# nomic-ai/contrastors

Measured on AMD Instinct MI355X. Metric: query-doc pairs/sec (whole node), nomic-bert-2048 seq128 global-batch 16384, higher is better.
Workload: dtype bf16

## Files before the change

contrastors_amd/_C.py:

```python
from __future__ import annotations

import ctypes as C
import os
from pathlib import Path

_PKG = Path(__file__).resolve().parent
LIB_PATH = Path(os.environ.get("CONTRASTORS_HIP_LIB", _PKG / "lib" / "libcontrastors_hip.so"))

CX_OK = 0
_ERR = {-1: "CX_ERR_SHAPE", -2: "CX_ERR_ALIGN", -3: "CX_ERR_ARG", -4: "CX_ERR_LAUNCH"}

vp = C.c_void_p
i32 = C.c_int
i64 = C.c_long
f32 = C.c_float
u64 = C.c_ulonglong
u32 = C.c_uint


class CxLayerWeights(C.Structure):
    _fields_ = (
        [(n, vp) for n in ("Wqkv", "Wout", "Wfc1", "Wfc2", "WqkvT", "WoutT", "Wfc1T", "Wfc2T")]
        + [(n, vp) for n in ("bqkv", "bout", "bfc1", "bfc2")]
        + [(n, vp) for n in ("ln1_g", "ln1_b", "ln2_g", "ln2_b")]
# ... 52 lines not shown
    "cx_error_string": (C.c_char_p, [i32]),
    "cx_gemm_bf16_nt": (i32, [vp, vp, vp, vp, i32, i32, i32, i32, i32, i32, i32, i32, f32, vp]),
    "cx_gemm_bf16_nt_accum": (i32, [vp, vp, vp, vp, i64, i32, i32, i32, i32, i32, vp]),
    "cx_gemm_bf16_tn_accum": (i32, [vp, vp, vp, vp, i64, i32, i32, i32, i32, i32, vp]),
    "cx_prof_gemm_config": (i32, [i32, i32]),
    "cx_prof_gemm_collect": (i32, [C.POINTER(C.c_double), C.POINTER(C.c_double), C.POINTER(i64), C.POINTER(i64)]),
    "cx_calib_mfma_bf16": (i32, [vp, i32, i32, vp, vp, vp]),
    "cx_calib_copy": (i32, [vp, vp, i64, vp]),
    "cx_transpose_bf16": (i32, [vp, vp, i32, i32, i32, i32, i32, vp]),
    "cx_cast_f32_to_bf16": (i32, [vp, vp, i64, vp]),
    "cx_cast_transpose_f32_to_bf16": (i32, [vp, vp, i32, i32, vp]),
    "cx_cast_transpose_f32_to_bf16_batched": (i32, [vp, i32, i32, vp]),
    "cx_cast_bf16_to_f32": (i32, [vp, vp, i64, vp]),
    "cx_layernorm_fwd": (i32, [vp, vp, vp, vp, vp, vp, vp, vp, i32, i32, f32, vp]),
    "cx_layernorm_bwd": (i32, [vp, vp, vp, vp, vp, vp, vp, vp, vp, vp, vp, i64, i32, i32, vp]),
    "cx_layernorm_bwd_pooled": (i32, [vp, vp, vp, vp, i32, i32, i32, vp, vp, vp, vp, vp, vp, vp, vp, vp, i64, i32, i32, vp]),
    "cx_layernorm_bwd_colsum": (i32, [vp, vp, vp, vp, vp, vp, vp, vp, vp, vp, vp, vp, i64, i32, i32, vp]),
    "cx_dropout_add_layernorm_fwd": (i32, [vp, vp, vp, vp, vp, vp, vp, vp, i32, i32, f32, f32, C.c_ulonglong, C.c_ulonglong,
                                           C.c_uint, vp]),
    "cx_dropout_add_layernorm_bwd": (i32, [vp, vp, vp, vp, vp, vp, vp, vp, vp, vp, vp, i64, i32, i32, f32, C.c_ulonglong,
                                           C.c_ulonglong, C.c_uint, vp]),
    "cx_dropout_add_layernorm_bwd_colsum": (i32, [vp, vp, vp, vp, vp, vp, vp, vp, vp, vp, vp, vp, i64, i32, i32, f32, C.c_ulonglong,
                                                  C.c_ulonglong, C.c_uint, vp]),
    "cx_dropout_scale": (i32, [vp, i64, f32, C.c_ulonglong, C.c_ulonglong, C.c_uint, vp]),
    "cx_layernorm_fwd_mixed": (i32, [vp, vp, vp, vp, vp, vp, vp, vp, i32, i32, f32, i32, vp]),
    "cx_layernorm_bwd_mixed": (i32, [vp, vp, vp, vp, vp, vp, vp, vp, vp, vp, i32, i32, i32, vp]),
    "cx_embed_ln_fwd": (i32, [vp, vp, vp, vp, vp, vp, vp, vp, vp, vp, i32, i32, i32, f32, vp]),
    "cx_embed_ln_bwd": (i32, [vp] * 15 + [i32, i32, i32, i32, vp]),
    "cx_embed_ln_bwd_sorted": (i32, [vp] * 15 + [i32, i32, i32, i32, i32, vp, vp, vp, vp]),
    "cx_swiglu_fwd": (i32, [vp, vp, i32, i32, i32, vp]),
    "cx_swiglu_bwd": (i32, [vp, vp, vp, i32, i32, i32, vp]),
    "cx_gemm_bf16_swiglu": (i32, [vp, vp, vp, vp, i32, i32, i32, i32, i32, i32, i32, vp]),
    "cx_gemm_bf16_nt_residual": (i32, [vp, vp, vp, vp, vp, i32, i32, i32, i32, i32, i32, i32, vp]),
    "cx_gemm_bf16_swiglu_bwd": (i32, [vp, vp, vp, vp, i32, i32, i32, i32, i32, i32, vp]),
    "cx_gemm_bf16_nt_splitk": (i32, [vp, vp, vp, vp, vp, vp, i64, i32, i32, i32, i32, i32, i32, i32, vp]),
    "cx_gemm_bf16_swiglu_gate": (i32, [vp, vp, vp, vp, i32, i32, i32, i32, i32, i32, i32, vp]),
    "cx_gemm_bf16_swiglu_bwd_gate": (i32, [vp, vp, vp, vp, vp, i32, i32, i32, i32, i32, i32, i32, vp]),
    "cx_swiglu_bwd_gate": (i32, [vp, vp, vp, vp, i32, i32, vp]),
    "cx_gemm_bf16_bias_gelu": (i32, [vp, vp, vp, vp, vp, i32, i32, i32, i32, i32, i32, i32, vp]),
    "cx_gemm_bf16_bias_act": (i32, [vp, vp, vp, vp, vp, i32, i32, i32, i32, i32, i32, i32, i32, vp]),
    "cx_bias_gelu_fwd": (i32, [vp, vp, vp, i32, i32, vp]),
    "cx_bias_gelu_bwd": (i32, [vp, vp, vp, vp, i32, i32, vp]),
    "cx_bias_grad": (i32, [vp, vp, i32, i32, i32, vp]),
    "cx_bias_gelu_bwd_colsum": (i32, [vp, vp, vp, vp, vp, i32, i32, vp]),
    "cx_bias_act_fwd": (i32, [vp, vp, vp, i32, i32, i32, vp]),
    "cx_bias_act_bwd_colsum": (i32, [vp, vp, vp, vp, vp, i32, i32, i32, vp]),
    "cx_gemm_bf16_act_bwd": (i32, [vp, vp, vp, vp, vp, vp, i64, i32, i32, i32, i32, i32, i32, i32, i32, vp]),
    "cx_attn_varlen_fwd": (i32, [vp, vp, vp, vp, vp, vp, i32, i32, i32, i32, f32, vp]),
    "cx_attn_varlen_bwd": (i32, [vp] * 9 + [i32, i32, i32, i32, f32, vp]),
    "cx_attn_varlen_bwd_prerotated": (i32, [vp] * 9 + [i32, i32, i32, i32, f32, vp]),
    "cx_attn_varlen_dropout_fwd": (i32, [vp] * 6 + [i32, i32, i32, i32, f32, f32, u64, u64, u32, vp]),
    "cx_attn_varlen_dropout_bwd": (i32, [vp] * 9 + [i32, i32, i32, i32, f32, f32, u64, u64, u32, vp]),
    "cx_ipc_alloc": (i32, [C.POINTER(vp), i64, i32]),
    "cx_ipc_free": (i32, [vp]),
    "cx_ipc_export": (i32, [vp, vp]),
    "cx_ipc_open": (i32, [vp, C.POINTER(vp)]),
    "cx_ipc_close": (i32, [vp]),
    "cx_xgmi_push": (i32, [vp, vp, i64, i64, i32, vp]),
    "cx_xgmi_scatter": (i32, [vp, vp, i32, i64, i32, vp]),
    "cx_xgmi_signal_wait": (i32, [vp, vp, i32, i32, u32, i64, vp, vp]),
    "cx_sum_slots_f32": (i32, [vp, vp, i64, i32, vp]),
    "cx_attn_varlen_kvpacked_fwd": (i32, [vp] * 6 + [i32, i32, i32, i32, i32, f32, vp]),
    "cx_attn_varlen_kvpacked_bwd": (i32, [vp] * 10 + [i32, i32, i32, i32, i32, f32, vp]),
    "cx_rotary_qkv_inplace": (i32, [vp, vp, vp, vp, i32, i32, i32, i32, i32, vp]),
    "cx_rotary_apply": (i32, [vp, i64, vp, vp, vp, i32, i32, i32, i32, i32, vp]),
    "cx_pool_normalize_fwd": (i32, [vp, vp, vp, vp, i32, i32, i32, i32, vp]),
# ... 29 lines not shown
    "cx_infonce_ws_floats": (i64, [i32, i32]),
    "cx_infonce_fwd": (i32, [vp, vp, vp, f32, vp, vp, vp, i32, i32, i32, i32, i32, vp]),
    "cx_infonce_argmax_ws_floats": (i64, [i32, i32]),
    "cx_infonce_fwd_argmax": (i32, [vp, vp, vp, f32, vp, vp, vp, vp, i32, i32, i32, i32, i32, vp]),
    "cx_infonce_bwd": (i32, [vp, vp, vp, vp, f32, f32, vp, vp, vp, vp, vp, vp, vp, i32, i32, i32, i32, i32, vp]),
    "cx_search_ws_bytes": (i64, [i32, i64, i32, i32]),
    "cx_search_topk": (i32, [vp, vp, i32, i64, i32, i64, i64, i32, vp, vp, vp, i32, vp, vp, vp, vp]),
    "cx_pack_sign_bits": (i32, [vp, i32, i64, i32, i64, vp, i64, vp]),
    "cx_search_hamming_ws_bytes": (i64, [i32, i64, i32, i32]),
    "cx_search_hamming_topk": (i32, [vp, vp, i32, i64, i32, i64, i64, i32, vp, vp, vp, i32, vp, vp, vp, vp]),
    "cx_rescore_topk": (i32, [vp, vp, vp, vp, i32, i64, i32, i64, i64, i32, i32, vp, vp, vp, vp]),
    "cx_embed_ln_fwd_typed": (i32, [vp, vp, vp, vp, vp, i32, vp, vp, vp, vp, vp, vp, i32, i32, i32, f32, vp]),
    "cx_embed_ln_bwd_typed": (i32, [vp] * 7 + [i32] + [vp] * 10 + [i64, i32, i32, i32, i32, vp]),
    "cx_embed_ln_bwd_sorted_typed": (i32, [vp] * 7 + [i32] + [vp] * 10 + [i64, i32, i32, i32, i32, i32, vp, vp, vp, vp]),
    "cx_seqcls_ws_floats": (i64, [i32, i32, i32]),
    "cx_seqcls_head_fwd": (i32, [vp, i64, vp, vp, vp, vp, vp, i32, f32, u64, u64, vp, vp, vp, i32, i32, i32, vp]),
    "cx_seqcls_head_bwd": (i32, [vp, i64, vp, vp, vp, vp, vp, i32, f32, f32, u64, u64, vp, i64, vp, vp, vp, vp, vp, i32, i32,
                                 i32, vp]),
    "cx_simkl_ws_floats": (i64, [i32, i32]),
    "cx_simkl_fwd": (i32, [vp, vp, vp, vp, f32, vp, vp, vp, vp, i32, i32, i32, i32, i32, i32, i32, i32, vp]),
    "cx_simkl_bwd": (i32, [vp, vp, vp, vp, vp, vp, f32, f32, vp, vp, vp, vp, vp, vp, i32, i32, i32, i32, i32, i32, i32, i32, vp]),
    "cx_infonce_fp8_ws_floats": (i64, [i32, i32]),
    "cx_infonce_fp8_fwd": (i32, [vp, vp, vp, f32, vp, vp, vp, vp, vp, vp, vp, i32, i32, i32, i32, i32, vp]),
    "cx_infonce_fp8_bwd": (i32, [vp, vp, vp, vp, f32, f32, vp, vp, vp, vp, vp, vp, vp, vp, vp, i64, vp, vp, vp, i32, i32, i32,
                                 i32, i32, vp]),
    "cx_sgemm_nt": (i32, [vp, vp, vp, i32, i32, i32, i32, i32, i32, vp]),
    "cx_transpose_f32": (i32, [vp, vp, i32, i32, i32, i32, vp]),
    "cx_encoder_forward": (i32, [C.POINTER(CxEncoderDesc), C.POINTER(CxChunkBuffers), vp, vp, vp, i32, i32, i32,
                                 i32, i32, vp, vp]),
    "cx_encoder_forward_typed": (i32, [C.POINTER(CxEncoderDesc), C.POINTER(CxChunkBuffers), vp, vp, vp, vp, i32, i32, i32,
                                       i32, i32, vp, vp]),
    "cx_encoder_backward_typed": (i32, [C.POINTER(CxEncoderDesc), C.POINTER(CxChunkBuffers), vp, vp, vp, vp, i32, i32, i32,
                                        i32, vp, vp, vp, vp, vp]),
    "cx_encoder_forward_hidden": (i32, [C.POINTER(CxEncoderDesc), C.POINTER(CxChunkBuffers), vp, vp, vp, i32, i32, i32,
                                        i32, i32, vp, vp]),
    "cx_encoder_backward_hidden": (i32, [C.POINTER(CxEncoderDesc), C.POINTER(CxChunkBuffers), vp, vp, vp, i32, i32, i32,
                                         i32, vp, vp, vp, vp]),
    "cx_encoder_backward": (i32, [C.POINTER(CxEncoderDesc), C.POINTER(CxChunkBuffers), vp, vp, vp, i32, i32, i32,
                                  i32, vp, vp, vp, vp, vp]),
}

_DEV_SIGS = {
    "cx_gemm_set_variant": (None, [i32]),
    "cx_gemm_get_variant": (i32, []),
    "cx_gemm_set_debug": (None, [i32]),
    "cx_gemm_set_trace": (None, [vp]),
    "cx_gemm_v6_ablate": (None, [i32]),
    "cx_gemm_v6_trace": (None, [vp]),
    "cx_gemm_v7_mode": (None, [i32]),
    "cx_gemm_v7_trace": (None, [vp]),
    "cx_gemm_v7_occupancy": (i32, []),
    "cx_gemm_v7_ablate": (None, [i32]),
    "cx_gemm_v7_flags": (None, [i32]),
    "cx_gemm_v7_period": (None, [i32]),
    "cx_gemm_set_glds": (None, [i32]),
    "cx_gemm_get_glds": (i32, []),
    "cx_attn_set_bwd_s128": (None, [i32]),
    "cx_attn_set_prio": (None, [i32]),
    "cx_attn_set_fwd_s128": (None, [i32]),
    "cx_attn_set_fwd_long": (None, [i32]),
    "cx_attn_set_bwd_long": (None, [i32]),
    "cx_probe_mfma_layout": (i32, [vp, vp]),
    "cx_probe_ds_read_tr16": (i32, [vp, vp, vp]),
    "cx_probe_mfma_rate": (i32, [vp, i32, i32, i32, vp, vp, vp]),
    "cx_attn_dropout_keep_mask": (i32, [vp, i32, i32, i32, f32, u64, u64, u32, vp]),
    "cx_probe_rmw": (i32, [vp, i64, i32, i32, i32, vp]),
# ... 61 lines not shown
```

contrastors_amd/csrc/cx_common.h:

```cpp
#pragma once
#include <hip/hip_runtime.h>
#include <stdint.h>
#include "../../include/contrastors_hip.h"

typedef uint16_t bf16_t;

typedef __attribute__((ext_vector_type(8))) __bf16 bf16x8_t;
typedef __attribute__((ext_vector_type(4))) __bf16 bf16x4_t;
typedef __attribute__((ext_vector_type(16))) float f32x16_t;
typedef __attribute__((ext_vector_type(4))) float f32x4_t;
typedef __attribute__((ext_vector_type(2))) float f32x2_t;
typedef __attribute__((ext_vector_type(4))) uint32_t u32x4_t;
typedef __attribute__((ext_vector_type(2))) uint32_t u32x2_t;

#define CX_DEVICE __device__ __forceinline__

CX_DEVICE float bf16_to_f32(bf16_t v) { return __uint_as_float(((uint32_t)v) << 16); }
CX_DEVICE float bf16lo_to_f32(uint32_t packed) { return __uint_as_float(packed << 16); }
CX_DEVICE float bf16hi_to_f32(uint32_t packed) { return __uint_as_float(packed & 0xffff0000u); }

typedef float cx_f32x2 __attribute__((ext_vector_type(2)));
typedef __bf16 cx_bf16x2 __attribute__((ext_vector_type(2)));
CX_DEVICE uint32_t pack_bf16x2(float lo, float hi) {
    const cx_f32x2 v = {lo, hi};
// ... 14 lines not shown
    v.z = pack_bf16x2(f[4], f[5]); v.w = pack_bf16x2(f[6], f[7]);
    return v;
}
CX_DEVICE void load8_f32(const float* p, float (&f)[8]) {
    const float4 a = *reinterpret_cast<const float4*>(p), b = *reinterpret_cast<const float4*>(p + 4);
    f[0] = a.x; f[1] = a.y; f[2] = a.z; f[3] = a.w; f[4] = b.x; f[5] = b.y; f[6] = b.z; f[7] = b.w;
}

CX_DEVICE int ycol(int c, int I, int layout) { return layout ? ((c >> 5) << 6) + (c & 31) : c; }
CX_DEVICE int gcol(int c, int I, int layout) { return layout ? ((c >> 5) << 6) + 32 + (c & 31) : I + c; }

CX_DEVICE float sigmoid_fast(float x) { return __builtin_amdgcn_rcpf(1.f + __builtin_amdgcn_exp2f(-1.4426950408889634f * x)); }

CX_DEVICE void rotary_pair(float x1, float x2, float c, float s, float& o1, float& o2) {
#pragma clang fp contract(off)
    o1 = __builtin_fmaf(x1, c, -(x2 * s));
    o2 = __builtin_fmaf(x2, c, x1 * s);
}

CX_DEVICE float rcp_clamped(float g) { return __builtin_amdgcn_fmed3f(__builtin_amdgcn_rcpf(g), -3.4028235e38f, 3.4028235e38f); }
CX_DEVICE void swiglu_bwd_from_act(float d, float act, float g, float& dy, float& dg) {
    const float s = sigmoid_fast(g);
    dy = g * s * d;
    dg = (d * act) * (rcp_clamped(g) + 1.f - s);
}
typedef float cx_f2 __attribute__((ext_vector_type(2)));
CX_DEVICE void swiglu_bwd_from_act2(cx_f2 d, cx_f2 act, cx_f2 g, cx_f2& dy, cx_f2& dg) {
    const cx_f2 m = g * -1.4426950408889634f;
    const cx_f2 t = cx_f2{__builtin_amdgcn_exp2f(m.x), __builtin_amdgcn_exp2f(m.y)} + 1.f;
    const cx_f2 s = {__builtin_amdgcn_rcpf(t.x), __builtin_amdgcn_rcpf(t.y)};
    dy = g * s * d;
    const cx_f2 w = cx_f2{rcp_clamped(g.x), rcp_clamped(g.y)} + 1.f - s;
    dg = (d * act) * w;
}

CX_DEVICE float gelu_cdf(float v, float& gauss) {
    const float av = fabsf(v);
    const float t = __builtin_amdgcn_rcpf(1.f + 0.3275911f * 0.70710678118654752f * av);
    const float poly =
        t * (0.254829592f + t * (-0.284496736f + t * (1.421413741f + t * (-1.453152027f + t * 1.061405429f))));
    gauss = __builtin_amdgcn_exp2f(-0.72134752044448170f * v * v);
    const float erf_abs = 1.f - poly * gauss;
    return 0.5f * (1.f + copysignf(erf_abs, v));
}

enum { CX_ACT_GELU = 0, CX_ACT_QUICK_GELU = 1 };
CX_DEVICE float act_val(float v, int act) {
    if (act == CX_ACT_QUICK_GELU) return v * __builtin_amdgcn_rcpf(1.f + __builtin_amdgcn_exp2f(-1.702f * 1.4426950408889634f * v));
    float gauss;
    return v * gelu_cdf(v, gauss);
}
CX_DEVICE float act_grad(float v, int act) {
    if (act == CX_ACT_QUICK_GELU) {
        const float s = __builtin_amdgcn_rcpf(1.f + __builtin_amdgcn_exp2f(-1.702f * 1.4426950408889634f * v));
        return s * (1.f + 1.702f * v * (1.f - s));
    }
    float gauss;
    const float cdf = gelu_cdf(v, gauss);
    return cdf + v * 0.3989422804014327f * gauss;
}

CX_DEVICE float wave_sum(float v) {
#pragma unroll
    for (int o = 32; o > 0; o >>= 1) v += __shfl_xor(v, o, 64);
    return v;
}
// ... 67 lines not shown
```

contrastors_amd/csrc/engine.hip:

```cpp
#include <hip/hip_runtime.h>
#include "../../include/contrastors_hip.h"
#include "ln_workspace.h"

namespace {

#define CX_TRY(expr)              \
    do {                          \
        int rc__ = (expr);        \
        if (rc__ != CX_OK) return rc__; \
    } while (0)

inline long round_up(long v, long m) { return (v + m - 1) / m * m; }

inline int mark_grads_done(const CxChunkBuffers* buf, int idx, void* stream) {
    if (!buf->layer_events || !buf->layer_events[idx]) return CX_OK;
    return hipEventRecord((hipEvent_t)buf->layer_events[idx], (hipStream_t)stream) == hipSuccess ? CX_OK : CX_ERR_LAUNCH;
}

struct Slots {
    const CxChunkBuffers* b;
    const CxEncoderDesc* e;
    long T_cap;
    int d, I, wfc1;
    int mode;
// ... 40 lines not shown
                 save ? (buf->checkpoint ? 2 : 1) : 0, L - keep};
}

int check_desc(const CxEncoderDesc* e, const CxChunkBuffers* b, int T) {
    if (!e || !b || !e->layers) return CX_ERR_ARG;
    if (e->n_layer <= 0 || e->d <= 0 || e->n_head <= 0) return CX_ERR_ARG;
    if (e->d != e->n_head * 64) return CX_ERR_SHAPE;
    if ((e->d % 64) != 0 || (e->d_inner % 64) != 0) return CX_ERR_SHAPE;
    if (b->T_cap < round_up(T, 64)) return CX_ERR_SHAPE;
    return CX_OK;
}

int wgrad_split(int out_f, int in_f, long Tp) {
    const long tiles = (long)((out_f + 127) / 128) * ((in_f + 127) / 128);
    const long nk = Tp / 64;
    long s = (512 + tiles - 1) / tiles;
    if (s > nk / 2) s = nk / 2;
    if (s < 1) s = 1;
    return (int)s;
}

int wgrad(const uint16_t* dY, int out_f, const uint16_t* X, int in_f, float* gW, const CxChunkBuffers* b, int T,
          void* stream) {
    if (!gW) return CX_OK;
    const int rc = cx_gemm_bf16_tn_accum(dY, X, gW, b->ws_f32, b->ws_floats, T, out_f, in_f, out_f, in_f, stream);
    if (rc != CX_ERR_SHAPE) return rc;
    if (!b->tr_a || !b->tr_b) return CX_ERR_ARG;
    const int Tp = (int)round_up(T, 64);
    CX_TRY(cx_transpose_bf16(dY, b->tr_a, T, out_f, out_f, Tp, Tp, stream));
    CX_TRY(cx_transpose_bf16(X, b->tr_b, T, in_f, in_f, Tp, Tp, stream));
    return cx_gemm_bf16_nt_accum(b->tr_a, b->tr_b, gW, b->ws_f32, b->ws_floats, out_f, in_f, Tp, Tp, Tp, stream);
}

int proj_residual(const uint16_t* x, const uint16_t* W, const float* bias, const uint16_t* residual, uint16_t* out, int T,
                  int N, int K, bool* folded, void* stream, const CxChunkBuffers* buf = nullptr) {
    *folded = false;
    if (buf && buf->ws_f32 && (long)((T + 255) / 256) * ((N + 255) / 256) <= 64 && K >= 1536) {
        const int rc = cx_gemm_bf16_nt_splitk(x, W, out, bias, residual, buf->ws_f32, buf->ws_floats, T, N, K, K, K, N, N, stream);
        if (rc != CX_ERR_SHAPE) {
            *folded = residual != nullptr && rc == CX_OK;
            return rc;
        }
    }
    if (residual) {
        const int rc = cx_gemm_bf16_nt_residual(x, W, out, bias, residual, T, N, K, K, K, N, N, stream);
        if (rc != CX_ERR_SHAPE) {
            *folded = rc == CX_OK;
            return rc;
        }
    }
    return cx_gemm_bf16_nt(x, W, out, bias, T, N, K, K, K, N, 0, 1, 1.f, stream);
}

bool gelu_fused_shape(int T, int N, int K) {
    return T > 0 && (K % 64) == 0 && (N % 8) == 0;
}

struct BlockRunner {
    const CxEncoderDesc* enc;
    const CxChunkBuffers* buf;
    const Slots& s;
    const int32_t* cu_seqlens;
    int Bc, T, max_seqlen;
    void* stream;
    const CxVitExt* ext = nullptr;

    int mlp_up(const CxLayerWeights& w, const uint16_t* x, int l, bool keep) const {
        const int d = enc->d, I = enc->d_inner;
        if (ext_subln(ext)) {
            uint16_t* yg = ext->yg_wide ? ext->yg_wide : buf->g_wide;
            CX_TRY(cx_gemm_bf16_nt(x, w.Wfc1, yg, w.bfc1, T, 2 * I, d, d, d, 2 * I, 0, 1, 1.f, stream));
            const CxVitSubLN& n = ext->sub_ln[l];
            return cx_swiglu_subln_fwd(yg, n.norm_g, n.norm_b, keep ? s.yg(l) : nullptr, s.act(l), s.ez(ext, l), s.ezmean(ext, l),
                                       s.ezrstd(ext, l), T, I, ext->subln_eps, stream);
        }
        if (enc->gated) {
            return cx_gemm_bf16_swiglu_gate(x, w.Wfc1, keep ? s.yg(l) : nullptr, s.act(l), T, I, d, d, d, I, I, stream);
        }
        const int rc = cx_gemm_bf16_bias_act(x, w.Wfc1, w.bfc1, keep ? s.yg(l) : nullptr, s.act(l), T, s.wfc1, d, d, d, s.wfc1,
                                             I, enc->mlp_act, stream);
        if (rc != CX_ERR_SHAPE) return rc;
        CX_TRY(cx_gemm_bf16_nt(x, w.Wfc1, s.yg(l), nullptr, T, s.wfc1, d, d, d, s.wfc1, 0, 1, 1.f, stream));
        return cx_bias_act_fwd(s.yg(l), w.bfc1, s.act(l), T, I, enc->mlp_act, stream);
    }
    int mlp(const CxLayerWeights& w, const uint16_t* x, int l, uint16_t* out, const uint16_t* residual, bool keep,
            bool* folded) const {
        CX_TRY(mlp_up(w, x, l, keep));
        return proj_residual(ext_subln(ext) ? s.ez(ext, l) : s.act(l), w.Wfc2, w.bfc2, residual, out, T, enc->d, enc->d_inner, folded, stream, buf);
    }
    int attn(const CxLayerWeights& w, const uint16_t* x, int l, uint16_t* out, const uint16_t* residual, bool* folded) const {
        const int d = enc->d;
        CX_TRY(cx_gemm_bf16_nt(x, w.Wqkv, s.qkv(l), w.bqkv, T, 3 * d, d, d, d, 3 * d, 0, 1, 1.f, stream));
        if (ext_rope(ext))
            CX_TRY(cx_rope2d_qkv_inplace(s.qkv(l), cu_seqlens, ext->rope_cos, ext->rope_sin, ext->n_rope, Bc, enc->n_head, T,
                                         ext->n_prefix, 1, stream));
        if (buf->drop_active && enc->attn_pdrop > 0.f) {
            CX_TRY(cx_attn_varlen_dropout_fwd(s.qkv(l), cu_seqlens, enc->rot_cos, enc->rot_sin, s.ctx(l), s.lse(l), Bc,
                                              enc->n_head, T, max_seqlen, enc->softmax_scale, enc->attn_pdrop, buf->drop_seed,
                                              buf->drop_offset, (unsigned)(2 * enc->n_layer + 1 + l), stream));
        } else if (enc->rot_cos && max_seqlen > 128) {
            CX_TRY(cx_rotary_qkv_inplace(s.qkv(l), cu_seqlens, enc->rot_cos, enc->rot_sin, Bc, enc->n_head, T, max_seqlen, 1,
                                         stream));
            CX_TRY(cx_attn_varlen_fwd(s.qkv(l), cu_seqlens, nullptr, nullptr, s.ctx(l), s.lse(l), Bc, enc->n_head, T, max_seqlen,
                                      enc->softmax_scale, stream));
        } else {
            CX_TRY(cx_attn_varlen_fwd(s.qkv(l), cu_seqlens, enc->rot_cos, enc->rot_sin, s.ctx(l), s.lse(l), Bc, enc->n_head, T,
                                      max_seqlen, enc->softmax_scale, stream));
        }
        return proj_residual(s.ctx(l), w.Wout, w.bout, residual, out, T, d, d, folded, stream);
    }
    int post_block(int l, const uint16_t* h_in, bool keep) const {
        const CxLayerWeights& w = enc->layers[l];
        const int d = enc->d;
        bool f1 = false, f2 = false;
        if (drop()) {
            const float p = enc->resid_pdrop;
            CX_TRY(attn(w, h_in, l, s.z1(l), nullptr, &f1));
            CX_TRY(cx_dropout_add_layernorm_fwd(s.z1(l), h_in, w.ln1_g, w.ln1_b, s.h1(l), keep ? s.z1(l) : nullptr, s.mean1(l),
                                                s.rstd1(l), T, d, enc->ln_eps, p, buf->drop_seed, buf->drop_offset, 2 * l, stream));
            CX_TRY(mlp(w, s.h1(l), l, s.z2(l), nullptr, keep, &f2));
            return cx_dropout_add_layernorm_fwd(s.z2(l), s.h1(l), w.ln2_g, w.ln2_b, s.h2(l), keep ? s.z2(l) : nullptr, s.mean2(l),
                                                s.rstd2(l), T, d, enc->ln_eps, p, buf->drop_seed, buf->drop_offset, 2 * l + 1,
                                                stream);
        }
        CX_TRY(attn(w, h_in, l, s.z1(l), h_in, &f1));
        CX_TRY(cx_layernorm_fwd(s.z1(l), f1 ? nullptr : h_in, w.ln1_g, w.ln1_b, s.h1(l), (keep && !f1) ? s.z1(l) : nullptr,
                                s.mean1(l), s.rstd1(l), T, d, enc->ln_eps, stream));
        CX_TRY(mlp(w, s.h1(l), l, s.z2(l), s.h1(l), keep, &f2));
        return cx_layernorm_fwd(s.z2(l), f2 ? nullptr : s.h1(l), w.ln2_g, w.ln2_b, s.h2(l), (keep && !f2) ? s.z2(l) : nullptr,
                                s.mean2(l), s.rstd2(l), T, d, enc->ln_eps, stream);
    }
    bool drop() const { return buf->drop_active && enc->resid_pdrop > 0.f; }
    int pre_block(int l, const uint16_t* x, const uint16_t* r, bool r_folded, bool keep, bool up_only, const uint16_t** x_out,
                  const uint16_t** r_out, bool* folded_out) const {
        const CxLayerWeights& w = enc->layers[l];
        const int d = enc->d, L = enc->n_layer;
        CX_TRY(cx_layernorm_fwd(x, r, w.ln1_g, w.ln1_b, s.h1(l), (r_folded && x == s.z1(l)) ? nullptr : s.z1(l), s.mean1(l),
                                s.rstd1(l), T, d, enc->ln_eps, stream));
        bool f1 = false, f2 = false;
        CX_TRY(attn(w, s.h1(l), l, s.z2(l), s.z1(l), &f1));
        CX_TRY(cx_layernorm_fwd(s.z2(l), f1 ? nullptr : s.z1(l), w.ln2_g, w.ln2_b, s.h2(l), f1 ? nullptr : s.z2(l), s.mean2(l),
                                s.rstd2(l), T, d, enc->ln_eps, stream));
        if (up_only) return mlp_up(w, s.h2(l), l, keep);
        uint16_t* nxt = (l + 1 < L) ? s.z1(l + 1) : buf->zf;
        CX_TRY(mlp(w, s.h2(l), l, nxt, s.z2(l), keep, &f2));
        *x_out = nxt;
        *r_out = f2 ? nullptr : s.z2(l);
        *folded_out = f2;
        return CX_OK;
    }
};

int blocks_forward(const CxEncoderDesc* enc, const CxChunkBuffers* buf, const Slots& s, const uint16_t* h0,
                   const int32_t* cu_seqlens, int Bc, int T, int max_seqlen, int save, const uint16_t** h_final,
                   void* stream, const CxVitExt* ext = nullptr) {
    const int d = enc->d, L = enc->n_layer;
    const BlockRunner run{enc, buf, s, cu_seqlens, Bc, T, max_seqlen, stream, ext};
    if (!enc->prenorm) {
        const uint16_t* h_in = h0;
        for (int l = 0; l < L; ++l) {
            CX_TRY(run.post_block(l, h_in, save != 0 && s.kept(l)));
            h_in = s.h2(l);
        }
        *h_final = h_in;
        return CX_OK;
    }
    if (!buf->zf || !buf->hf || !buf->meanf || !buf->rstdf || (!ext_no_lnf(ext) && (!enc->lnf_g || !enc->lnf_b))) return CX_ERR_ARG;
    if (buf->drop_active && enc->resid_pdrop > 0.f) return CX_ERR_ARG;
    const uint16_t* x = h0;
    const uint16_t* r = nullptr;
    bool r_folded = false;
    for (int l = 0; l < L; ++l) {
        CX_TRY(run.pre_block(l, x, r, r_folded, save != 0 && s.kept(l), false, &x, &r, &r_folded));
        if (save == 2 && !r_folded) return CX_ERR_SHAPE;
    }
    if (ext_no_lnf(ext)) {
        if (!r_folded || x != buf->zf) return CX_ERR_SHAPE;
        *h_final = buf->zf;
        return CX_OK;
    }
    CX_TRY(cx_layernorm_fwd(x, r, enc->lnf_g, enc->lnf_b, buf->hf, r_folded ? nullptr : buf->zf, buf->meanf, buf->rstdf, T,
                            d, enc->ln_eps, stream));
    *h_final = buf->hf;
    return CX_OK;
}

int check_bwd_buffers(const CxChunkBuffers* buf) {
    return (!buf->g_a || !buf->g_b || !buf->g_c || !buf->g_wide || !buf->g_act || !buf->delta ||
            !buf->ws_f32) ? CX_ERR_ARG : CX_OK;
}
// ... 3 lines not shown
    const int Tp = (int)round_up(T, 64);
    if (Tp == T) return CX_OK;
    const int d = enc->d, I = enc->d_inner, L = enc->n_layer;
    auto clear = [&](uint16_t* base, int width) {
        return hipMemsetAsync(base + (size_t)T * width, 0, (size_t)(Tp - T) * width * sizeof(uint16_t),
                              (hipStream_t)stream) == hipSuccess ? CX_OK : CX_ERR_LAUNCH;
    };
    CX_TRY(clear(buf->g_a, d));
    CX_TRY(clear(buf->g_b, d));
    CX_TRY(clear(buf->g_c, d));
    if (buf->g_d) CX_TRY(clear(buf->g_d, d));
    CX_TRY(clear(buf->g_wide, 3 * d));
    CX_TRY(clear(buf->g_wide, s.wfc1));
    CX_TRY(clear(buf->h0, d));
    for (int l = 0; l < L; ++l) {
        CX_TRY(clear(s.act(l), I));
        CX_TRY(clear(s.h1(l), d));
        CX_TRY(clear(s.ctx(l), d));
        CX_TRY(clear(s.h2(l), d));
        if (ext_subln(ext)) CX_TRY(clear(s.ez(ext, l), I));
    }
    return CX_OK;
}

struct PooledGrad {
    const float* demb;
    const float* emb;
    const float* norm;
    int pool_mode, normalize;
};

int blocks_backward(const CxEncoderDesc* enc, const CxChunkBuffers* buf, const Slots& s, const int32_t* cu_seqlens, int Bc,
                    int T, int max_seqlen, const PooledGrad* pg, const uint16_t** da_out, const uint16_t** db_out, void* stream,
                    const CxVitExt* ext = nullptr) {
    const int d = enc->d, I = enc->d_inner, H = enc->n_head, L = enc->n_layer;
    auto mlp_bwd = [&](const CxLayerWeights& w, int l, const uint16_t* dm, const uint16_t* mlp_in, const uint16_t* add,
                       bool* folded, bool bias_done) -> int {
        if (w.gbfc2 && !bias_done) CX_TRY(cx_bias_grad(dm, w.gbfc2, T, d, d, stream));
        if (ext_subln(ext)) {
            CX_TRY(wgrad(dm, d, s.ez(ext, l), I, w.gWfc2, buf, T, stream));
            CX_TRY(cx_gemm_bf16_nt(dm, w.Wfc2T, buf->g_act, nullptr, T, I, d, d, d, I, 0, 1, 1.f, stream));
            const CxVitSubLN& n = ext->sub_ln[l];
            CX_TRY(cx_swiglu_subln_bwd(buf->g_act, s.act(l), s.yg(l), s.ezmean(ext, l), s.ezrstd(ext, l), n.norm_g, buf->g_wide,
                                       n.gnorm_g, n.gnorm_b, w.gbfc1, buf->ws_f32, buf->ws_floats, T, I, stream));
            CX_TRY(wgrad(buf->g_wide, s.wfc1, mlp_in, d, w.gWfc1, buf, T, stream));
            return proj_residual(buf->g_wide, w.Wfc1T, nullptr, add, buf->g_b, T, d, s.wfc1, folded, stream, buf);
        }
        CX_TRY(wgrad(dm, d, s.act(l), I, w.gWfc2, buf, T, stream));
        int fused = CX_ERR_SHAPE;
        if (enc->gated)
            fused = cx_gemm_bf16_swiglu_bwd_gate(dm, w.Wfc2T, s.act(l), s.yg(l), buf->g_wide, T, I, d, d, d, I, s.wfc1, stream);
#ifndef CX_AB_R5_ROUTES
        if (!enc->gated && gelu_fused_shape(T, s.wfc1, d))
            fused = cx_gemm_bf16_act_bwd(dm, w.Wfc2T, s.yg(l), buf->g_wide, w.gbfc1, buf->ws_f32, buf->ws_floats, T, I, d, d, d, I, I,
                                         enc->mlp_act, stream);
#endif
        if (fused != CX_ERR_SHAPE) {
            CX_TRY(fused);
        } else {
            CX_TRY(cx_gemm_bf16_nt(dm, w.Wfc2T, buf->g_act, nullptr, T, I, d, d, d, I, 0, 1, 1.f, stream));
        }
        if (enc->gated) {
            if (fused == CX_ERR_SHAPE)
                CX_TRY(cx_swiglu_bwd_gate(buf->g_act, s.act(l), s.yg(l), buf->g_wide, T, I, stream));
        } else if (fused == CX_ERR_SHAPE) {
            CX_TRY(cx_bias_act_bwd_colsum(buf->g_act, s.yg(l), gelu_fused_shape(T, s.wfc1, d) ? nullptr : w.bfc1, buf->g_wide,
                                          w.gbfc1, T, I, enc->mlp_act, stream));
// ... 2 lines not shown
        return proj_residual(buf->g_wide, w.Wfc1T, nullptr, add, buf->g_b, T, d, s.wfc1, folded, stream, buf);
    };
    auto attn_bwd = [&](const CxLayerWeights& w, int l, const uint16_t* dx, const uint16_t* attn_in, const uint16_t* add,
                        bool* folded, bool bias_done) -> int {
        if (w.gbout && !bias_done) CX_TRY(cx_bias_grad(dx, w.gbout, T, d, d, stream));
        CX_TRY(wgrad(dx, d, s.ctx(l), d, w.gWout, buf, T, stream));
        CX_TRY(cx_gemm_bf16_nt(dx, w.WoutT, buf->g_b, nullptr, T, d, d, d, d, d, 0, 1, 1.f, stream));
        if (buf->drop_active && enc->attn_pdrop > 0.f) {
            CX_TRY(cx_attn_varlen_dropout_bwd(buf->g_b, s.qkv(l), s.ctx(l), s.lse(l), cu_seqlens, enc->rot_cos, enc->rot_sin,
                                              buf->delta, buf->g_wide, Bc, H, T, max_seqlen, enc->softmax_scale, enc->attn_pdrop,
                                              buf->drop_seed, buf->drop_offset, (unsigned)(2 * enc->n_layer + 1 + l), stream));
        } else if (enc->rot_cos && max_seqlen > 128) {
            CX_TRY(cx_attn_varlen_bwd_prerotated(buf->g_b, s.qkv(l), s.ctx(l), s.lse(l), cu_seqlens, enc->rot_cos, enc->rot_sin,
                                                 buf->delta, buf->g_wide, Bc, H, T, max_seqlen, enc->softmax_scale, stream));
        } else {
            CX_TRY(cx_attn_varlen_bwd(buf->g_b, s.qkv(l), s.ctx(l), s.lse(l), cu_seqlens, enc->rot_cos, enc->rot_sin,
                                      buf->delta, buf->g_wide, Bc, H, T, max_seqlen, enc->softmax_scale, stream));
        }
        if (ext_rope(ext))
            CX_TRY(cx_rope2d_qkv_inplace(buf->g_wide, cu_seqlens, ext->rope_cos, ext->rope_sin, ext->n_rope, Bc, H, T, ext->n_prefix,
                                         -1, stream));
        if (w.gbqkv) CX_TRY(cx_bias_grad(buf->g_wide, w.gbqkv, T, 3 * d, 3 * d, stream));
        CX_TRY(wgrad(buf->g_wide, 3 * d, attn_in, d, w.gWqkv, buf, T, stream));
        return proj_residual(buf->g_wide, w.WqkvT, nullptr, add, buf->g_b, T, d, 3 * d, folded, stream, buf);
    };
    const bool ws_holds_colsum = cx_ln_bwd_ws_holds(buf->ws_f32, buf->ws_floats, 3, d);
    auto ln_bwd = [&](const uint16_t* a, const uint16_t* b2, const uint16_t* z, const float* g, const float* mean,
                      const float* rstd, const uint16_t* dz_extra, uint16_t* dz, float* gg, float* gb, float* gbias,
                      bool* done) -> int {
        *done = gbias && ws_holds_colsum;
        return cx_layernorm_bwd_colsum(a, b2, z, g, mean, rstd, dz_extra, dz, gg, gb, *done ? gbias : nullptr, buf->ws_f32,
                                       buf->ws_floats, T, d, stream);
    };
    const BlockRunner run{enc, buf, s, cu_seqlens, Bc, T, max_seqlen, stream, ext};
    if (!enc->prenorm) {
        const uint16_t* da = buf->g_a;
        const uint16_t* db = nullptr;
        for (int l = L - 1; l >= 0; --l) {
            const CxLayerWeights& w = enc->layers[l];
            const uint16_t* h_in = (l == 0) ? buf->h0 : s.h2(l - 1);
            if (!s.kept(l)) CX_TRY(run.post_block(l, h_in, true));
            if (run.drop()) {
                if (!buf->g_d) return CX_ERR_ARG;
                const float p = enc->resid_pdrop;
                bool f1 = false, f2 = false;
#ifdef CX_AB_R5_ROUTES
                const bool cs = false;
#else
                const bool cs = ws_holds_colsum;
#endif
                CX_TRY(cx_dropout_add_layernorm_bwd_colsum(da, db, s.z2(l), w.ln2_g, s.mean2(l), s.rstd2(l), buf->g_c, buf->g_d, w.gln2_g,
                                                           w.gln2_b, cs ? w.gbfc2 : nullptr, buf->ws_f32, buf->ws_floats, T, d, p,
                                                           buf->drop_seed, buf->drop_offset, 2 * l + 1, stream));
                CX_TRY(mlp_bwd(w, l, buf->g_d, s.h1(l), buf->g_c, &f1, cs));
                CX_TRY(cx_dropout_add_layernorm_bwd_colsum(f1 ? buf->g_b : buf->g_c, f1 ? nullptr : buf->g_b, s.z1(l), w.ln1_g, s.mean1(l),
                                                           s.rstd1(l), buf->g_a, buf->g_d, w.gln1_g, w.gln1_b, cs ? w.gbout : nullptr,
                                                           buf->ws_f32, buf->ws_floats, T, d, p, buf->drop_seed, buf->drop_offset, 2 * l,
                                                           stream));
                CX_TRY(attn_bwd(w, l, buf->g_d, h_in, buf->g_a, &f2, cs));
                da = f2 ? buf->g_b : buf->g_a;
                db = f2 ? nullptr : buf->g_b;
                CX_TRY(mark_grads_done(buf, l, stream));
                continue;
            }
            bool b2_done = false, b1_done = false;
            if (pg && l == L - 1) {
                const bool cs = w.gbfc2 && ws_holds_colsum;
// ... 124 lines not shown
                                     enc->normalize, stream));
    }
    const uint16_t* da = nullptr;
    const uint16_t* db = nullptr;
    CX_TRY(blocks_backward(enc, buf, s, cu_seqlens, Bc, T, S, fold_pool ? &pg : nullptr, &da, &db, stream, ext));
    if (db) return CX_ERR_ARG;
    if (enc->lnpre_g) {
        if (!buf->zpre) return CX_ERR_ARG;
        CX_TRY(cx_layernorm_bwd(da, nullptr, buf->zpre, enc->lnpre_g, buf->emb_mean, buf->emb_rstd, nullptr, buf->g_a,
                                enc->glnpre_g, enc->glnpre_b, buf->ws_f32, buf->ws_floats, T, d, stream));
        da = buf->g_a;
    }
    const int Tp = Bc * P, Tpp = (int)round_up(Tp, 64);
    if (Tpp > Tp) {
        if (hipMemsetAsync(buf->patch_proj + (size_t)Tp * d, 0, (size_t)(Tpp - Tp) * d * 2, (hipStream_t)stream) != hipSuccess ||
            hipMemsetAsync(buf->patch_in + (size_t)Tp * enc->patch_dim, 0, (size_t)(Tpp - Tp) * enc->patch_dim * 2,
                           (hipStream_t)stream) != hipSuccess)
            return CX_ERR_LAUNCH;
    }
    if (buf->patch_keep) {
        if (!buf->patch_inv || buf->n_keep != P || buf->n_patch_all < P) return CX_ERR_ARG;
        CX_TRY(cx_vit_assemble_bwd_gather(da, buf->patch_proj, enc->gcls_token, enc->gvit_pos, Bc, P, d, buf->patch_inv,
                                          buf->n_patch_all, stream));
    } else {
        CX_TRY(cx_vit_assemble_bwd(da, buf->patch_proj, enc->gcls_token, enc->gvit_pos, Bc, P, d, stream));
    }
    if (enc->gbpatch) CX_TRY(cx_bias_grad(buf->patch_proj, enc->gbpatch, Tp, d, d, stream));
    CX_TRY(wgrad(buf->patch_proj, d, buf->patch_in, enc->patch_dim, enc->gWpatch, buf, Tp, stream));
    return mark_grads_done(buf, enc->n_layer, stream);
}

int text_forward_impl(const CxEncoderDesc* enc, const CxChunkBuffers* buf, const int64_t* input_ids,
                      const int64_t* token_type_ids, const int32_t* indices, const int32_t* cu_seqlens, int Bc, int S, int T,
                      int max_seqlen, int save_for_backward, float* emb_out, void* stream) {
    if (Bc <= 0 || T <= 0) return CX_OK;
    CX_TRY(check_desc(enc, buf, T));
    (void)hipGetLastError();
    const int d = enc->d, I = enc->d_inner;
    const Slots s = make_slots(enc, buf, save_for_backward);
    if (token_type_ids)
        CX_TRY(cx_embed_ln_fwd_typed(input_ids, token_type_ids, indices, enc->word_emb, enc->type_emb, 2, enc->pos_emb,
                                     enc->emb_ln_g, enc->emb_ln_b, buf->h0, buf->emb_mean, buf->emb_rstd, T, S, d, enc->ln_eps,
                                     stream));
    else
        CX_TRY(cx_embed_ln_fwd(input_ids, indices, enc->word_emb, enc->type_emb, enc->pos_emb, enc->emb_ln_g,
                               enc->emb_ln_b, buf->h0, buf->emb_mean, buf->emb_rstd, T, S, d, enc->ln_eps, stream));
    if (buf->drop_active && enc->embd_pdrop > 0.f)
        CX_TRY(cx_dropout_scale(buf->h0, (long)T * d, enc->embd_pdrop, buf->drop_seed, buf->drop_offset, 2 * enc->n_layer, stream));
    const uint16_t* h_final = nullptr;
    CX_TRY(blocks_forward(enc, buf, s, buf->h0, cu_seqlens, Bc, T, max_seqlen, s.mode, &h_final, stream));
    return cx_pool_normalize_fwd(h_final, cu_seqlens, emb_out, buf->pool_norm, Bc, d, enc->pool_mode, enc->normalize,
                                 stream);
}

int text_backward_impl(const CxEncoderDesc* enc, const CxChunkBuffers* buf, const int64_t* input_ids,
                       const int64_t* token_type_ids, const int32_t* indices, const int32_t* cu_seqlens, int Bc, int S, int T,
                       int max_seqlen, const float* demb, const float* emb_out, const int32_t* sort_ids,
                       const int32_t* sort_perm, void* stream) {
    if (Bc <= 0 || T <= 0) return CX_OK;
    CX_TRY(check_desc(enc, buf, T));
    if (!demb || !emb_out) return CX_ERR_ARG;
    CX_TRY(check_bwd_buffers(buf));
    (void)hipGetLastError();
    const int d = enc->d, I = enc->d_inner;
    const Slots s = make_slots(enc, buf, 1);
    CX_TRY(clear_pad_rows(enc, buf, s, T, stream));
    const PooledGrad pg{demb, emb_out, buf->pool_norm, enc->pool_mode, enc->normalize};
    const bool fold_pool = !(buf->drop_active && enc->resid_pdrop > 0.f) && (enc->pool_mode == 0 || enc->pool_mode == 1);
    if (!fold_pool)
        CX_TRY(cx_pool_normalize_bwd(demb, emb_out, buf->pool_norm, cu_seqlens, buf->g_a, Bc, d, enc->pool_mode,
                                     enc->normalize, stream));
    const uint16_t* da = fold_pool ? nullptr : buf->g_a;
    const uint16_t* db = nullptr;
    CX_TRY(blocks_backward(enc, buf, s, cu_seqlens, Bc, T, max_seqlen, fold_pool ? &pg : nullptr, &da, &db, stream));
    if (buf->drop_active && enc->embd_pdrop > 0.f) {
        CX_TRY(cx_dropout_scale(const_cast<uint16_t*>(da), (long)T * d, enc->embd_pdrop, buf->drop_seed, buf->drop_offset,
                                2 * enc->n_layer, stream));
        if (db)
            CX_TRY(cx_dropout_scale(const_cast<uint16_t*>(db), (long)T * d, enc->embd_pdrop, buf->drop_seed, buf->drop_offset,
                                    2 * enc->n_layer, stream));
    }
    if (token_type_ids && sort_ids && sort_perm) {
        CX_TRY(cx_embed_ln_bwd_sorted_typed(da, db, input_ids, token_type_ids, indices, enc->word_emb, enc->type_emb, 2,
                                            enc->pos_emb, enc->emb_ln_g, buf->emb_mean, buf->emb_rstd, enc->gword_emb,
                                            enc->gtype_emb, enc->gpos_emb, enc->gemb_ln_g, enc->gemb_ln_b, buf->ws_f32,
                                            buf->ws_floats, T, S, d, enc->padding_idx, enc->vocab, sort_ids, sort_perm,
                                            reinterpret_cast<float*>(buf->g_wide), stream));
    } else if (token_type_ids) {
        CX_TRY(cx_embed_ln_bwd_typed(da, db, input_ids, token_type_ids, indices, enc->word_emb, enc->type_emb, 2, enc->pos_emb,
                                     enc->emb_ln_g, buf->emb_mean, buf->emb_rstd, enc->gword_emb, enc->gtype_emb, enc->gpos_emb,
                                     enc->gemb_ln_g, enc->gemb_ln_b, buf->ws_f32, buf->ws_floats, T, S, d, enc->padding_idx,
                                     stream));
    } else if (sort_ids && sort_perm) {
        CX_TRY(cx_embed_ln_bwd_sorted(da, db, input_ids, indices, enc->word_emb, enc->type_emb, enc->pos_emb, enc->emb_ln_g,
                                      buf->emb_mean, buf->emb_rstd, enc->gword_emb, enc->gtype_emb, enc->gpos_emb,
                                      enc->gemb_ln_g, enc->gemb_ln_b, T, S, d, enc->padding_idx, enc->vocab, sort_ids,
                                      sort_perm, reinterpret_cast<float*>(buf->g_wide), stream));
    } else {
        CX_TRY(cx_embed_ln_bwd(da, db, input_ids, indices, enc->word_emb, enc->type_emb, enc->pos_emb, enc->emb_ln_g,
                               buf->emb_mean, buf->emb_rstd, enc->gword_emb, enc->gtype_emb, enc->gpos_emb,
                               enc->gemb_ln_g, enc->gemb_ln_b, T, S, d, enc->padding_idx, stream));
    }
    return mark_grads_done(buf, enc->n_layer, stream);
}
}

extern "C" {

int cx_encoder_forward(const CxEncoderDesc* enc, const CxChunkBuffers* buf, const int64_t* input_ids,
                       const int32_t* indices, const int32_t* cu_seqlens, int Bc, int S, int T, int max_seqlen,
                       int save_for_backward, float* emb_out, void* stream) {
    return text_forward_impl(enc, buf, input_ids, nullptr, indices, cu_seqlens, Bc, S, T, max_seqlen, save_for_backward, emb_out,
                             stream);
}
int cx_encoder_forward_typed(const CxEncoderDesc* enc, const CxChunkBuffers* buf, const int64_t* input_ids,
                             const int64_t* token_type_ids, const int32_t* indices, const int32_t* cu_seqlens, int Bc, int S,
                             int T, int max_seqlen, int save_for_backward, float* emb_out, void* stream) {
    return text_forward_impl(enc, buf, input_ids, token_type_ids, indices, cu_seqlens, Bc, S, T, max_seqlen, save_for_backward,
                             emb_out, stream);
}

int cx_encoder_backward(const CxEncoderDesc* enc, const CxChunkBuffers* buf, const int64_t* input_ids,
                        const int32_t* indices, const int32_t* cu_seqlens, int Bc, int S, int T, int max_seqlen,
                        const float* demb, const float* emb_out, const int32_t* sort_ids, const int32_t* sort_perm,
                        void* stream) {
    return text_backward_impl(enc, buf, input_ids, nullptr, indices, cu_seqlens, Bc, S, T, max_seqlen, demb, emb_out, sort_ids,
                              sort_perm, stream);
}
int cx_encoder_backward_typed(const CxEncoderDesc* enc, const CxChunkBuffers* buf, const int64_t* input_ids,
                              const int64_t* token_type_ids, const int32_t* indices, const int32_t* cu_seqlens, int Bc, int S,
                              int T, int max_seqlen, const float* demb, const float* emb_out, const int32_t* sort_ids,
                              const int32_t* sort_perm, void* stream) {
    return text_backward_impl(enc, buf, input_ids, token_type_ids, indices, cu_seqlens, Bc, S, T, max_seqlen, demb, emb_out,
                              sort_ids, sort_perm, stream);
}

int cx_encoder_forward_hidden(const CxEncoderDesc* enc, const CxChunkBuffers* buf, const int64_t* input_ids,
                              const int32_t* indices, const int32_t* cu_seqlens, int Bc, int S, int T, int max_seqlen,
                              int save_for_backward, uint16_t* hidden_out, void* stream) {
    if (Bc <= 0 || T <= 0) return CX_OK;
    CX_TRY(check_desc(enc, buf, T));
    if (!hidden_out) return CX_ERR_ARG;
    (void)hipGetLastError();
    const int d = enc->d, I = enc->d_inner;
    const Slots s = make_slots(enc, buf, save_for_backward);
    CX_TRY(cx_embed_ln_fwd(input_ids, indices, enc->word_emb, enc->type_emb, enc->pos_emb, enc->emb_ln_g,
                           enc->emb_ln_b, buf->h0, buf->emb_mean, buf->emb_rstd, T, S, d, enc->ln_eps, stream));
    if (buf->drop_active && enc->embd_pdrop > 0.f)
        CX_TRY(cx_dropout_scale(buf->h0, (long)T * d, enc->embd_pdrop, buf->drop_seed, buf->drop_offset, 2 * enc->n_layer, stream));
    const uint16_t* h_final = nullptr;
    CX_TRY(blocks_forward(enc, buf, s, buf->h0, cu_seqlens, Bc, T, max_seqlen, s.mode, &h_final, stream));
    return hipMemcpyAsync(hidden_out, h_final, (size_t)T * d * sizeof(uint16_t), hipMemcpyDeviceToDevice,
                          (hipStream_t)stream) == hipSuccess ? CX_OK : CX_ERR_LAUNCH;
}

int cx_encoder_backward_hidden(const CxEncoderDesc* enc, const CxChunkBuffers* buf, const int64_t* input_ids,
                               const int32_t* indices, const int32_t* cu_seqlens, int Bc, int S, int T, int max_seqlen,
                               const uint16_t* dhidden, const int32_t* sort_ids, const int32_t* sort_perm, void* stream) {
    if (Bc <= 0 || T <= 0) return CX_OK;
    CX_TRY(check_desc(enc, buf, T));
    if (!dhidden) return CX_ERR_ARG;
    CX_TRY(check_bwd_buffers(buf));
    (void)hipGetLastError();
    const int d = enc->d, I = enc->d_inner;
    const Slots s = make_slots(enc, buf, 1);
    CX_TRY(clear_pad_rows(enc, buf, s, T, stream));
    if (hipMemcpyAsync(buf->g_a, dhidden, (size_t)T * d * sizeof(uint16_t), hipMemcpyDeviceToDevice,
// ... 94 lines not shown
```

contrastors_amd/csrc/gemm_api.hip:

```cpp
#include "cx_common.h"
#include "../../include/contrastors_hip.h"
#include "gemm_params.h"
#include <mutex>

namespace {

constexpr int BK = 64;

__global__ __launch_bounds__(256) void splitk_reduce_kernel(const float* __restrict__ part, float* __restrict__ out, long n4,
                                                            long slab, int splits) {
    const long stride = (long)gridDim.x * blockDim.x;
    for (long i = (long)blockIdx.x * blockDim.x + threadIdx.x; i < n4; i += stride) {
        float4 a = reinterpret_cast<const float4*>(out)[i];
        for (int s = 0; s < splits; ++s) {
            const float4 v = reinterpret_cast<const float4*>(part + s * slab)[i];
            a.x += v.x; a.y += v.y; a.z += v.z; a.w += v.w;
        }
        reinterpret_cast<float4*>(out)[i] = a;
    }
}

int reduce_slabs(const float* ws, float* out, long slab, int split, hipStream_t s) {
    const long n4 = slab / 4;
    long g = (n4 + 255) / 256;
// ... 133 lines not shown
    GemmParams p = base_params(X, W, YG, nullptr, M, 2 * I, K, ldx, ldw, ld_yg);
    p.Out2 = Act; p.ldo2 = ld_act;
    ProfScope prof(2.0 * (double)M * (double)(2 * I) * (double)K, (hipStream_t)stream);
    const hipError_t e = ((ld_yg % 8) == 0 && (ld_act % 8) == 0)
                             ? cx_launch_gemm_v6(p, GEMM_EPI_SWIGLU, (hipStream_t)stream)
                             : cx_launch_gemm_v5(p, 0, GEMM_OUT_BF16, GEMM_EPI_SWIGLU, (hipStream_t)stream);
    return e == hipSuccess ? CX_OK : CX_ERR_LAUNCH;
}

int cx_gemm_bf16_swiglu_gate(const uint16_t* X, const uint16_t* W, uint16_t* G, uint16_t* Act, int M, int I, int K, int ldx,
                             int ldw, int ld_g, int ld_act, void* stream) {
    if (M <= 0 || I <= 0) return CX_OK;
    if (K <= 0 || (K % BK) != 0 || (I % 32) != 0 || (ld_g % 8) != 0 || (ld_act % 8) != 0) return CX_ERR_SHAPE;
    if ((ldx % 8) != 0 || (ldw % 8) != 0) return CX_ERR_ALIGN;
    if (!Act) return CX_ERR_ARG;
    GemmParams p = base_params(X, W, G, nullptr, M, 2 * I, K, ldx, ldw, ld_g);
    p.Out2 = Act; p.ldo2 = ld_act;
    ProfScope prof(2.0 * (double)M * (double)(2 * I) * (double)K, (hipStream_t)stream);
    return cx_launch_gemm_v6(p, GEMM_EPI_SWIGLU_G, (hipStream_t)stream) == hipSuccess ? CX_OK : CX_ERR_LAUNCH;
}

int cx_gemm_bf16_nt_residual(const uint16_t* X, const uint16_t* W, uint16_t* Out, const float* bias, const uint16_t* Residual,
                             int M, int N, int K, int ldx, int ldw, int ldo, int ldr, void* stream) {
    if (M <= 0 || N <= 0) return CX_OK;
    if (!Residual || !Out) return CX_ERR_ARG;
    if (K <= 0 || (K % 64) != 0 || (N % 8) != 0 || (ldo % 8) != 0 || (ldr % 8) != 0) return CX_ERR_SHAPE;
    if ((ldx % 8) != 0 || (ldw % 8) != 0) return CX_ERR_ALIGN;
    GemmParams p = base_params(X, W, Out, bias, M, N, K, ldx, ldw, ldo);
    p.Out2 = const_cast<uint16_t*>(Residual); p.ldo2 = ldr;
    ProfScope prof(2.0 * (double)M * (double)N * (double)K, (hipStream_t)stream);
    return cx_launch_gemm_v6(p, GEMM_EPI_NONE, (hipStream_t)stream) == hipSuccess ? CX_OK : CX_ERR_LAUNCH;
}

int cx_gemm_bf16_bias_gelu(const uint16_t* X, const uint16_t* W, const float* bias, uint16_t* Pre, uint16_t* Act, int M, int N,
                           int K, int ldx, int ldw, int ld_pre, int ld_act, void* stream) {
    return cx_gemm_bf16_bias_act(X, W, bias, Pre, Act, M, N, K, ldx, ldw, ld_pre, ld_act, 0, stream);
}

int cx_gemm_bf16_bias_act(const uint16_t* X, const uint16_t* W, const float* bias, uint16_t* Pre, uint16_t* Act, int M, int N,
                          int K, int ldx, int ldw, int ld_pre, int ld_act, int act, void* stream) {
    if (M <= 0 || N <= 0) return CX_OK;
    if (!Act || (act != 0 && act != 1)) return CX_ERR_ARG;
    if (K <= 0 || (K % 64) != 0 || (N % 8) != 0 || (ld_act % 8) != 0 || (Pre && (ld_pre % 8) != 0)) return CX_ERR_SHAPE;
    if ((ldx % 8) != 0 || (ldw % 8) != 0) return CX_ERR_ALIGN;
    GemmParams p = base_params(X, W, Pre, bias, M, N, K, ldx, ldw, ld_pre);
    p.Out2 = Act; p.ldo2 = ld_act;
    p.act = act;
    ProfScope prof(2.0 * (double)M * (double)N * (double)K, (hipStream_t)stream);
    return cx_launch_gemm_v6(p, act == 1 ? GEMM_EPI_QGELU : GEMM_EPI_GELU, (hipStream_t)stream) == hipSuccess ? CX_OK : CX_ERR_LAUNCH;
}

int cx_gemm_bf16_swiglu_bwd(const uint16_t* dY, const uint16_t* W, const uint16_t* YG, uint16_t* dYG, int M, int I, int K,
                            int ldx, int ldw, int ld_yg, void* stream) {
    if (M <= 0 || I <= 0) return CX_OK;
    if (!dY || !W || !YG || !dYG) return CX_ERR_ARG;
    if (K <= 0 || (K % 64) != 0 || (I % 256) != 0 || (ld_yg % 8) != 0 || ld_yg < 2 * I) return CX_ERR_SHAPE;
    if ((ldx % 8) != 0 || (ldw % 8) != 0) return CX_ERR_ALIGN;
    GemmParams p = base_params(dY, W, dYG, nullptr, M, I, K, ldx, ldw, ld_yg);
    p.Out2 = const_cast<uint16_t*>(YG); p.ldo2 = ld_yg;
    ProfScope prof(2.0 * (double)M * (double)I * (double)K, (hipStream_t)stream);
    return cx_launch_gemm_v6(p, GEMM_EPI_SWIGLU_BWD, (hipStream_t)stream) == hipSuccess ? CX_OK : CX_ERR_LAUNCH;
}

int cx_gemm_bf16_swiglu_bwd_gate(const uint16_t* dY, const uint16_t* W, const uint16_t* Act, const uint16_t* G, uint16_t* dYG,
                                 int M, int I, int K, int ldx, int ldw, int ld_ag, int ld_dyg, void* stream) {
    if (M <= 0 || I <= 0) return CX_OK;
// ... 61 lines not shown
```

contrastors_amd/csrc/gemm_bf16.hip:

```cpp
#include "cx_common.h"
#include "../../include/contrastors_hip.h"
#include "gemm_params.h"

namespace {

constexpr int BM = 128, BN = 128, BK = 64;
constexpr int TILE_BYTES = 128 * BK * 2;

typedef __attribute__((address_space(3))) void* lds_void_ptr;
typedef const __attribute__((address_space(1))) void* glb_void_ptr;

enum OutMode { OUT_BF16 = GEMM_OUT_BF16, OUT_F32 = GEMM_OUT_F32, OUT_F32_ATOMIC = GEMM_OUT_F32_ATOMIC };

struct StageRegs { uint4 r0, r1, r2, r3; };

CX_DEVICE uint4 stage_load(const bf16_t* __restrict__ base, int ld, int row0, int nrows, int k0, int tid, int p) {
    const int r = p * 32 + (tid >> 3);
    int gr = row0 + r;
    gr = gr < nrows ? gr : nrows - 1;
    return *reinterpret_cast<const uint4*>(base + (size_t)gr * ld + k0 + (tid & 7) * 8);
}

template <bool GLDS>
CX_DEVICE void stage_tile(const bf16_t* __restrict__ base, int ld, int row0, int nrows, int k0, char* lds_tile,
// ... 765 lines not shown

int cx_gemm_bf16_nt_residual(const uint16_t* X, const uint16_t* W, uint16_t* Out, const float* bias,
                             const uint16_t* Residual, int M, int N, int K, int ldx, int ldw, int ldo, int ldr,
                             void* stream) {
    if (M <= 0 || N <= 0) return CX_OK;
    if (!Residual || !Out) return CX_ERR_ARG;
    if (K <= 0 || (K % 64) != 0 || (N % 8) != 0 || (ldo % 8) != 0 || (ldr % 8) != 0) return CX_ERR_SHAPE;
    if ((ldx % 8) != 0 || (ldw % 8) != 0) return CX_ERR_ALIGN;
    if (cx_gemm_get_variant() != 6) return CX_ERR_SHAPE;
    GemmParams p;
    p.X = X; p.W = W; p.Out = Out; p.bias = bias;
    p.M = M; p.N = N; p.K = K; p.ldx = ldx; p.ldw = ldw; p.ldo = ldo;
    p.tiles_m = p.tiles_n = 0; p.split_k = 1; p.alpha = 1.f; p.dbg = g_dbg;
    p.Out2 = const_cast<uint16_t*>(Residual); p.ldo2 = ldr; p.sup_m = p.sup_n = 0; p.trace = nullptr;
    int slot = -1;
    if (g_prof.enabled) {
        if ((g_prof.launches % g_prof.stride) == 0 && g_prof.used < GemmProf::CAP) {
            slot = g_prof.used++;
            if (slot >= g_prof.created) {
                if (hipEventCreate(&g_prof.ev0[slot]) != hipSuccess || hipEventCreate(&g_prof.ev1[slot]) != hipSuccess)
                    return CX_ERR_LAUNCH;
                g_prof.created = slot + 1;
            }
            g_prof.flop[slot] = 2.0 * (double)M * (double)N * (double)K;
            (void)hipEventRecord(g_prof.ev0[slot], (hipStream_t)stream);
        }
        ++g_prof.launches;
    }
    const hipError_t e = cx_launch_gemm_v6(p, GEMM_EPI_NONE, (hipStream_t)stream);
    if (slot >= 0) (void)hipEventRecord(g_prof.ev1[slot], (hipStream_t)stream);
    return e == hipSuccess ? CX_OK : CX_ERR_LAUNCH;
}

int cx_gemm_bf16_bias_gelu(const uint16_t* X, const uint16_t* W, const float* bias, uint16_t* Pre, uint16_t* Act, int M,
                           int N, int K, int ldx, int ldw, int ld_pre, int ld_act, void* stream) {
    return cx_gemm_bf16_bias_act(X, W, bias, Pre, Act, M, N, K, ldx, ldw, ld_pre, ld_act, 0, stream);
}

int cx_gemm_bf16_bias_act(const uint16_t* X, const uint16_t* W, const float* bias, uint16_t* Pre, uint16_t* Act, int M,
                          int N, int K, int ldx, int ldw, int ld_pre, int ld_act, int act, void* stream) {
    if (M <= 0 || N <= 0) return CX_OK;
    if (!Act || (act != 0 && act != 1)) return CX_ERR_ARG;
    if (K <= 0 || (K % 64) != 0 || (N % 8) != 0 || (ld_act % 8) != 0 || (Pre && (ld_pre % 8) != 0)) return CX_ERR_SHAPE;
    if ((ldx % 8) != 0 || (ldw % 8) != 0) return CX_ERR_ALIGN;
    if (cx_gemm_get_variant() != 6) return CX_ERR_SHAPE;
    GemmParams p;
    p.X = X; p.W = W; p.Out = Pre; p.bias = bias;
    p.M = M; p.N = N; p.K = K; p.ldx = ldx; p.ldw = ldw; p.ldo = ld_pre;
    p.tiles_m = p.tiles_n = 0; p.split_k = 1; p.alpha = 1.f; p.dbg = g_dbg;
    p.Out2 = Act; p.ldo2 = ld_act; p.sup_m = p.sup_n = 0; p.trace = nullptr;
    p.act = act;
    int slot = -1;
    if (g_prof.enabled) {
        if ((g_prof.launches % g_prof.stride) == 0 && g_prof.used < GemmProf::CAP) {
            slot = g_prof.used++;
            if (slot >= g_prof.created) {
                if (hipEventCreate(&g_prof.ev0[slot]) != hipSuccess || hipEventCreate(&g_prof.ev1[slot]) != hipSuccess)
                    return CX_ERR_LAUNCH;
                g_prof.created = slot + 1;
            }
            g_prof.flop[slot] = 2.0 * (double)M * (double)N * (double)K;
            (void)hipEventRecord(g_prof.ev0[slot], (hipStream_t)stream);
        }
        ++g_prof.launches;
    }
    const hipError_t e = cx_launch_gemm_v6(p, act == 1 ? GEMM_EPI_QGELU : GEMM_EPI_GELU, (hipStream_t)stream);
// ... 112 lines not shown
```

contrastors_amd/csrc/gemm_bf16_v6.hip:

```cpp
#include "cx_common.h"
#include "../../include/contrastors_hip.h"
#include "gemm_params.h"
#include <type_traits>

namespace {

#ifndef CX_V6_HI_EARLY
#define CX_V6_HI_EARLY 1
#endif
#ifndef CX_V6_OPAQUE
#define CX_V6_OPAQUE 1
#endif
#ifndef CX_V6_NT
#define CX_V6_NT 3
#endif
template <int J>
__device__ __forceinline__ void v6_dma_m0(uint32_t slot_base) {
    asm volatile("s_add_u32 m0, %0, %1" ::"s"(slot_base), "n"(J * 4096) : "memory", "scc");
}
__device__ __forceinline__ void v6_dma_ld(uint32_t off, const bf16_t* base) {
    asm volatile("global_load_lds_dwordx4 %0, %1" ::"v"(off), "s"(base) : "memory");
}
template <int J>
__device__ __forceinline__ void v6_dma_full(uint32_t slot_base, uint32_t off, const bf16_t* base) {
// ... 252 lines not shown
        const char* nxs = dsm + nxs_slot * XS6;
        const char* nws = dsm + (3 + nws_slot) * XS6;
        CX_SEG(mma1, F1, 32, 64, F0, nxs, nws, 0, RS_ == 2 ? 32 : 33, RS_, 2, RS_ == 2 ? 33 : 49, RS_ == 2 ? 8 : DS_, 4, 4);
        x_advance();
        if constexpr ((DBG & 128) != 0 && decltype(first)::value) {
            const long long now_ = (long long)__builtin_amdgcn_s_memtime();
            kt0_cyc += now_ - t_last;
        }
        ++cp_kt;
        pxs_slot = xs_slot;
        pws_slot = ws_slot;
        xs_slot = nxs_slot;
        ws_slot = nws_slot;
    };

#pragma unroll 1
    while (cp_tile >= 0) {
        cp_kt = 0;
        kt_body(std::true_type{});
#pragma unroll 1
        while (cp_kt < nk) kt_body(std::false_type{});

        {
            CX_PH(2);
            asm volatile("s_nop 7\n\ts_nop 7\n\ts_nop 7" ::: "memory");
            const int tn = cp_tile & 255, tm = cp_tile >> 8;
            const int m0 = tm * BM6 + wm * 128, n0 = tn * BN6 + wn * 128;
            char* my = ((wave < 2) ? dsm + pxs_slot * XS6 : dsm + (3 + pws_slot) * XS6) + (wave & 1) * 16384;
            constexpr int ROWB = 272;
            auto prow = [&](int q) { return (q >> 1) * 16 + l15; };
            auto pcol = [&](int q) { return (q & 1) * 16 + 4 * g4; };
            auto qoff = [](int q, int rowb) { return (q >> 1) * 16 * rowb + (q & 1) * 32; };
            if constexpr ((DBG & 16) != 0) {
            } else if constexpr (EPI == GEMM_EPI_NONE || EPI == GEMM_EPI_ACT_BWD || EPI == GEMM_EPI_QACT_BWD) {
                constexpr bool ACTB = EPI == GEMM_EPI_ACT_BWD || EPI == GEMM_EPI_QACT_BWD;
                float cs0 = 0.f, cs1 = 0.f, cs2 = 0.f, cs3 = 0.f, cs4 = 0.f, cs5 = 0.f, cs6 = 0.f, cs7 = 0.f;
                constexpr int act_kind = EPI == GEMM_EPI_QACT_BWD ? CX_ACT_QUICK_GELU : CX_ACT_GELU;
                auto mul_grad = [&](uint4& v, const uint4& r) {
#define CX_MG(w_, ca, cb)                                                                              \
    {                                                                                                 \
        const float o0 = bf16lo_to_f32(v.w_) * act_grad(bf16lo_to_f32(r.w_), act_kind);               \
        const float o1 = bf16hi_to_f32(v.w_) * act_grad(bf16hi_to_f32(r.w_), act_kind);               \
        v.w_ = pack_bf16x2(o0, o1);                                                                   \
        ca += bf16lo_to_f32(v.w_);                                                                    \
        cb += bf16hi_to_f32(v.w_);                                                                    \
    }
                    CX_MG(x, cs0, cs1) CX_MG(y, cs2, cs3) CX_MG(z, cs4, cs5) CX_MG(w, cs6, cs7)
#undef CX_MG
                };
                auto flush_colsum = [&]() {
                    if constexpr (ACTB) {
                        float c[8] = {cs0, cs1, cs2, cs3, cs4, cs5, cs6, cs7};
#pragma unroll
                        for (int e = 0; e < 8; ++e) {
                            c[e] += __shfl_xor(c[e], 16, 64);
                            c[e] += __shfl_xor(c[e], 32, 64);
                        }
                        const int n = n0 + (lane & 15) * 8;
                        if (p.colsum_part && lane < 16 && m0 < p.M && n + 8 <= p.N) {
                            float* dst = p.colsum_part + (size_t)(m0 >> 7) * p.N + n;
                            *reinterpret_cast<float4*>(dst) = make_float4(c[0], c[1], c[2], c[3]);
                            *reinterpret_cast<float4*>(dst + 4) = make_float4(c[4], c[5], c[6], c[7]);
                        }
                    }
                };
                const bool add_bias = p.bias != nullptr;
                const bf16_t* resid = reinterpret_cast<const bf16_t*>(p.Out2);
                auto fast_tile = [&](auto with_resid) {
                    constexpr bool RES = decltype(with_resid)::value;
                    const int rrow = lane >> 4, rch = lane & 15;
                    bf16_t* outp = reinterpret_cast<bf16_t*>(p.Out) + (size_t)(m0 + rrow) * p.ldo + n0 + rch * 8;
                    const bf16_t* resp = RES ? resid + (size_t)(m0 + rrow) * p.ldo2 + n0 + rch * 8 : nullptr;
                    const char* rd = my + rrow * ROWB + rch * 16;
                    char* wr = my + prow(0) * ROWB + pcol(0) * 2;
                    uint2 pk[16];
                    auto pack_pass = [&](int b) {
#pragma unroll
                        for (int a = 0; a < 4; ++a) {
                            float blk[16];
                            v6_read_block(4 * b + a, blk);
#pragma unroll
                            for (int q = 0; q < 4; ++q) {
                                pk[a * 4 + q].x = pack_bf16x2(blk[4 * q], blk[4 * q + 1]);
                                pk[a * 4 + q].y = pack_bf16x2(blk[4 * q + 2], blk[4 * q + 3]);
                            }
                        }
                    };
                    auto stage = [&]() {
#pragma unroll
                        for (int a = 0; a < 4; ++a)
#pragma unroll
                            for (int q = 0; q < 4; ++q) *reinterpret_cast<uint2*>(wr + a * 64 + qoff(q, ROWB)) = pk[a * 4 + q];
                    };
                    uint4 r0 = {}, r1 = {}, r2 = {}, r3 = {}, r4 = {}, r5 = {}, r6 = {}, r7 = {};
#define CX_RES_ROWS(b_)                                                                                   \
    r0 = gld(resp + (size_t)((b_) * 32 + 0) * p.ldo2);                          \
    r1 = gld(resp + (size_t)((b_) * 32 + 4) * p.ldo2);                          \
    r2 = gld(resp + (size_t)((b_) * 32 + 8) * p.ldo2);                          \
    r3 = gld(resp + (size_t)((b_) * 32 + 12) * p.ldo2);                         \
    r4 = gld(resp + (size_t)((b_) * 32 + 16) * p.ldo2);                         \
    r5 = gld(resp + (size_t)((b_) * 32 + 20) * p.ldo2);                         \
    r6 = gld(resp + (size_t)((b_) * 32 + 24) * p.ldo2);                         \
    r7 = gld(resp + (size_t)((b_) * 32 + 28) * p.ldo2);
                    auto add_res = [&](uint4& v, const uint4& r) {
                        v.x = pack_bf16x2(bf16lo_to_f32(v.x) + bf16lo_to_f32(r.x), bf16hi_to_f32(v.x) + bf16hi_to_f32(r.x));
                        v.y = pack_bf16x2(bf16lo_to_f32(v.y) + bf16lo_to_f32(r.y), bf16hi_to_f32(v.y) + bf16hi_to_f32(r.y));
                        v.z = pack_bf16x2(bf16lo_to_f32(v.z) + bf16lo_to_f32(r.z), bf16hi_to_f32(v.z) + bf16hi_to_f32(r.z));
// ... 4 lines not shown
                        uint4 v0 = *reinterpret_cast<const uint4*>(rd + 0 * ROWB), v1 = *reinterpret_cast<const uint4*>(rd + 4 * ROWB),
                              v2 = *reinterpret_cast<const uint4*>(rd + 8 * ROWB), v3 = *reinterpret_cast<const uint4*>(rd + 12 * ROWB),
                              v4 = *reinterpret_cast<const uint4*>(rd + 16 * ROWB), v5 = *reinterpret_cast<const uint4*>(rd + 20 * ROWB),
                              v6 = *reinterpret_cast<const uint4*>(rd + 24 * ROWB), v7 = *reinterpret_cast<const uint4*>(rd + 28 * ROWB);
                        __builtin_amdgcn_sched_barrier(0);
                        if constexpr (b < 3) pack_pass(b + 1);
                        __builtin_amdgcn_sched_barrier(0);
                        if constexpr (RES) {
                            add_res(v0, r0); add_res(v1, r1); add_res(v2, r2); add_res(v3, r3);
                            add_res(v4, r4); add_res(v5, r5); add_res(v6, r6); add_res(v7, r7);
                            if constexpr (b < 3) {
                                __builtin_amdgcn_sched_barrier(0);
                                CX_RES_ROWS(b + 1)
                                __builtin_amdgcn_sched_barrier(0);
                            }
                        }
                        if constexpr (b < 3) stage();
                        bf16_t* o = outp + (size_t)(b * 32) * p.ldo;
                        if constexpr ((DBG & 64) != 0) {
                            const uint4 vs[8] = {v0, v1, v2, v3, v4, v5, v6, v7};
#pragma unroll
                            for (int i = 0; i < 8; ++i) asm volatile("" ::"v"(vs[i].x), "v"(vs[i].y), "v"(vs[i].z), "v"(vs[i].w));
                            asm volatile("" ::"v"(o));
                            return;
                        }
                        gst(o, v0);
                        gst(o + (size_t)4 * p.ldo, v1);
                        gst(o + (size_t)8 * p.ldo, v2);
                        gst(o + (size_t)12 * p.ldo, v3);
                        gst(o + (size_t)16 * p.ldo, v4);
                        gst(o + (size_t)20 * p.ldo, v5);
                        gst(o + (size_t)24 * p.ldo, v6);
                        gst(o + (size_t)28 * p.ldo, v7);
                    };
                    if constexpr (RES) { CX_RES_ROWS(0) }
                    pack_pass(0);
                    stage();
                    one_pass(std::integral_constant<int, 0>{});
                    one_pass(std::integral_constant<int, 1>{});
                    one_pass(std::integral_constant<int, 2>{});
                    one_pass(std::integral_constant<int, 3>{});
#undef CX_RES_ROWS
                };
                auto fast_tile_actb = [&]() {
                    const int rrow = lane >> 4, rch = lane & 15;
                    bf16_t* outp = reinterpret_cast<bf16_t*>(p.Out) + (size_t)(m0 + rrow) * p.ldo + n0 + rch * 8;
                    const bf16_t* resp = resid + (size_t)(m0 + rrow) * p.ldo2 + n0 + rch * 8;
                    const char* rd = my + rrow * ROWB + rch * 16;
                    char* wr = my + prow(0) * ROWB + pcol(0) * 2;
                    auto stage_pass = [&](int b) {
#pragma unroll
                        for (int a = 0; a < 4; ++a) {
                            float blk[16];
                            v6_read_block(4 * b + a, blk);
#pragma unroll
                            for (int q = 0; q < 4; ++q) {
                                uint2 pk2;
                                pk2.x = pack_bf16x2(blk[4 * q], blk[4 * q + 1]);
                                pk2.y = pack_bf16x2(blk[4 * q + 2], blk[4 * q + 3]);
                                *reinterpret_cast<uint2*>(wr + a * 64 + qoff(q, ROWB)) = pk2;
                            }
                            __builtin_amdgcn_sched_barrier(0);
                        }
                    };
                    uint4 r0, r1, r2, r3;
#define CX_PRE_ROWS(hh_)                                                        \
    r0 = gld(resp + (size_t)((hh_) * 16 + 0) * p.ldo2);                         \
    r1 = gld(resp + (size_t)((hh_) * 16 + 4) * p.ldo2);                         \
    r2 = gld(resp + (size_t)((hh_) * 16 + 8) * p.ldo2);                         \
    r3 = gld(resp + (size_t)((hh_) * 16 + 12) * p.ldo2);
// ... 58 lines not shown
                                    if (add_bias) {
                                        const int n = n0 + nl;
                                        if (n < p.N) {
                                            const float4 bv = *reinterpret_cast<const float4*>(p.bias + n);
                                            v[0] += bv.x; v[1] += bv.y; v[2] += bv.z; v[3] += bv.w;
                                        }
                                    }
                                }
                                uint2 pk;
                                pk.x = pack_bf16x2(v[0], v[1]);
                                pk.y = pack_bf16x2(v[2], v[3]);
                                *reinterpret_cast<uint2*>(my + prow(q) * ROWB + nl * 2) = pk;
                            }
                        }
#pragma unroll
                        for (int ps = 0; ps < 8; ++ps) {
                            const int row = ps * 4 + (lane >> 4), ch = lane & 15;
                            const int m = m0 + b * 32 + row, n = n0 + ch * 8;
                            uint4 vv = *reinterpret_cast<const uint4*>(my + row * ROWB + ch * 16);
                            if (resid && ACTB) {
                                const uint4 rr = ps == 0 ? r0 : ps == 1 ? r1 : ps == 2 ? r2 : ps == 3 ? r3 : ps == 4 ? r4 : ps == 5 ? r5
                                                 : ps == 6 ? r6 : r7;
                                if (m < p.M && n + 8 <= p.N) mul_grad(vv, rr);
                            } else if (resid) {
                                const uint4 rr = ps == 0 ? r0 : ps == 1 ? r1 : ps == 2 ? r2 : ps == 3 ? r3 : ps == 4 ? r4 : ps == 5 ? r5
                                                 : ps == 6 ? r6 : r7;
                                vv.x = pack_bf16x2(bf16lo_to_f32(vv.x) + bf16lo_to_f32(rr.x), bf16hi_to_f32(vv.x) + bf16hi_to_f32(rr.x));
                                vv.y = pack_bf16x2(bf16lo_to_f32(vv.y) + bf16lo_to_f32(rr.y), bf16hi_to_f32(vv.y) + bf16hi_to_f32(rr.y));
                                vv.z = pack_bf16x2(bf16lo_to_f32(vv.z) + bf16lo_to_f32(rr.z), bf16hi_to_f32(vv.z) + bf16hi_to_f32(rr.z));
                                vv.w = pack_bf16x2(bf16lo_to_f32(vv.w) + bf16lo_to_f32(rr.w), bf16hi_to_f32(vv.w) + bf16hi_to_f32(rr.w));
                            }
                            if (m < p.M && n + 8 <= p.N)
                                gst(reinterpret_cast<bf16_t*>(p.Out) + (size_t)m * p.ldo + n, vv);
                        }
                    }
                };
                if constexpr (ACTB) {
                    if (fast) {
                        fast_tile_actb();
                    } else {
                        store_tile(std::true_type{});
                    }
                    flush_colsum();
                } else if (fast) {
                    if (resid) {
                        fast_tile(std::true_type{});
                    } else {
                        fast_tile(std::false_type{});
                    }
                } else if (p.alpha == 1.f && !add_bias) {
                    store_tile(std::true_type{});
                } else {
                    store_tile(std::false_type{});
                }
            } else if constexpr (IS_SWIGLU_BWD) {
                const bf16_t* yg_in = reinterpret_cast<const bf16_t*>(p.Out2);
                const bf16_t* g_in = reinterpret_cast<const bf16_t*>(p.In3);
                bf16_t* dyg = reinterpret_cast<bf16_t*>(p.Out);
                const int c0 = 2 * n0;
                auto bwd_elem = [&](float yv, float gv, float dv, float& dyo, float& dgo) {
                    if constexpr (AG) {
                        swiglu_bwd_from_act(dv, yv, gv, dyo, dgo);
                    } else {
                        const float sg = __builtin_amdgcn_rcpf(1.f + __builtin_amdgcn_exp2f(-1.4426950408889634f * gv));
                        const float gs = gv * sg;
                        dyo = gs * dv;
                        dgo = (sg + gs * (1.f - sg)) * dv * yv;
                    }
                };
                auto bwd_quad = [&](const float (&yv)[4], const float (&gv)[4], const float* dv, float (&dyo)[4], float (&dgo)[4]) {
                    if constexpr (AG) {
#pragma unroll
                        for (int h = 0; h < 2; ++h) {
                            cx_f2 y2, g2;
                            swiglu_bwd_from_act2(cx_f2{dv[2 * h], dv[2 * h + 1]}, cx_f2{yv[2 * h], yv[2 * h + 1]},
                                                 cx_f2{gv[2 * h], gv[2 * h + 1]}, y2, g2);
// ... 797 lines not shown
#ifndef CX_PRODUCT
    if (epi == GEMM_EPI_NONE && g_v6_dbg) {
        p.trace = g_v6_trace;
        switch (g_v6_dbg) {
            case 1: return launch6<GEMM_EPI_NONE, 1>(p, stream);
            case 2: return launch6<GEMM_EPI_NONE, 2>(p, stream);
            case 4: return launch6<GEMM_EPI_NONE, 4>(p, stream);
            case 16: return launch6<GEMM_EPI_NONE, 16>(p, stream);
            case 32: return launch6<GEMM_EPI_NONE, 32>(p, stream);
            case 33: return launch6<GEMM_EPI_NONE, 33>(p, stream);
            case 35: return launch6<GEMM_EPI_NONE, 35>(p, stream);
            case 39: return launch6<GEMM_EPI_NONE, 39>(p, stream);
            case 55: return launch6<GEMM_EPI_NONE, 55>(p, stream);
            case 59: return launch6<GEMM_EPI_NONE, 59>(p, stream);
            case 64: return launch6<GEMM_EPI_NONE, 64>(p, stream);
            case 128: return launch6<GEMM_EPI_NONE, 128>(p, stream);
            default: break;
        }
    }
#endif
#ifndef CX_PRODUCT
    if (g_v6_dbg == 128 && (epi == GEMM_EPI_SWIGLU_G || epi == GEMM_EPI_SWIGLU || epi == GEMM_EPI_SWIGLU_BWD_AG)) {
        p.trace = g_v6_trace;
        return epi == GEMM_EPI_SWIGLU_G ? launch6<GEMM_EPI_SWIGLU_G, 128>(p, stream)
               : epi == GEMM_EPI_SWIGLU ? launch6<GEMM_EPI_SWIGLU, 128>(p, stream) : launch6<GEMM_EPI_SWIGLU_BWD_AG, 128>(p, stream);
    }
#endif
    return epi == GEMM_EPI_SWIGLU ? launch6<GEMM_EPI_SWIGLU>(p, stream)
           : epi == GEMM_EPI_SWIGLU_G ? launch6<GEMM_EPI_SWIGLU_G>(p, stream)
           : epi == GEMM_EPI_SWIGLU_BWD_AG ? launch6<GEMM_EPI_SWIGLU_BWD_AG>(p, stream)
           : epi == GEMM_EPI_GELU ? launch6<GEMM_EPI_GELU>(p, stream)
           : epi == GEMM_EPI_QGELU ? launch6<GEMM_EPI_QGELU>(p, stream)
           : epi == GEMM_EPI_SWIGLU_BWD ? launch6<GEMM_EPI_SWIGLU_BWD>(p, stream)
           : epi == GEMM_EPI_ACT_BWD ? (p.act == CX_ACT_QUICK_GELU ? launch6<GEMM_EPI_QACT_BWD>(p, stream) : launch6<GEMM_EPI_ACT_BWD>(p, stream))
                                  : launch6<GEMM_EPI_NONE>(p, stream);
}
```

contrastors_amd/csrc/gemm_bf16_v7.hip:

```cpp
#include "cx_common.h"
#include "../../include/contrastors_hip.h"
#include "gemm_params.h"
#include <type_traits>

namespace {

#ifndef CX_V7_NT
#define CX_V7_NT 3
#endif

template <int IMM>
__device__ __forceinline__ void v7_dma_m0(uint32_t base) {
    asm volatile("s_add_u32 m0, %0, %1" ::"s"(base), "n"(IMM) : "memory", "scc");
}
__device__ __forceinline__ void v7_dma_ld(uint32_t off, const bf16_t* base) {
    asm volatile("global_load_lds_dwordx4 %0, %1" ::"v"(off), "s"(base) : "memory");
}
template <int IMM>
__device__ __forceinline__ void v7_dma_full(uint32_t slot_base, uint32_t off, const bf16_t* base) {
    asm volatile("s_add_u32 m0, %0, %1\n\ts_nop 0\n\tglobal_load_lds_dwordx4 %2, %3" ::"s"(slot_base), "n"(IMM), "v"(off), "s"(base)
                 : "memory", "scc");
}
typedef unsigned int v4u7 __attribute__((ext_vector_type(4)));
__device__ __forceinline__ __amdgpu_buffer_rsrc_t rsrc7(const void* base, uint32_t bytes) {
// ... 13 lines not shown
__device__ __forceinline__ void bst7(__amdgpu_buffer_rsrc_t r, uint32_t voff, uint32_t soff, uint4 v) {
    const v4u7 t = {v.x, v.y, v.z, v.w};
    __builtin_amdgcn_raw_buffer_store_b128(t, r, voff, soff, (CX_V7_NT & 1) ? 2 : 0);
}
template <uint32_t IMM>
__device__ __forceinline__ uint32_t vxor7(uint32_t a) {
    uint32_t r;
    asm volatile("v_xor_b32 %0, %2, %1" : "=v"(r) : "v"(a), "i"(IMM));
    return r;
}

typedef __attribute__((address_space(3))) void* lds_void_ptr7;

constexpr int BM7 = 256, BN7 = 128, BK7 = 64;
constexpr int XW7 = 8192;
constexpr int W0_OFF7 = 32768, SP_OFF7 = 49152, W1_OFF7 = 65536;
constexpr int LDS7 = 81920;

#define V7_MFMA(i, w, x) asm volatile("v_mfma_f32_32x32x16_bf16 %0, %1, %2, %0" : "+a"(acc[(i)]) : "v"(w), "v"(x))
#define V7_MFMA_Z(i, w, x) asm volatile("v_mfma_f32_32x32x16_bf16 %0, %1, %2, 0" : "=a"(acc[(i)]) : "v"(w), "v"(x))

struct XFrags7 {
    bf16x8_t f[2][4];
};
struct WFrags7 {
    bf16x8_t f[4];
};

template <int EPI, int DBG = 0>
__global__ __launch_bounds__(256, 2) __attribute__((amdgpu_waves_per_eu(2, 2))) void gemm_bf16_v7_kernel(GemmParams p) {
    extern __shared__ __attribute__((aligned(16))) char dsm[];
    constexpr bool IS_BWD = EPI == GEMM_EPI_SWIGLU_BWD_AG;
    constexpr bool IS_SWIGLU = EPI == GEMM_EPI_SWIGLU_G;
    static_assert(EPI == GEMM_EPI_NONE || IS_BWD || IS_SWIGLU, "v7 serves the plain / residual, SwiGLU (gate save) and SwiGLU-backward (act, gate) forms");
    const int tid = threadIdx.x;
    const int lane = tid & 63;
    const int wave = __builtin_amdgcn_readfirstlane(tid >> 6);
#ifndef CX_PRODUCT
    long long t_begin = 0;
    if (p.trace) t_begin = (long long)__builtin_amdgcn_s_memtime();
#endif
    const int hi_m = lane >> 5, l31_m = lane & 31;
    const int nk = p.K / BK7;
    const int per_xcd = gridDim.x >> 3;
    const int xcd = blockIdx.x & 7, idx = blockIdx.x >> 3;
    const int gn = p.sup_n > 0 ? p.sup_n : 1, gm = 8 / gn;
    const int xi = xcd / gn, xj = xcd - xi * gn;
    const int m_lo = p.tiles_m * xi / gm, m_hi = p.tiles_m * (xi + 1) / gm;
    const int n_lo = p.tiles_n * xj / gn, n_wd = p.tiles_n * (xj + 1) / gn - n_lo;
    const int nloc = (m_hi - m_lo) * n_wd;
    auto tile_of = [&](int round) {
        const int l = round * per_xcd + idx;
        if (l >= nloc) return -1;
        const int q = l / n_wd;
        return ((m_lo + q) << 8) | (n_lo + (l - q * n_wd));
    };

    uint32_t xoff[8], woff[8];
    const bf16_t* xbase = p.X;
    const bf16_t* wbase = p.W;
    int lx_round = 0, lx_kt = 0;
    int lw_round = 0, lw_kt = 0, lw_slot = 0;
    const int first_tile = tile_of(0);
    bool x_clamped = true, w_clamped = true;
    auto x_setup = [&](int tile) {
        const int tm = tile >> 8;
        xbase = p.X + (size_t)tm * BM7 * p.ldx;
// ... 173 lines not shown
        V7_SLOT(V7_MFMA, 1, W1, 3, 0, 0, read_w(W0, nws, 0, 1));
        V7_SLOT(V7_MFMA, 2, W1, 3, 0, 0, read_w(W0, nws, 0, 2));
        V7_SLOT(V7_MFMA, 3, W1, 3, 0, 0, read_w(W0, nws, 0, 3));
        V7_SLOT(V7_MFMA, 4, W1, 3, 0, 0, V7_NORD);
        V7_SLOT(V7_MFMA, 5, W1, 3, 0, 0, V7_NORD);
        V7_SLOT(V7_MFMA, 6, W1, 3, 0, 0, V7_NORD);
        V7_SLOT(V7_MFMA, 7, W1, 3, 0, 0, V7_NORD);
        ws_slot ^= 1;
    };

#pragma unroll 1
    while (cp_tile >= 0) {
        if (p.dbg & 1) __builtin_amdgcn_s_setprio(1);
        kt_body(std::true_type{});
#pragma unroll 1
        for (int kt = 1; kt < nk; ++kt) kt_body(std::false_type{});

        if (p.dbg & 1) __builtin_amdgcn_s_setprio(0);
        asm volatile("s_nop 7\n\ts_nop 7\n\ts_nop 7" : "+a"(acc[0]), "+a"(acc[1]), "+a"(acc[2]), "+a"(acc[3]), "+a"(acc[4]), "+a"(acc[5]), "+a"(acc[6]), "+a"(acc[7]));
        int le = lane;
        asm volatile("" : "+v"(le));
        const int hi = le >> 5, l31 = le & 31;
        const int tn = cp_tile & 255, tm = cp_tile >> 8;
        const int m0 = tm * BM7 + wave * 64, n0 = tn * BN7;
        const int rows_left = p.M - m0;
        const uint32_t rows_here = rows_left >= 64 ? 64u : (rows_left > 0 ? (uint32_t)rows_left : 0u);
        const uint32_t my = (uint32_t)((ws_slot ? W0_OFF7 : SP_OFF7) + wave * 8192);
        const uint32_t cb = my + (uint32_t)l31 * 256 + ((l31 & 15) << 4) + hi * 8;
        const int lrow = le >> 4, lch = le & 15;
        const uint32_t rb = my + (uint32_t)lrow * 256 + ((lch ^ lrow) << 4);
#define V7_CELL(c) (dsm + vxor7<((c) << 4)>(cb))
#define V7_ROW(i) (dsm + vxor7<(((i) & 3) << 6)>(rb) + 1024 * (i))
        if constexpr ((DBG & 16) != 0) {
        } else if constexpr (EPI == GEMM_EPI_NONE) {
            const bf16_t* resid = reinterpret_cast<const bf16_t*>(p.Out2);
            const __amdgpu_buffer_rsrc_t rs_out = rsrc7(reinterpret_cast<bf16_t*>(p.Out) + (size_t)m0 * p.ldo + n0, rows_here * (uint32_t)p.ldo * 2u);
            const uint32_t vo = ((uint32_t)lrow * (uint32_t)p.ldo + lch * 8) * 2u;
            const uint32_t so = (uint32_t)p.ldo * 8u;
            auto add_res = [&](uint4& v, const uint4& r) {
                v.x = pack_bf16x2(bf16lo_to_f32(v.x) + bf16lo_to_f32(r.x), bf16hi_to_f32(v.x) + bf16hi_to_f32(r.x));
                v.y = pack_bf16x2(bf16lo_to_f32(v.y) + bf16lo_to_f32(r.y), bf16hi_to_f32(v.y) + bf16hi_to_f32(r.y));
                v.z = pack_bf16x2(bf16lo_to_f32(v.z) + bf16lo_to_f32(r.z), bf16hi_to_f32(v.z) + bf16hi_to_f32(r.z));
                v.w = pack_bf16x2(bf16lo_to_f32(v.w) + bf16lo_to_f32(r.w), bf16hi_to_f32(v.w) + bf16hi_to_f32(r.w));
            };
            auto tile_epi = [&](auto with_resid, auto with_bias) {
                constexpr bool RES = decltype(with_resid)::value;
                constexpr bool BIAS = decltype(with_bias)::value;
                const __amdgpu_buffer_rsrc_t rs_bias = rsrc7(BIAS ? p.bias + n0 : nullptr, BIAS ? (uint32_t)BN7 * 4u : 0u);
                const __amdgpu_buffer_rsrc_t rs_res = rsrc7(RES ? resid + (size_t)m0 * p.ldo2 + n0 : nullptr, RES ? rows_here * (uint32_t)p.ldo2 * 2u : 0u);
                const uint32_t vr = ((uint32_t)lrow * (uint32_t)p.ldo2 + lch * 8) * 2u;
                const uint32_t sr = (uint32_t)p.ldo2 * 8u;
                uint4 r0 = {}, r1 = {}, r2 = {}, r3 = {}, r4 = {}, r5 = {}, r6 = {}, r7 = {};
#define V7_RES_ROWS(b_)                                                                                                     \
    r0 = bld7(rs_res, vr, sr * (8 * (b_) + 0)); r1 = bld7(rs_res, vr, sr * (8 * (b_) + 1)); r2 = bld7(rs_res, vr, sr * (8 * (b_) + 2)); \
    r3 = bld7(rs_res, vr, sr * (8 * (b_) + 3)); r4 = bld7(rs_res, vr, sr * (8 * (b_) + 4)); r5 = bld7(rs_res, vr, sr * (8 * (b_) + 5)); \
    r6 = bld7(rs_res, vr, sr * (8 * (b_) + 6)); r7 = bld7(rs_res, vr, sr * (8 * (b_) + 7));
                auto stage_pass = [&](auto bc) {
                    constexpr int b = decltype(bc)::value;
#pragma unroll
                    for (int a = 0; a < 4; ++a) {
                        uint2 pk[4];
                        float4 bq[4] = {};
                        if constexpr (BIAS) {
#pragma unroll
                            for (int q = 0; q < 4; ++q) bq[q] = bldf7(rs_bias, (uint32_t)hi * 16u, (uint32_t)(a * 128 + q * 32));
                        }
#pragma unroll
                        for (int q = 0; q < 4; ++q) {
                            pk[q].x = pack_bf16x2(acc[4 * b + a][4 * q] + bq[q].x, acc[4 * b + a][4 * q + 1] + bq[q].y);
                            pk[q].y = pack_bf16x2(acc[4 * b + a][4 * q + 2] + bq[q].z, acc[4 * b + a][4 * q + 3] + bq[q].w);
                        }
                        if (a == 0) { *reinterpret_cast<uint2*>(V7_CELL(0)) = pk[0]; *reinterpret_cast<uint2*>(V7_CELL(1)) = pk[1]; *reinterpret_cast<uint2*>(V7_CELL(2)) = pk[2]; *reinterpret_cast<uint2*>(V7_CELL(3)) = pk[3]; }
                        if (a == 1) { *reinterpret_cast<uint2*>(V7_CELL(4)) = pk[0]; *reinterpret_cast<uint2*>(V7_CELL(5)) = pk[1]; *reinterpret_cast<uint2*>(V7_CELL(6)) = pk[2]; *reinterpret_cast<uint2*>(V7_CELL(7)) = pk[3]; }
                        if (a == 2) { *reinterpret_cast<uint2*>(V7_CELL(8)) = pk[0]; *reinterpret_cast<uint2*>(V7_CELL(9)) = pk[1]; *reinterpret_cast<uint2*>(V7_CELL(10)) = pk[2]; *reinterpret_cast<uint2*>(V7_CELL(11)) = pk[3]; }
                        if (a == 3) { *reinterpret_cast<uint2*>(V7_CELL(12)) = pk[0]; *reinterpret_cast<uint2*>(V7_CELL(13)) = pk[1]; *reinterpret_cast<uint2*>(V7_CELL(14)) = pk[2]; *reinterpret_cast<uint2*>(V7_CELL(15)) = pk[3]; }
                        __builtin_amdgcn_sched_barrier(0);
                    }
                };
                auto one_pass = [&](auto bc) {
                    constexpr int b = decltype(bc)::value;
                    uint4 v0 = *reinterpret_cast<const uint4*>(V7_ROW(0)), v1 = *reinterpret_cast<const uint4*>(V7_ROW(1)),
                          v2 = *reinterpret_cast<const uint4*>(V7_ROW(2)), v3 = *reinterpret_cast<const uint4*>(V7_ROW(3)),
                          v4 = *reinterpret_cast<const uint4*>(V7_ROW(4)), v5 = *reinterpret_cast<const uint4*>(V7_ROW(5)),
                          v6 = *reinterpret_cast<const uint4*>(V7_ROW(6)), v7 = *reinterpret_cast<const uint4*>(V7_ROW(7));
                    __builtin_amdgcn_sched_barrier(0);
                    if constexpr (RES) {
                        add_res(v0, r0); add_res(v1, r1); add_res(v2, r2); add_res(v3, r3);
                        add_res(v4, r4); add_res(v5, r5); add_res(v6, r6); add_res(v7, r7);
                        __builtin_amdgcn_sched_barrier(0);
                        if constexpr (b == 0) {
                            V7_RES_ROWS(1)
                            __builtin_amdgcn_sched_barrier(0);
                        }
                    }
                    if constexpr (b == 0) stage_pass(std::integral_constant<int, 1>{});
                    bst7(rs_out, vo, so * (8 * b + 0), v0); bst7(rs_out, vo, so * (8 * b + 1), v1);
                    bst7(rs_out, vo, so * (8 * b + 2), v2); bst7(rs_out, vo, so * (8 * b + 3), v3);
                    bst7(rs_out, vo, so * (8 * b + 4), v4); bst7(rs_out, vo, so * (8 * b + 5), v5);
                    bst7(rs_out, vo, so * (8 * b + 6), v6); bst7(rs_out, vo, so * (8 * b + 7), v7);
                    __builtin_amdgcn_sched_barrier(0);
                };
                if constexpr (RES) { V7_RES_ROWS(0) }
                __builtin_amdgcn_sched_barrier(0);
                stage_pass(std::integral_constant<int, 0>{});
                one_pass(std::integral_constant<int, 0>{});
                one_pass(std::integral_constant<int, 1>{});
#undef V7_RES_ROWS
            };
            if (p.bias) {
                if (resid) tile_epi(std::true_type{}, std::true_type{});
                else tile_epi(std::false_type{}, std::true_type{});
            } else {
                if (resid) tile_epi(std::true_type{}, std::false_type{});
                else tile_epi(std::false_type{}, std::false_type{});
            }
        } else if constexpr (IS_SWIGLU) {
            const uint32_t ab = my + (uint32_t)l31 * 128 + ((l31 & 7) << 4) + hi * 8;
            const int arow = le >> 3, ach = le & 7;
            const uint32_t arb = my + (uint32_t)arow * 128 + ((ach ^ arow) << 4);
            const int ncol = (n0 >> 1);
            const __amdgpu_buffer_rsrc_t rs_act = rsrc7(reinterpret_cast<bf16_t*>(p.Out2) + (size_t)m0 * p.ldo2 + ncol, rows_here * (uint32_t)p.ldo2 * 2u);
            const uint32_t va = ((uint32_t)arow * (uint32_t)p.ldo2 + ach * 8) * 2u;
            const uint32_t sa8 = (uint32_t)p.ldo2 * 16u;
            auto swiglu_epi = [&](auto save_c) {
                constexpr bool SAVE = decltype(save_c)::value;
                const __amdgpu_buffer_rsrc_t rs_g = rsrc7(SAVE ? reinterpret_cast<bf16_t*>(p.Out) + (size_t)m0 * p.ldo + ncol : nullptr, SAVE ? rows_here * (uint32_t)p.ldo * 2u : 0u);
                const uint32_t vg = ((uint32_t)arow * (uint32_t)p.ldo + ach * 8) * 2u;
                const uint32_t sg8 = (uint32_t)p.ldo * 16u;
                auto stage_q = [&](auto bc, auto prc, auto qc) {
                    constexpr int b = decltype(bc)::value, pr = decltype(prc)::value, q = decltype(qc)::value;
                    uint2 py, pg;
                    py.x = pack_bf16x2(acc[4 * b + 2 * pr][4 * q], acc[4 * b + 2 * pr][4 * q + 1]);
                    py.y = pack_bf16x2(acc[4 * b + 2 * pr][4 * q + 2], acc[4 * b + 2 * pr][4 * q + 3]);
                    pg.x = pack_bf16x2(acc[4 * b + 2 * pr + 1][4 * q], acc[4 * b + 2 * pr + 1][4 * q + 1]);
                    pg.y = pack_bf16x2(acc[4 * b + 2 * pr + 1][4 * q + 2], acc[4 * b + 2 * pr + 1][4 * q + 3]);
                    const float yy[4] = {bf16lo_to_f32(py.x), bf16hi_to_f32(py.x), bf16lo_to_f32(py.y), bf16hi_to_f32(py.y)};
                    const float gg[4] = {bf16lo_to_f32(pg.x), bf16hi_to_f32(pg.x), bf16lo_to_f32(pg.y), bf16hi_to_f32(pg.y)};
                    float o[4];
#pragma unroll
                    for (int e = 0; e < 4; ++e) o[e] = gg[e] * yy[e] * __builtin_amdgcn_rcpf(1.f + __expf(-gg[e]));
                    uint2 pa;
                    pa.x = pack_bf16x2(o[0], o[1]);
// ... 161 lines not shown
    }
#endif
}

template <int EPI, int DBG = 0>
hipError_t launch7(const GemmParams& p, hipStream_t stream) {
    static CxLdsOptIn lds;
    if (!lds.ensure(reinterpret_cast<const void*>(&gemm_bf16_v7_kernel<EPI, DBG>), LDS7)) return hipErrorInvalidValue;
    const int ntiles = p.tiles_m * p.tiles_n;
    const int grid = ntiles < 512 ? (ntiles + 7) / 8 * 8 : 512;
    hipLaunchKernelGGL((gemm_bf16_v7_kernel<EPI, DBG>), dim3(grid), dim3(256), LDS7, stream, p);
    return hipGetLastError();
}

int v7_groups(int tiles_m, int tiles_n, int K) {
    const double xb = (double)tiles_m * BM7 * K * 2, wb = (double)tiles_n * BN7 * K * 2;
    int best = 1;
    double best_cost = 0;
    for (int gn = 1; gn <= 8; gn *= 2) {
        const int gm = 8 / gn;
        if ((tiles_n % gn) != 0 || (tiles_m % gm) != 0) continue;
        const double slice = wb / gn;
        const double rounds = (double)tiles_m / gm * (tiles_n / gn) / 64.0;
        const double wcost = slice <= 2.5 * 1048576 ? gm * wb : (rounds < 1 ? 1 : rounds) * slice * 8;
        const double cost = gn * xb + wcost;
        if (gn == 1 || cost < best_cost) { best = gn; best_cost = cost; }
    }
    return best;
}

}

bool cx_gemm_v7_covers(const GemmParams& p, int epi) {
    if (epi != GEMM_EPI_NONE && epi != GEMM_EPI_SWIGLU_G && epi != GEMM_EPI_SWIGLU_BWD_AG) return false;
    if ((p.N % BN7) != 0 || (p.K % BK7) != 0 || p.K < 2 * BK7) return false;
    if (epi == GEMM_EPI_NONE && p.alpha != 1.f) return false;
    if ((p.N / BN7) > 256) return false;
    return true;
}

#ifndef CX_PRODUCT
static int g_v7_period = -1;
void cx_gemm_v7_set_period(int cycles) { g_v7_period = cycles; }
#else
constexpr int g_v7_period = -1;
#endif
static int v7_stagger_unit(const GemmParams& p, int epi) {
    if (g_v7_period == 0) return 0;
    if ((long)p.tiles_m * p.tiles_n < 1024) return 0;
    const int epi_cycles = epi == GEMM_EPI_SWIGLU_BWD_AG ? 24000 : epi == GEMM_EPI_SWIGLU_G ? 12000 : 9000;
    const int period = g_v7_period > 0 ? g_v7_period : (p.K / BK7) * 2400 + epi_cycles;
    return period / 64;
}

#ifndef CX_PRODUCT
static long long* g_v7_trace = nullptr;
static int g_v7_dbg = 0;
static int g_v7_flags = 1;
void cx_gemm_v7_set_flags(int f) { g_v7_flags = f; }
void cx_gemm_v7_set_trace(long long* buf) { g_v7_trace = buf; }
void cx_gemm_v7_set_ablate(int mask) { g_v7_dbg = mask; }
int cx_gemm_v7_occupancy_query(void) {
    int n = -1;
    static CxLdsOptIn lds;
    if (!lds.ensure(reinterpret_cast<const void*>(&gemm_bf16_v7_kernel<GEMM_EPI_SWIGLU_BWD_AG>), LDS7)) return -2;
    if (hipOccupancyMaxActiveBlocksPerMultiprocessor(&n, gemm_bf16_v7_kernel<GEMM_EPI_SWIGLU_BWD_AG>, 256, LDS7) != hipSuccess) return -3;
    return n;
}
#endif

hipError_t cx_launch_gemm_v7(GemmParams p, int epi, int force_gn, hipStream_t stream) {
#ifndef CX_PRODUCT
    p.trace = g_v7_trace;
    p.dbg = g_v7_flags;
#else
    p.trace = nullptr;
    p.dbg = 1;
#endif
#ifndef CX_PRODUCT
    if (g_v7_dbg) {
        p.tiles_m = (p.M + BM7 - 1) / BM7;
        p.tiles_n = p.N / BN7;
        p.sup_n = force_gn > 0 ? force_gn : v7_groups(p.tiles_m, p.tiles_n, p.K);
        p.sup_m = v7_stagger_unit(p, epi);
        const bool bwd = epi == GEMM_EPI_SWIGLU_BWD_AG;
        switch (g_v7_dbg) {
#define V7_ABL(m) case m: return bwd ? launch7<GEMM_EPI_SWIGLU_BWD_AG, m>(p, stream) : launch7<GEMM_EPI_NONE, m>(p, stream);
            V7_ABL(1) V7_ABL(2) V7_ABL(16) V7_ABL(17) V7_ABL(19) V7_ABL(64) V7_ABL(65) V7_ABL(81) V7_ABL(83) V7_ABL(87) V7_ABL(119) V7_ABL(127) V7_ABL(111)
#undef V7_ABL
            default: break;
        }
    }
#endif
    p.tiles_m = (p.M + BM7 - 1) / BM7;
    p.tiles_n = p.N / BN7;
    p.sup_n = force_gn > 0 ? force_gn : v7_groups(p.tiles_m, p.tiles_n, p.K);
    p.sup_m = v7_stagger_unit(p, epi);
    return epi == GEMM_EPI_SWIGLU_G        ? launch7<GEMM_EPI_SWIGLU_G>(p, stream)
           : epi == GEMM_EPI_SWIGLU_BWD_AG ? launch7<GEMM_EPI_SWIGLU_BWD_AG>(p, stream)
                                           : launch7<GEMM_EPI_NONE>(p, stream);
}
```

contrastors_amd/csrc/gemm_params.h:

```cpp
#pragma once
#include <hip/hip_runtime.h>
#include <stdint.h>

enum { GEMM_OUT_BF16 = 0, GEMM_OUT_F32 = 1, GEMM_OUT_F32_ATOMIC = 2, GEMM_OUT_F32_PARTIAL = 3 };
enum { GEMM_EPI_NONE = 0, GEMM_EPI_SWIGLU = 1, GEMM_EPI_GELU = 2, GEMM_EPI_SWIGLU_BWD = 3,
       GEMM_EPI_QGELU = 4,
       GEMM_EPI_SWIGLU_G = 5,
       GEMM_EPI_SWIGLU_BWD_AG = 6,
       GEMM_EPI_QACT_BWD = 8,
       GEMM_EPI_ACT_BWD = 7 };

struct GemmParams {
    const uint16_t* X;
    const uint16_t* W;
    void* Out;
    const float* bias;
    int M, N, K;
    int ldx, ldw, ldo;
    int tiles_m, tiles_n, split_k;
    float alpha;
    int dbg;
    int act;
    void* Out2;
    int ldo2;
    const uint16_t* In3;
    float* colsum_part;
    int sup_m, sup_n;
    long long* trace;
};

hipError_t cx_launch_gemm_v5(GemmParams p, int form, int out_mode, int epi, hipStream_t stream);
hipError_t cx_launch_gemm_v6(GemmParams p, int epi, hipStream_t stream);
void cx_gemm_v6_force_groups(int gn);
void cx_gemm_v6_set_trace(long long* buf);
void cx_gemm_v6_set_ablate(int mask);
hipError_t cx_launch_gemm_v6_tn(GemmParams p, hipStream_t stream);
hipError_t cx_launch_colsum_part_reduce(const float* part, float* dst, int nblocks, int N, hipStream_t stream);
bool cx_gemm_v7_covers(const GemmParams& p, int epi);
hipError_t cx_launch_gemm_v7(GemmParams p, int epi, int force_gn, hipStream_t stream);
void cx_gemm_v7_set_trace(long long* buf);
int cx_gemm_v7_occupancy_query(void);
void cx_gemm_v7_set_ablate(int mask);
void cx_gemm_v7_set_flags(int f);
void cx_gemm_v7_set_period(int cycles);
void cx_gemm_v7_set_mode(int mode);
void cx_gemm_v5_set_persistent(bool on);
void cx_gemm_v5_set_use_v6(bool on);
bool cx_gemm_v5_get_use_v6(void);
void cx_gemm_v5_set_trace(long long* buf);
```

contrastors_amd/csrc/layernorm.hip:

```cpp
#include "cx_common.h"
#include "ln_workspace.h"
#include "../../include/contrastors_hip.h"

namespace {

CX_DEVICE void unpack4_bf16(const uint2 u, float (&v)[4]) {
    v[0] = bf16lo_to_f32(u.x); v[1] = bf16hi_to_f32(u.x);
    v[2] = bf16lo_to_f32(u.y); v[3] = bf16hi_to_f32(u.y);
}
CX_DEVICE void load4_bf16(const bf16_t* p, float (&v)[4]) { unpack4_bf16(*reinterpret_cast<const uint2*>(p), v); }
CX_DEVICE uint2 store4_bf16(bf16_t* p, const float (&v)[4]) {
    uint2 u;
    u.x = pack_bf16x2(v[0], v[1]);
    u.y = pack_bf16x2(v[2], v[3]);
    *reinterpret_cast<uint2*>(p) = u;
    return u;
}
CX_DEVICE void load4_f32(const float* p, float (&v)[4]) {
    const float4 u = *reinterpret_cast<const float4*>(p);
    v[0] = u.x; v[1] = u.y; v[2] = u.z; v[3] = u.w;
}
CX_DEVICE void store4_bf16_sum(bf16_t* p, const float (&v)[4], float (&dc)[4]) {
    float r[4];
    unpack4_bf16(store4_bf16(p, v), r);
// ... 5 lines not shown
#pragma unroll
    for (int i = 0; i < N; ++i)
#pragma unroll
        for (int e = 0; e < 4; ++e) a[i][e] = 0.f;
}
template <int NCH>
CX_DEVICE void fetch_row(const bf16_t* __restrict__ base, int row, int lane, uint2 (&raw)[NCH]) {
#pragma unroll
    for (int i = 0; i < NCH; ++i)
        raw[i] = *reinterpret_cast<const uint2*>(base + (size_t)row * (NCH * 256) + (i * 64 + lane) * 4);
}

CX_DEVICE float wave_mean(float v, int d) { return wave_sum(v) / (float)d; }

template <int NCH>
CX_DEVICE void row_stats(const float (&z)[NCH][4], int d, float eps, float& mean, float& rstd) {
    float s = 0.f;
#pragma unroll
    for (int i = 0; i < NCH; ++i)
#pragma unroll
        for (int e = 0; e < 4; ++e) s += z[i][e];
    mean = wave_mean(s, d);
    float v = 0.f;
#pragma unroll
    for (int i = 0; i < NCH; ++i)
#pragma unroll
        for (int e = 0; e < 4; ++e) {
            const float c = z[i][e] - mean;
            v += c * c;
        }
    rstd = rsqrtf(wave_mean(v, d) + eps);
}

CX_DEVICE float ln_affine(float z, float mean, float rstd, float g, float b) { return (z - mean) * rstd * g + b; }
CX_DEVICE float ln_bwd_accum(float zz, float g, float dy, float mean, float rstd, float& s1, float& s2, float& dg, float& db) {
    const float xh = (zz - mean) * rstd;
    const float wdy = g * dy;
    s1 += wdy * xh;
    s2 += wdy;
    dg += dy * xh;
    db += dy;
    return xh;
}
CX_DEVICE float ln_bwd_dz(float g, float dy, float xh, float s1, float s2, float rstd) { return (g * dy - s1 * xh - s2) * rstd; }

template <int NCH>
__global__ __launch_bounds__(256) void ln_fwd_kernel(const bf16_t* __restrict__ x0, const bf16_t* __restrict__ res,
                                                     const float* __restrict__ gamma,
                                                     const float* __restrict__ beta, bf16_t* __restrict__ out,
                                                     bf16_t* z_out, float* __restrict__ mean_o,
                                                     float* __restrict__ rstd_o, int rows, float eps) {
    constexpr int D = NCH * 256;
    const int lane = threadIdx.x & 63, wave = threadIdx.x >> 6;
    float g[NCH][4], b[NCH][4];
#pragma unroll
    for (int i = 0; i < NCH; ++i) {
        load4_f32(gamma + (i * 64 + lane) * 4, g[i]);
        load4_f32(beta + (i * 64 + lane) * 4, b[i]);
    }
    const int stride = gridDim.x * 4;
    int row = blockIdx.x * 4 + wave;
    uint2 nx[NCH], nr[NCH];
    if (row < rows) {
        fetch_row<NCH>(x0, row, lane, nx);
        if (res) fetch_row<NCH>(res, row, lane, nr);
    }
    for (; row < rows; row += stride) {
// ... 988 lines not shown
```

contrastors_amd/loss.py:

```python
from __future__ import annotations

import contextlib
import logging
from typing import Dict, List, Optional

import numpy as np
import torch
import torch.distributed as dist

from . import _C
from .distributed import gather_with_grad
from .policy import GradCachePolicy
from .rand_state import RandContext


def _scale_of(logit_scale) -> tuple:
    if isinstance(logit_scale, (int, float)):
        return float(logit_scale), None
    p = getattr(logit_scale, "logit_scale", None)
    if p is None:
        raise TypeError("logit_scale must be a LogitScale module or a number")
    const = getattr(logit_scale, "_const_scale", None)
    if const is not None and not p.requires_grad:
        return float(const), None
# ... 274 lines not shown
    total = inputs["input_ids"].shape[0]
    lens = None
    mask = inputs.get("attention_mask")
    if "seqlens" in inputs:
        lens = inputs["seqlens"]
    elif mask is not None and mask.is_cuda:
        lens_t = mask.sum(-1)
        right_padded = (mask[:, 1:] <= mask[:, :-1]).all()
        host = torch.stack([lens_t.max(), right_padded.to(lens_t.dtype)]).cpu()
        lens = lens_t.cpu().numpy() if bool(host[1]) else None
    tail_seqs = max(0, min(int(tail_seqs), total))
    head = total - tail_seqs
    bounds = [(a, min(a + chunk_size, head)) for a in range(0, head, chunk_size)]
    tail = []
    e = total
    while e > head:
        tail.append((max(head, e - chunk_size), e))
        e -= chunk_size
    bounds += tail[::-1]
    chunks = []
    for a, b in bounds:
        c = {k: v[a:b] for k, v in inputs.items() if torch.is_tensor(v) and v.shape[0] == total}
        if lens is not None:
            c["seqlens"] = lens[a:b]
        chunks.append(c)
    return chunks


def _uses_rng(model) -> bool:
    trunk = getattr(model, "trunk", None)
    return bool(getattr(trunk, "uses_rng", False)) if trunk is not None else bool(getattr(model, "training", False))


def get_chunked_embeddings(model, chunks, rand_states=None, keep_tail: int = 0, kept: Optional[dict] = None):
    embs = []
    needed = rand_states is not None and _uses_rng(model)
    n = len(chunks)
    trainable = kept is not None and keep_tail > 0 and model.training and not getattr(model, "frozen_trunk", False)
    first_kept = n - keep_tail if trainable else n
    trunk = getattr(model, "trunk", None)
    for i, c in enumerate(chunks):
        if rand_states is not None:
            rand_states.append(RandContext(c, needed=needed))
        if i >= first_kept:
            suspended = (trunk.selective_checkpointing_suspended() if hasattr(trunk, "selective_checkpointing_suspended")
                         else contextlib.nullcontext())
            outstanding = getattr(trunk, "_outstanding", None)
            try:
                with torch.enable_grad(), suspended:
                    out = model(**c)["embedding"]
                kept[i] = out
                embs.append(out.detach())
                continue
            except torch.OutOfMemoryError:
                if outstanding is not None:
                    trunk._outstanding = outstanding
                first_kept = n
                if rand_states is not None:
                    rand_states[-1].restore()
                _log_once(("gradcache-tail-oom",), "GradCache: a kept chunk ran out of memory; the rest of the step re-forwards")
        with torch.no_grad():
            embs.append(model(**c)["embedding"])
    return torch.cat(embs, dim=0)


def accumulate_gradients(model, chunks, cache, rand_states=None, final: bool = False, skip=()):
    todo = [i for i in range(len(chunks)) if i not in skip]
    for i in todo:
        c, g = chunks[i], cache[i]
        state = rand_states[i] if rand_states is not None else RandContext(c, needed=False)
        if final and i == todo[-1] and hasattr(model, "arm_overlapped_reduce"):
            model.arm_overlapped_reduce()
        with state:
            out = model(**c)["embedding"]
        out.backward(g.to(out.dtype))


def cache_loss(query_embeddings, document_embeddings, logit_scale, bidirectional=False, *, use_fp8=False):
    q = query_embeddings.detach().requires_grad_()
    d = document_embeddings.detach().requires_grad_()
    loss = clip_loss(q, d, logit_scale, gather_enabled=True, bidirectional=bidirectional, use_fp8=use_fp8)
    loss.backward()
    return q.grad, d.grad, loss.detach()


_LOGGED: set = set()
LAST_SCHEDULE: dict = {}


def _log_once(key, msg: str):
    if key in _LOGGED:
        return
    _LOGGED.add(key)
    if not (dist.is_available() and dist.is_initialized()) or dist.get_rank() == 0:
        logging.getLogger("contrastors_amd").info(msg)


def effective_chunk(tower, inputs, chunk_size: int, policy: Optional[GradCachePolicy] = None) -> int:
    mode = (policy or GradCachePolicy()).with_env().chunk
    if mode == "exact" or chunk_size is None or chunk_size <= 0:
        return chunk_size
    if mode != "auto":
        return max(1, int(mode))
    cfg = getattr(getattr(tower, "trunk", None), "config", None)
    ids = inputs.get("input_ids") if isinstance(inputs, dict) else None
    if cfg is None or ids is None or ids.ndim != 2 or not ids.is_cuda:
        return chunk_size
# ... 199 lines not shown
            fell_back = True
            LAST_SCHEDULE.update(schedule="two-pass", fell_back=True)
            for tw in {id(tower1): tower1, id(tower2): tower2}.values():
                drop = getattr(getattr(tw, "trunk", None), "drop_idle_arenas", None)
                if drop is not None:
                    drop()
            torch.cuda.empty_cache()
            ids_ = t1_inputs.get("input_ids") if isinstance(t1_inputs, dict) else None
            if ids_ is not None and ids_.is_cuda:
                note_local_memory_shortfall(ids_.device, [tower1, tower2])
            _log_once(("gradcache-oom",), "GradCache: resident activations ran out of memory; falling back to the two-pass "
                                          "schedule (set train_args.gradcache_resident: false to skip the attempt)")
        else:
            try:
                q_cache, d_cache, loss = cache_loss(torch.cat([o.detach() for o in q_out]), torch.cat([o.detach() for o in d_out]),
                                                    logit_scale, bidirectional=bidirectional, use_fp8=pol.use_fp8)
            except torch.OutOfMemoryError:
                _release_resident(tower1, q_out)
                _release_resident(tower2, d_out)
                raise
            _resident_backward(tower1, q_out, q_cache.split(sizes_q), final=tower1 is not tower2 or not was_training2)
            _resident_backward(tower2, d_out, d_cache.split(sizes_d), final=True)
            del q_out, d_out
            done = True
    if not done:
        nq_keep = 0 if fell_back else (kq_seqs + cq - 1) // cq if kq_seqs else 0
        nd_keep = 0 if fell_back else (kd_seqs + cd - 1) // cd if kd_seqs else 0
        if nq_keep or nd_keep:
            _log_once(("gradcache-tail", len(q_chunks), len(d_chunks), kq_seqs, kd_seqs),
                      f"GradCache schedule: the last {kq_seqs} query and {kd_seqs} document sequences ({nq_keep} + {nd_keep} chunks of "
                      f"{len(q_chunks)} + {len(d_chunks)}) keep their activations (no re-forward for them)")
        q_rnd, d_rnd = [], []
        q_kept, d_kept = {}, {}
        try:
            q_embs = get_chunked_embeddings(tower1, q_chunks, q_rnd, keep_tail=nq_keep, kept=q_kept)
            d_embs = get_chunked_embeddings(tower2, d_chunks, d_rnd, keep_tail=nd_keep, kept=d_kept)
            q_cache, d_cache, loss = cache_loss(q_embs, d_embs, logit_scale, bidirectional=bidirectional, use_fp8=pol.use_fp8)
        except BaseException:
            _release_resident(tower1, list(q_kept.values()))
            _release_resident(tower2, list(d_kept.values()))
            raise
        q_grads, d_grads = q_cache.split(sizes_q), d_cache.split(sizes_d)
        done_q, done_d = set(q_kept), set(d_kept)
        re_q = len(done_q) < len(q_chunks)
        re_d = was_training2 and len(done_d) < len(d_chunks)
        shared = tower1 is tower2
        for i in sorted(done_q):
            o = q_kept.pop(i)
            last_of_tower1 = not re_q and not q_kept and (not shared or (not done_d and not re_d))
            if last_of_tower1 and hasattr(tower1, "arm_overlapped_reduce"):
                tower1.arm_overlapped_reduce()
            o.backward(q_grads[i].to(o.dtype))
        for i in sorted(done_d):
            o = d_kept.pop(i)
            last_of_tower2 = not re_d and not d_kept and not (shared and re_q)
            if last_of_tower2 and hasattr(tower2, "arm_overlapped_reduce"):
                tower2.arm_overlapped_reduce()
            o.backward(d_grads[i].to(o.dtype))
        if re_q:
            accumulate_gradients(tower1, q_chunks, q_grads, q_rnd, final=(not shared) or not re_d, skip=done_q)
        if re_d:
            accumulate_gradients(tower2, d_chunks, d_grads, d_rnd, final=True, skip=done_d)
    seen = set()
    for tw, active in ((tower1, was_training1), (tower2, was_training2)):
        if active and id(tw) not in seen and hasattr(tw, "sync_gradients"):
            seen.add(id(tw))
            tw.sync_gradients()
    return loss


def _release_resident(tower, outs):
    if not outs:
        return
    for o in outs:
        fn = getattr(o, "grad_fn", None)
        eng, arena = getattr(fn, "engine", None), getattr(fn, "arena", None)
        if eng is not None and arena is not None and hasattr(eng, "abandon_arena"):
            eng.abandon_arena(arena)
            fn.arena = None
```

contrastors_amd/nomic_bert.py:

```python
from __future__ import annotations

import contextlib
import ctypes as C
import logging
import math
import os
from dataclasses import dataclass
from typing import Dict, List, Optional, Tuple, Union

import numpy as np
import torch
import torch.distributed as dist

from . import _C
from .policy import _parse_keep


@dataclass
class NomicBertConfig:

    vocab_size: int = 30528
    n_positions: int = 2048
    n_embd: int = 768
    n_layer: int = 12
# ... 132 lines not shown
            if not with_backward:
                t["yg_wide"] = torch.empty(T_cap, 2 * I, **bf)
        ws_floats = max(8 * max(3 * d, wfc1, patch_dim) * d, 16 * d * d)
        if with_backward and wfc1 == I:
            ws_floats = max(ws_floats, ((T_cap + 127) // 128) * I)
        t["ws_f32"] = torch.empty(ws_floats, **f32)
        if with_backward:
            wide = max(3 * d, wfc1, patch_dim)
            for n in ("g_a", "g_b", "g_c"):
                t[n] = torch.empty(T_cap, d, **bf)
            t["g_wide"] = torch.empty(T_cap, wide, **bf)
            t["g_act"] = torch.empty(T_cap, I, **bf)
            if any(f % 256 for f in (d, 3 * d, I, wfc1) + ((patch_dim,) if patch_dim else ())):
                t["tr_a"] = torch.empty(wide, T_cap, **bf)
                t["tr_b"] = torch.empty(wide, T_cap, **bf)
            t["delta"] = torch.empty(T_cap * H, **f32)
            if getattr(cfg, "resid_pdrop", 0.0) > 0:
                t["g_d"] = torch.empty(T_cap, d, **bf)
        self.tensors = t
        self.desc = _C.CxChunkBuffers()
        self.desc.T_cap = T_cap
        for name, _ in _C.CxChunkBuffers._fields_[1:]:
            if name == "ws_floats":
                self.desc.ws_floats = t["ws_f32"].numel() if "ws_f32" in t else 0
            elif name == "checkpoint":
                self.desc.checkpoint = int(self.checkpoint)
            elif name == "ckpt_keep":
                self.desc.ckpt_keep = int(self.keep_layers)
            elif name in ("drop_active", "drop_seed", "drop_offset", "n_keep", "n_patch_all"):
                setattr(self.desc, name, 0)
            else:
                setattr(self.desc, name, t[name].data_ptr() if name in t else None)
        self.emb_out: Optional[torch.Tensor] = None

    def nbytes(self) -> int:
        return sum(x.numel() * x.element_size() for x in self.tensors.values())

    @staticmethod
    def slot_bytes_per_token(cfg) -> int:
        d, I, H = cfg.n_embd, cfg.n_inner, cfg.n_head
        extra = 2 * I + 4 * 2 if getattr(cfg, "norm_mlp", False) else 0
        return 2 * (3 * d + d + 3 * d + I + I) + 4 * (H + 4) + extra


_FULL_CACHE: Dict[tuple, tuple] = {}


@dataclass
class VarlenBatch:

    input_ids: torch.Tensor
    indices: torch.Tensor
    cu_seqlens: torch.Tensor
    B: int
    S: int
    T: int
    max_seqlen: int
    _sort: Optional[tuple] = None
    token_type_ids: Optional[torch.Tensor] = None

    def with_token_types(self, token_type_ids: Optional[torch.Tensor]) -> "VarlenBatch":
        if token_type_ids is not None:
            if token_type_ids.shape != self.input_ids.shape or token_type_ids.dtype != torch.int64 \
                    or token_type_ids.device != self.input_ids.device:
                raise ValueError("token_type_ids must be an int64 tensor of input_ids' shape on its device")
            token_type_ids = token_type_ids.contiguous()
        self.token_type_ids = token_type_ids
        return self

    def embedding_sort(self):
        if self._sort is None:
            import os

            if os.environ.get("CX_EMBED_ATOMICS"):
                self._sort = (None, None)
                return self._sort
            tok = self.input_ids.reshape(-1)[self.indices.long()].to(torch.int32)
            sorted_ids, perm = torch.sort(tok, stable=True)
# ... 52 lines not shown
        self.normalize_default = bool(normalize)
        decay, nodecay = self._param_specs()
        self._layout: Dict[str, Tuple[int, Tuple[int, ...]]] = {}
        off = 0
        for name, shape in decay:
            self._layout[name] = (off, shape)
            off += _round_up(int(np.prod(shape)), 64)
        self.n_decay = off
        for name, shape in nodecay:
            self._layout[name] = (off, shape)
            off += _round_up(int(np.prod(shape)), 64)
        self.n_total = off
        self._linear_names = [n for n, s in decay if self._is_linear(n)]
        self._lin_begin = self._layout[self._linear_names[0]][0]
        self._lin_end = self.n_decay

        dev = self.device_
        self.flat_param = torch.zeros(self.n_total, dtype=torch.float32, device=dev)
        self.flat_grad = torch.zeros(self.n_total, dtype=torch.float32, device=dev)
        self.flat_decay = torch.nn.Parameter(self.flat_param[: self.n_decay])
        self.flat_nodecay = torch.nn.Parameter(self.flat_param[self.n_decay:])
        self.flat_decay.grad = self.flat_grad[: self.n_decay]
        self.flat_nodecay.grad = self.flat_grad[self.n_decay:]
        n_lin = self._lin_end - self._lin_begin
        self.w16 = torch.zeros(n_lin, dtype=torch.bfloat16, device=dev)
        self.w16_t = torch.zeros(n_lin, dtype=torch.bfloat16, device=dev)

        self._init_weights(seed)
        self._build_rotary()
        self._build_desc()
        self._arena_nograd: Optional[_ChunkArena] = None
        self._arena_free: List[_ChunkArena] = []
        self._outstanding = 0
        self._overlap_armed = None
        self._ov_works = None
        self.gradient_checkpointing = False
        self.checkpoint_keep: Union[int, str] = 0
        self._keep_logged: set = set()
        self._keep_suspended = 0
        self._keep_plan: Dict[int, int] = {}
        self._keep_granted: Dict[int, int] = {}
        self._keep_granted_B: Dict[int, int] = {}
        self._arena_tick = 0
        self.sync_shadows()

    _LAYER_PREFIX = "encoder.layers.{l}."

    def _layer_specs(self, l: int):
        cfg = self.config
        d, I = cfg.n_embd, cfg.n_inner
        wfc1 = 2 * I if cfg.gated else I
        p = self._LAYER_PREFIX.format(l=l)
        decay = [(p + "attn.Wqkv.weight", (3 * d, d)), (p + "attn.out_proj.weight", (d, d)),
                 (p + "mlp.fc1_fused.weight", (wfc1, d)), (p + "mlp.fc2.weight", (d, I))]
        nodecay = []
        if cfg.qkv_proj_bias:
            nodecay += [(p + "attn.Wqkv.bias", (3 * d,)), (p + "attn.out_proj.bias", (d,))]
        if cfg.mlp_fc1_bias:
            nodecay.append((p + "mlp.fc1_fused.bias", (wfc1,)))
        if cfg.mlp_fc2_bias:
            nodecay.append((p + "mlp.fc2.bias", (d,)))
        nodecay += [(p + "norm1.weight", (d,)), (p + "norm1.bias", (d,)),
                    (p + "norm2.weight", (d,)), (p + "norm2.bias", (d,))]
        return decay, nodecay

    def _param_specs(self):
# ... 71 lines not shown

    def reference_grad_dict(self) -> Dict[str, torch.Tensor]:
        return self._export(self.g)

    @torch.no_grad()
    def load_reference_state_dict(self, sd: Dict[str, torch.Tensor], strict: bool = True):
        I = self.config.n_inner
        missing = []
        for name in self._layout:
            dst = self.p(name)
            if ".mlp.fc1_fused." in name and self.config.gated:
                k1, k2 = name.replace("fc1_fused", "fc11"), name.replace("fc1_fused", "fc12")
                if k1 not in sd or k2 not in sd:
                    missing.append(k1)
                    continue
                v = dst.view(I // 32, 2, 32, *dst.shape[1:])
                v[:, 0].copy_(sd[k1].to(device=dst.device, dtype=torch.float32).view(I // 32, 32, *dst.shape[1:]))
                v[:, 1].copy_(sd[k2].to(device=dst.device, dtype=torch.float32).view(I // 32, 32, *dst.shape[1:]))
                continue
            key = name.replace("fc1_fused", "fc1")
            if key not in sd:
                missing.append(key)
                continue
            src = sd[key]
            if tuple(src.shape) != tuple(dst.shape):
                raise ValueError(f"{key}: shape {tuple(src.shape)} != {tuple(dst.shape)}")
            dst.copy_(src.to(device=dst.device, dtype=torch.float32))
        if strict and missing:
            raise KeyError(f"missing keys: {missing[:5]}...")
        self.sync_shadows()

    @torch.no_grad()
    def sync_shadows(self):
        s = _C.cur_stream()
        n = self._lin_end - self._lin_begin
        _C.check(self.lib.cx_cast_f32_to_bf16(self.flat_param.data_ptr() + 4 * self._lin_begin, self.w16.data_ptr(),
                                               n, s), "cast")
        jobs = getattr(self, "_cast_jobs", None)
        if jobs is not None and (jobs[3] != self.flat_param.data_ptr() or jobs[4] != self.w16_t.data_ptr()):
            jobs = None
        if jobs is None:
            tab = np.zeros(len(self._linear_names), dtype=np.dtype([("in", "u8"), ("out", "u8"), ("rows", "i4"), ("cols", "i4")]))
            tiles = 0
            for i, name in enumerate(self._linear_names):
                off, shape = self._layout[name]
                tab[i] = (self.flat_param.data_ptr() + 4 * off, self._w16(name, True).data_ptr(), shape[0], shape[1])
                tiles = max(tiles, ((shape[0] + 63) // 64) * ((shape[1] + 63) // 64))
            dev_tab = torch.from_numpy(tab.view(np.uint8).copy()).to(self.device_)
            jobs = self._cast_jobs = (dev_tab, len(self._linear_names), tiles, self.flat_param.data_ptr(), self.w16_t.data_ptr())
        _C.check(self.lib.cx_cast_transpose_f32_to_bf16_batched(jobs[0].data_ptr(), jobs[1], jobs[2], s), "cast_transpose")

    def zero_grad(self, set_to_none: bool = False):
        self.flat_grad.zero_()

    def _build_rotary(self):
        cfg = self.config
        self.rot_cos = self.rot_sin = None
        self._rot_len = 0
        if cfg.rotary_emb_fraction > 0:
            self._inv_freq = self._rot_inv_freq(cfg.rotary_emb_base)
            self._rot_tables(0 if cfg.rotary_scaling_factor else cfg.n_positions)

    @staticmethod
    def _rot_inv_freq(base: float) -> torch.Tensor:
        dim = 64
        return 1.0 / (base ** (torch.arange(0, dim, 2, dtype=torch.float32) / dim))
# ... 257 lines not shown
            self._ov_ranges = self.grad_ranges()
        return self._ov_events

    def _launch_overlapped_reduce(self):
        ev = self._ov_events
        per_layer, tail = self._ov_ranges
        works = []
        with torch.cuda.stream(self._ov_stream):
            for l in range(self.config.n_layer - 1, -1, -1):
                self._ov_stream.wait_event(ev[l])
                for a, b in per_layer[l]:
                    works.append(dist.all_reduce(self.flat_grad[a:b], op=dist.ReduceOp.SUM, async_op=True))
            self._ov_stream.wait_event(ev[self.config.n_layer])
            for a, b in tail:
                works.append(dist.all_reduce(self.flat_grad[a:b], op=dist.ReduceOp.SUM, async_op=True))
        self._ov_works = works

    def finish_overlapped_reduce(self) -> bool:
        works = getattr(self, "_ov_works", None)
        if not works:
            return False
        for w in works:
            w.wait()
        torch.cuda.current_stream(self.device_).wait_stream(self._ov_stream)
        self._ov_works = None
        return True

    def gradient_checkpointing_enable(self, enabled: bool = True, keep_layers: Union[int, str, None] = None):
        self.gradient_checkpointing = bool(enabled)
        if keep_layers is not None:
            self.checkpoint_keep = parse_checkpoint_keep(keep_layers, "checkpoint_keep_layers")
        self._arena_free = []

    def forward_chunk(self, vb: VarlenBatch, save_for_backward: bool, normalize: Optional[bool] = None,
                      out: Optional[torch.Tensor] = None) -> Tuple[torch.Tensor, Optional[_ChunkArena]]:
        d = self.config.n_embd
        if self.config.rotary_emb_fraction > 0 and self.config.rotary_scaling_factor:
            self._update_rotary(vb.max_seqlen)
        elif vb.S > (self.config.n_positions if self.rot_cos is not None else self.config.max_position_embeddings):
            raise ValueError("sequence longer than the position table")
        if out is None:
            out = torch.empty(vb.B, d, dtype=torch.float32, device=self.device_)
        arena = self._get_arena(vb.T, vb.B, save_for_backward)
        self._arm_dropout(arena)
        self._desc.normalize = int(self.normalize_default if normalize is None else normalize)
        if vb.token_type_ids is None:
            rc = self.lib.cx_encoder_forward(C.byref(self._desc), C.byref(arena.desc), vb.input_ids.data_ptr(),
                                             vb.indices.data_ptr(), vb.cu_seqlens.data_ptr(), vb.B, vb.S, vb.T,
                                             vb.max_seqlen, int(save_for_backward), out.data_ptr(), _C.cur_stream())
            _C.check(rc, "cx_encoder_forward")
        else:
            self._check_token_types()
            rc = self.lib.cx_encoder_forward_typed(C.byref(self._desc), C.byref(arena.desc), vb.input_ids.data_ptr(),
                                                   vb.token_type_ids.data_ptr(), vb.indices.data_ptr(),
                                                   vb.cu_seqlens.data_ptr(), vb.B, vb.S, vb.T, vb.max_seqlen,
                                                   int(save_for_backward), out.data_ptr(), _C.cur_stream())
            _C.check(rc, "cx_encoder_forward_typed")
        if save_for_backward:
            arena.emb_out = out
            arena.normalize = self._desc.normalize
            self._outstanding += 1
            return out, arena
        return out, None

    def _check_token_types(self):
        if self.config.type_vocab_size != 2:
            raise NotImplementedError(f"token_type_ids need type_vocab_size == 2 (the config has {self.config.type_vocab_size})")

    def drop_idle_arenas(self):
        for a in self._arena_free:
            self._keep_plan.pop(a.T_cap, None)
        self._arena_free = []
        self._arena_nograd = None
        torch.cuda.empty_cache()

    def backward_chunk(self, vb: VarlenBatch, arena: _ChunkArena, demb: torch.Tensor):
        assert arena.emb_out is not None, "backward_chunk needs a forward with save_for_backward=True"
        demb = demb.to(torch.float32).contiguous()
        self._desc.normalize = arena.normalize
        sids, perm = vb.embedding_sort()
        fires = self._begin_backward(arena)
        if vb.token_type_ids is None:
            rc = self.lib.cx_encoder_backward(C.byref(self._desc), C.byref(arena.desc), vb.input_ids.data_ptr(),
                                              vb.indices.data_ptr(), vb.cu_seqlens.data_ptr(), vb.B, vb.S, vb.T,
                                              vb.max_seqlen, demb.data_ptr(), arena.emb_out.data_ptr(), _C.ptr(sids),
                                              _C.ptr(perm), _C.cur_stream())
            _C.check(rc, "cx_encoder_backward")
        else:
            rc = self.lib.cx_encoder_backward_typed(C.byref(self._desc), C.byref(arena.desc), vb.input_ids.data_ptr(),
                                                    vb.token_type_ids.data_ptr(), vb.indices.data_ptr(),
                                                    vb.cu_seqlens.data_ptr(), vb.B, vb.S, vb.T, vb.max_seqlen,
                                                    demb.data_ptr(), arena.emb_out.data_ptr(), _C.ptr(sids), _C.ptr(perm),
                                                    _C.cur_stream())
            _C.check(rc, "cx_encoder_backward_typed")
        self._end_backward(arena, fires)

    def _begin_backward(self, arena: _ChunkArena) -> bool:
        fires = self._overlap_fires()
        if fires:
            self._overlap_events()
            arena.desc.layer_events = C.cast(self._ov_handles, C.POINTER(C.c_void_p))
        return fires

    def _end_backward(self, arena: _ChunkArena, fires: bool):
        self._outstanding = max(0, self._outstanding - 1)
        if fires:
            self._launch_overlapped_reduce()
        self.release_arena(arena)

    def _rotary_or_bounds(self, vb: VarlenBatch):
        if self.config.rotary_emb_fraction > 0 and self.config.rotary_scaling_factor:
            self._update_rotary(vb.max_seqlen)
        elif vb.S > (self.config.n_positions if self.rot_cos is not None else self.config.max_position_embeddings):
            raise ValueError("sequence longer than the position table")

# ... 66 lines not shown
```

include/contrastors_hip.h:

```cpp
#ifndef CONTRASTORS_HIP_H
#define CONTRASTORS_HIP_H

#include <stdint.h>

#ifdef __cplusplus
extern "C" {
#endif

#define CX_OK 0
#define CX_ERR_SHAPE (-1)
#define CX_ERR_ALIGN (-2)
#define CX_ERR_ARG (-3)
#define CX_ERR_LAUNCH (-4)

int cx_abi_version(void);
const char* cx_build_info(void);
const char* cx_error_string(int code);

int cx_gemm_bf16_nt(const uint16_t* X, const uint16_t* W, void* Out, const float* bias, int M, int N, int K, int ldx,
                    int ldw, int ldo, int out_mode, int split_k, float alpha, void* stream);
int cx_gemm_bf16_nt_accum(const uint16_t* X, const uint16_t* W, float* Out, float* ws, long ws_floats, int M, int N,
                          int K, int ldx, int ldw, void* stream);
int cx_gemm_bf16_tn_accum(const uint16_t* dY, const uint16_t* A, float* G, float* ws, long ws_floats, int T, int O, int I,
                          int ld_dy, int ld_a, void* stream);
// ... 54 lines not shown
                    const float* pos_emb, const float* gamma, const float* beta, uint16_t* out, float* mean,
                    float* rstd, int T, int S, int d, float eps, void* stream);
int cx_embed_ln_bwd(const uint16_t* dout_a, const uint16_t* dout_b, const int64_t* input_ids,
                    const int32_t* indices, const float* word, const float* type0, const float* pos_emb,
                    const float* gamma, const float* mean, const float* rstd, float* dword, float* dtype0,
                    float* dpos, float* dgamma, float* dbeta, int T, int S, int d, int padding_idx, void* stream);

int cx_embed_ln_bwd_sorted(const uint16_t* dout_a, const uint16_t* dout_b, const int64_t* input_ids,
                           const int32_t* indices, const float* word, const float* type0, const float* pos_emb,
                           const float* gamma, const float* mean, const float* rstd, float* dword, float* dtype0,
                           float* dpos, float* dgamma, float* dbeta, int T, int S, int d, int padding_idx, int vocab,
                           const int32_t* sorted_ids, const int32_t* perm, float* dz_scratch, void* stream);

int cx_embed_ln_fwd_typed(const int64_t* input_ids, const int64_t* token_type_ids, const int32_t* indices, const float* word,
                          const float* type, int type_vocab_size, const float* pos_emb, const float* gamma, const float* beta,
                          uint16_t* out, float* mean, float* rstd, int T, int S, int d, float eps, void* stream);
int cx_embed_ln_bwd_typed(const uint16_t* dout_a, const uint16_t* dout_b, const int64_t* input_ids,
                          const int64_t* token_type_ids, const int32_t* indices, const float* word, const float* type,
                          int type_vocab_size, const float* pos_emb, const float* gamma, const float* mean, const float* rstd,
                          float* dword, float* dtype, float* dpos, float* dgamma, float* dbeta, float* ws, long ws_floats, int T,
                          int S, int d, int padding_idx, void* stream);
int cx_embed_ln_bwd_sorted_typed(const uint16_t* dout_a, const uint16_t* dout_b, const int64_t* input_ids,
                                 const int64_t* token_type_ids, const int32_t* indices, const float* word, const float* type,
                                 int type_vocab_size, const float* pos_emb, const float* gamma, const float* mean,
                                 const float* rstd, float* dword, float* dtype, float* dpos, float* dgamma, float* dbeta,
                                 float* ws, long ws_floats, int T, int S, int d, int padding_idx, int vocab,
                                 const int32_t* sorted_ids, const int32_t* perm, float* dz_scratch, void* stream);

int cx_swiglu_fwd(const uint16_t* yg, uint16_t* act, int T, int I, int layout, void* stream);
int cx_swiglu_bwd(const uint16_t* dact, const uint16_t* yg, uint16_t* dyg, int T, int I, int layout, void* stream);
int cx_gemm_bf16_nt_residual(const uint16_t* X, const uint16_t* W, uint16_t* Out, const float* bias,
                             const uint16_t* Residual, int M, int N, int K, int ldx, int ldw, int ldo, int ldr,
                             void* stream);
int cx_gemm_bf16_nt_splitk(const uint16_t* X, const uint16_t* W, uint16_t* Out, const float* bias, const uint16_t* Residual,
                           float* ws, long ws_floats, int M, int N, int K, int ldx, int ldw, int ldo, int ldr, void* stream);
int cx_gemm_bf16_swiglu(const uint16_t* X, const uint16_t* W, uint16_t* YG, uint16_t* Act, int M, int I, int K, int ldx,
                        int ldw, int ld_yg, int ld_act, void* stream);
int cx_gemm_bf16_bias_gelu(const uint16_t* X, const uint16_t* W, const float* bias, uint16_t* Pre, uint16_t* Act, int M,
                           int N, int K, int ldx, int ldw, int ld_pre, int ld_act, void* stream);
int cx_gemm_bf16_bias_act(const uint16_t* X, const uint16_t* W, const float* bias, uint16_t* Pre, uint16_t* Act, int M,
                          int N, int K, int ldx, int ldw, int ld_pre, int ld_act, int act, void* stream);
int cx_gemm_bf16_act_bwd(const uint16_t* dY, const uint16_t* W, const uint16_t* Pre, uint16_t* dPre, float* dbias, float* ws,
                         long ws_floats, int M, int N, int K, int ldx, int ldw, int ld_pre, int ld_dpre, int act, void* stream);
int cx_gemm_bf16_swiglu_bwd(const uint16_t* dY, const uint16_t* W, const uint16_t* YG, uint16_t* dYG, int M, int I, int K,
                            int ldx, int ldw, int ld_yg, void* stream);
int cx_gemm_bf16_swiglu_gate(const uint16_t* X, const uint16_t* W, uint16_t* G, uint16_t* Act, int M, int I, int K, int ldx,
                             int ldw, int ld_g, int ld_act, void* stream);
int cx_gemm_bf16_swiglu_bwd_gate(const uint16_t* dY, const uint16_t* W, const uint16_t* Act, const uint16_t* G, uint16_t* dYG,
                                 int M, int I, int K, int ldx, int ldw, int ld_ag, int ld_dyg, void* stream);
int cx_swiglu_bwd_gate(const uint16_t* dact, const uint16_t* act, const uint16_t* gate, uint16_t* dyg, int T, int I,
                       void* stream);
int cx_bias_gelu_fwd(const uint16_t* pre, const float* bias, uint16_t* act, int T, int I, void* stream);
int cx_bias_gelu_bwd(const uint16_t* dact, const uint16_t* pre, const float* bias, uint16_t* dpre, int T, int I,
                     void* stream);
int cx_bias_gelu_bwd_colsum(const uint16_t* dact, const uint16_t* pre, const float* bias, uint16_t* dpre, float* dbias, int T,
                            int I, void* stream);
int cx_bias_act_fwd(const uint16_t* pre, const float* bias, uint16_t* act_out, int T, int I, int act, void* stream);
int cx_bias_act_bwd_colsum(const uint16_t* dact, const uint16_t* pre, const float* bias, uint16_t* dpre, float* dbias, int T,
                           int I, int act, void* stream);
int cx_bias_grad(const uint16_t* dY, float* dbias, int T, int N, int ld, void* stream);

int cx_attn_varlen_fwd(const uint16_t* qkv, const int32_t* cu_seqlens, const float* rot_cos, const float* rot_sin,
                       uint16_t* out, float* lse, int B, int H, int T, int max_seqlen, float softmax_scale,
                       void* stream);
int cx_attn_varlen_bwd(const uint16_t* dout, const uint16_t* qkv, const uint16_t* out, const float* lse,
                       const int32_t* cu_seqlens, const float* rot_cos, const float* rot_sin, float* delta,
// ... 147 lines not shown
    float* delta;
    float* ws_f32;
    long ws_floats;
    uint16_t* zf; uint16_t* hf; float* meanf; float* rstdf;
    uint16_t* patch_in; uint16_t* patch_proj;
    int checkpoint;
    int drop_active;
    unsigned long long drop_seed, drop_offset;
    uint16_t* g_d;
    void* const* layer_events;
    uint16_t* zpre;
    int ckpt_keep;
    const int32_t* patch_keep;
    const int32_t* patch_inv;
    int n_keep;
    int n_patch_all;
} CxChunkBuffers;

int cx_encoder_forward(const CxEncoderDesc* enc, const CxChunkBuffers* buf, const int64_t* input_ids,
                       const int32_t* indices, const int32_t* cu_seqlens, int Bc, int S, int T, int max_seqlen,
                       int save_for_backward, float* emb_out, void* stream);
int cx_encoder_backward(const CxEncoderDesc* enc, const CxChunkBuffers* buf, const int64_t* input_ids,
                        const int32_t* indices, const int32_t* cu_seqlens, int Bc, int S, int T, int max_seqlen,
                        const float* demb, const float* emb_out, const int32_t* sort_ids, const int32_t* sort_perm,
                        void* stream);

int cx_encoder_forward_typed(const CxEncoderDesc* enc, const CxChunkBuffers* buf, const int64_t* input_ids,
                             const int64_t* token_type_ids, const int32_t* indices, const int32_t* cu_seqlens, int Bc, int S,
                             int T, int max_seqlen, int save_for_backward, float* emb_out, void* stream);
int cx_encoder_backward_typed(const CxEncoderDesc* enc, const CxChunkBuffers* buf, const int64_t* input_ids,
                              const int64_t* token_type_ids, const int32_t* indices, const int32_t* cu_seqlens, int Bc, int S,
                              int T, int max_seqlen, const float* demb, const float* emb_out, const int32_t* sort_ids,
                              const int32_t* sort_perm, void* stream);

int cx_encoder_forward_hidden(const CxEncoderDesc* enc, const CxChunkBuffers* buf, const int64_t* input_ids,
                              const int32_t* indices, const int32_t* cu_seqlens, int Bc, int S, int T, int max_seqlen,
                              int save_for_backward, uint16_t* hidden_out, void* stream);
int cx_encoder_backward_hidden(const CxEncoderDesc* enc, const CxChunkBuffers* buf, const int64_t* input_ids,
                               const int32_t* indices, const int32_t* cu_seqlens, int Bc, int S, int T, int max_seqlen,
                               const uint16_t* dhidden, const int32_t* sort_ids, const int32_t* sort_perm, void* stream);

int cx_vit_patchify(const void* pixels, int pixels_bf16, uint16_t* patches, int B, int C, int H, int W, int patch,
                    void* stream);
int cx_vit_assemble_fwd(const uint16_t* proj, const float* cls_token, const float* pos_embed, uint16_t* out, int B,
                        int P, int d, void* stream);
int cx_vit_assemble_bwd(const uint16_t* dz, uint16_t* dproj, float* gcls, float* gpos, int B, int P, int d,
                        void* stream);
int cx_vit_patchify_gather(const void* pixels, int pixels_bf16, uint16_t* patches, int B, int C, int H, int W, int patch,
                           const int32_t* keep, int n_keep, void* stream);
int cx_vit_assemble_fwd_gather(const uint16_t* proj, const float* cls_token, const float* pos_embed, uint16_t* out, int B,
                               int P, int d, const int32_t* keep, void* stream);
int cx_vit_assemble_bwd_gather(const uint16_t* dz, uint16_t* dproj, float* gcls, float* gpos, int B, int P, int d,
                               const int32_t* inv, int P_all, void* stream);
int cx_vit_forward(const CxEncoderDesc* enc, const CxChunkBuffers* buf, const void* pixels, int pixels_bf16,
                   const int32_t* cu_seqlens, int Bc, int C, int H, int W, int patch, int save_for_backward,
                   float* emb_out, void* stream);
int cx_vit_backward(const CxEncoderDesc* enc, const CxChunkBuffers* buf, const int32_t* cu_seqlens, int Bc,
                    int n_patch, const float* demb, const float* emb_out, void* stream);
int cx_vit_forward_hidden(const CxEncoderDesc* enc, const CxChunkBuffers* buf, const void* pixels, int pixels_bf16,
                          const int32_t* cu_seqlens, int Bc, int Cc, int H, int W, int patch, int save_for_backward,
                          uint16_t* hidden_out, void* stream);
int cx_vit_backward_hidden(const CxEncoderDesc* enc, const CxChunkBuffers* buf, const int32_t* cu_seqlens, int Bc, int n_patch,
                           const uint16_t* dhidden, void* stream);

int cx_rope2d_qkv_inplace(uint16_t* qkv, const int32_t* cu_seqlens, const float* rope_cos, const float* rope_sin, int n_rope,
                          int B, int n_head, int T, int n_prefix, int sign, void* stream);
// ... 61 lines not shown
```

Before: 4395.

## Capture LayerNorm stats in no-grad pass and fuse LN into residual GEMM on replay

During the no-grad embedding pass (as in GradCache-style contrastive training), per-layer LayerNorm mean/rstd are captured. On the later re-forward with grad, they are replayed so the output-projection GEMM epilogue applies the residual add and LayerNorm affine directly, skipping separate LayerNorm kernels. Stats are also reused across recomputation under checkpointing for backward. This relies on identical inputs and weights between passes (guarded by a weights epoch and by disabling when RNG/dropout is used) and adds stats memory plus device copies when activations are kept.

```diff
diff --git a/contrastors_amd/_C.py b/contrastors_amd/_C.py
--- a/contrastors_amd/_C.py
+++ b/contrastors_amd/_C.py
@@ -108,6 +108,7 @@
     "cx_swiglu_bwd": (i32, [vp, vp, vp, i32, i32, i32, vp]),
     "cx_gemm_bf16_swiglu": (i32, [vp, vp, vp, vp, i32, i32, i32, i32, i32, i32, i32, vp]),
     "cx_gemm_bf16_nt_residual": (i32, [vp, vp, vp, vp, vp, i32, i32, i32, i32, i32, i32, i32, vp]),
+    "cx_gemm_bf16_nt_residual_ln": (i32, [vp] * 10 + [i32, i32, i32, i32, i32, i32, i32, i32, vp]),
     "cx_gemm_bf16_swiglu_bwd": (i32, [vp, vp, vp, vp, i32, i32, i32, i32, i32, i32, vp]),
     "cx_gemm_bf16_nt_splitk": (i32, [vp, vp, vp, vp, vp, vp, i64, i32, i32, i32, i32, i32, i32, i32, vp]),
     "cx_gemm_bf16_swiglu_gate": (i32, [vp, vp, vp, vp, i32, i32, i32, i32, i32, i32, i32, vp]),
@@ -203,6 +204,10 @@
                                        i32, i32, vp, vp]),
     "cx_encoder_backward_typed": (i32, [C.POINTER(CxEncoderDesc), C.POINTER(CxChunkBuffers), vp, vp, vp, vp, i32, i32, i32,
                                         i32, vp, vp, vp, vp, vp]),
+    "cx_encoder_forward_stats": (i32, [C.POINTER(CxEncoderDesc), C.POINTER(CxChunkBuffers), vp, vp, vp, vp, i32, i32, i32,
+                                       i32, i32, vp, vp, i64, i32, vp]),
+    "cx_encoder_backward_stats": (i32, [C.POINTER(CxEncoderDesc), C.POINTER(CxChunkBuffers), vp, vp, vp, vp, i32, i32, i32,
+                                        i32, vp, vp, vp, vp, vp, i64, vp]),
     "cx_encoder_forward_hidden": (i32, [C.POINTER(CxEncoderDesc), C.POINTER(CxChunkBuffers), vp, vp, vp, i32, i32, i32,
                                         i32, i32, vp, vp]),
     "cx_encoder_backward_hidden": (i32, [C.POINTER(CxEncoderDesc), C.POINTER(CxChunkBuffers), vp, vp, vp, i32, i32, i32,
diff --git a/contrastors_amd/csrc/cx_common.h b/contrastors_amd/csrc/cx_common.h
--- a/contrastors_amd/csrc/cx_common.h
+++ b/contrastors_amd/csrc/cx_common.h
@@ -70,6 +70,18 @@
     dy = g * s * d;
     const cx_f2 w = cx_f2{rcp_clamped(g.x), rcp_clamped(g.y)} + 1.f - s;
     dg = (d * act) * w;
+}
+
+CX_DEVICE float ln_affine(float z, float mean, float rstd, float g, float b) { return (z - mean) * rstd * g + b; }
+CX_DEVICE cx_f2 ln_affine2(cx_f2 z, float mean, float rstd, cx_f2 g, cx_f2 b) { return (z - mean) * rstd * g + b; }
+CX_DEVICE uint4 ln_affine8(const uint4& z, float mean, float rstd, const float (&g)[8], const float (&b)[8]) {
+    float f[8];
+    unpack8(z, f);
+    const cx_f2 o0 = ln_affine2(cx_f2{f[0], f[1]}, mean, rstd, cx_f2{g[0], g[1]}, cx_f2{b[0], b[1]});
+    const cx_f2 o1 = ln_affine2(cx_f2{f[2], f[3]}, mean, rstd, cx_f2{g[2], g[3]}, cx_f2{b[2], b[3]});
+    const cx_f2 o2 = ln_affine2(cx_f2{f[4], f[5]}, mean, rstd, cx_f2{g[4], g[5]}, cx_f2{b[4], b[5]});
+    const cx_f2 o3 = ln_affine2(cx_f2{f[6], f[7]}, mean, rstd, cx_f2{g[6], g[7]}, cx_f2{b[6], b[7]});
+    return make_uint4(pack_bf16x2(o0.x, o0.y), pack_bf16x2(o1.x, o1.y), pack_bf16x2(o2.x, o2.y), pack_bf16x2(o3.x, o3.y));
 }
 
 CX_DEVICE float gelu_cdf(float v, float& gauss) {
diff --git a/contrastors_amd/csrc/engine.hip b/contrastors_amd/csrc/engine.hip
--- a/contrastors_amd/csrc/engine.hip
+++ b/contrastors_amd/csrc/engine.hip
@@ -96,10 +96,27 @@
     return cx_gemm_bf16_nt_accum(b->tr_a, b->tr_b, gW, b->ws_f32, b->ws_floats, out_f, in_f, Tp, Tp, Tp, stream);
 }
 
+struct LnApply {
+    const float* mean;
+    const float* rstd;
+    const float* gamma;
+    const float* beta;
+    uint16_t* h;
+    bool applied;
+};
 int proj_residual(const uint16_t* x, const uint16_t* W, const float* bias, const uint16_t* residual, uint16_t* out, int T,
-                  int N, int K, bool* folded, void* stream, const CxChunkBuffers* buf = nullptr) {
+                  int N, int K, bool* folded, void* stream, const CxChunkBuffers* buf = nullptr, LnApply* ln = nullptr) {
     *folded = false;
-    if (buf && buf->ws_f32 && (long)((T + 255) / 256) * ((N + 255) / 256) <= 64 && K >= 1536) {
+    const bool splitk_case = buf && buf->ws_f32 && (long)((T + 255) / 256) * ((N + 255) / 256) <= 64 && K >= 1536;
+    if (ln && residual && !splitk_case) {
+        const int rc = cx_gemm_bf16_nt_residual_ln(x, W, out, ln->h, bias, residual, ln->mean, ln->rstd, ln->gamma, ln->beta, T, N, K,
+                                                   K, K, N, N, N, stream);
+        if (rc != CX_ERR_SHAPE) {
+            *folded = ln->applied = rc == CX_OK;
+            return rc;
+        }
+    }
+    if (splitk_case) {
         const int rc = cx_gemm_bf16_nt_splitk(x, W, out, bias, residual, buf->ws_f32, buf->ws_floats, T, N, K, K, K, N, N, stream);
         if (rc != CX_ERR_SHAPE) {
             *folded = residual != nullptr && rc == CX_OK;
@@ -119,6 +136,12 @@
 bool gelu_fused_shape(int T, int N, int K) {
     return T > 0 && (K % 64) == 0 && (N % 8) == 0;
 }
+
+struct LnStats {
+    float* p;
+    long ld;
+    bool valid;
+};
 
 struct BlockRunner {
     const CxEncoderDesc* enc;
@@ -128,6 +151,13 @@
     int Bc, T, max_seqlen;
     void* stream;
     const CxVitExt* ext = nullptr;
+    const LnStats* stats = nullptr;
+    float* st(int l, int ln, int which) const { return stats->p + (((size_t)l * 2 + ln) * 2 + which) * stats->ld; }
+    int copy_stats(int l, int ln, float* mean, float* rstd) const {
+        const size_t n = (size_t)T * sizeof(float);
+        return (hipMemcpyAsync(mean, st(l, ln, 0), n, hipMemcpyDeviceToDevice, (hipStream_t)stream) == hipSuccess &&
+                hipMemcpyAsync(rstd, st(l, ln, 1), n, hipMemcpyDeviceToDevice, (hipStream_t)stream) == hipSuccess) ? CX_OK : CX_ERR_LAUNCH;
+    }
 
     int mlp_up(const CxLayerWeights& w, const uint16_t* x, int l, bool keep) const {
         const int d = enc->d, I = enc->d_inner;
@@ -148,11 +178,12 @@
         return cx_bias_act_fwd(s.yg(l), w.bfc1, s.act(l), T, I, enc->mlp_act, stream);
     }
     int mlp(const CxLayerWeights& w, const uint16_t* x, int l, uint16_t* out, const uint16_t* residual, bool keep,
-            bool* folded) const {
+            bool* folded, LnApply* ln = nullptr) const {
         CX_TRY(mlp_up(w, x, l, keep));
-        return proj_residual(ext_subln(ext) ? s.ez(ext, l) : s.act(l), w.Wfc2, w.bfc2, residual, out, T, enc->d, enc->d_inner, folded, stream, buf);
-    }
-    int attn(const CxLayerWeights& w, const uint16_t* x, int l, uint16_t* out, const uint16_t* residual, bool* folded) const {
+        return proj_residual(ext_subln(ext) ? s.ez(ext, l) : s.act(l), w.Wfc2, w.bfc2, residual, out, T, enc->d, enc->d_inner, folded, stream, buf, ln);
+    }
+    int attn(const CxLayerWeights& w, const uint16_t* x, int l, uint16_t* out, const uint16_t* residual, bool* folded,
+             LnApply* ln = nullptr) const {
         const int d = enc->d;
         CX_TRY(cx_gemm_bf16_nt(x, w.Wqkv, s.qkv(l), w.bqkv, T, 3 * d, d, d, d, 3 * d, 0, 1, 1.f, stream));
         if (ext_rope(ext))
@@ -171,7 +202,7 @@
             CX_TRY(cx_attn_varlen_fwd(s.qkv(l), cu_seqlens, enc->rot_cos, enc->rot_sin, s.ctx(l), s.lse(l), Bc, enc->n_head, T,
                                       max_seqlen, enc->softmax_scale, stream));
         }
-        return proj_residual(s.ctx(l), w.Wout, w.bout, residual, out, T, d, d, folded, stream);
+        return proj_residual(s.ctx(l), w.Wout, w.bout, residual, out, T, d, d, folded, stream, nullptr, ln);
     }
     int post_block(int l, const uint16_t* h_in, bool keep) const {
         const CxLayerWeights& w = enc->layers[l];
@@ -187,12 +218,23 @@
                                                 s.rstd2(l), T, d, enc->ln_eps, p, buf->drop_seed, buf->drop_offset, 2 * l + 1,
                                                 stream);
         }
-        CX_TRY(attn(w, h_in, l, s.z1(l), h_in, &f1));
-        CX_TRY(cx_layernorm_fwd(s.z1(l), f1 ? nullptr : h_in, w.ln1_g, w.ln1_b, s.h1(l), (keep && !f1) ? s.z1(l) : nullptr,
-                                s.mean1(l), s.rstd1(l), T, d, enc->ln_eps, stream));
-        CX_TRY(mlp(w, s.h1(l), l, s.z2(l), s.h1(l), keep, &f2));
+        const bool replay = stats && stats->valid, capture = stats && !stats->valid && !keep;
+        LnApply a1{}, a2{};
+        if (replay) {
+            a1 = LnApply{st(l, 0, 0), st(l, 0, 1), w.ln1_g, w.ln1_b, s.h1(l), false};
+            a2 = LnApply{st(l, 1, 0), st(l, 1, 1), w.ln2_g, w.ln2_b, s.h2(l), false};
+        }
+        CX_TRY(attn(w, h_in, l, s.z1(l), h_in, &f1, replay ? &a1 : nullptr));
+        if (a1.applied) {
+            if (keep) CX_TRY(copy_stats(l, 0, s.mean1(l), s.rstd1(l)));
+        } else {
+            CX_TRY(cx_layernorm_fwd(s.z1(l), f1 ? nullptr : h_in, w.ln1_g, w.ln1_b, s.h1(l), (keep && !f1) ? s.z1(l) : nullptr,
+                                    capture ? st(l, 0, 0) : s.mean1(l), capture ? st(l, 0, 1) : s.rstd1(l), T, d, enc->ln_eps, stream));
+        }
+        CX_TRY(mlp(w, s.h1(l), l, s.z2(l), s.h1(l), keep, &f2, replay ? &a2 : nullptr));
+        if (a2.applied) return keep ? copy_stats(l, 1, s.mean2(l), s.rstd2(l)) : CX_OK;
         return cx_layernorm_fwd(s.z2(l), f2 ? nullptr : s.h1(l), w.ln2_g, w.ln2_b, s.h2(l), (keep && !f2) ? s.z2(l) : nullptr,
-                                s.mean2(l), s.rstd2(l), T, d, enc->ln_eps, stream);
+                                capture ? st(l, 1, 0) : s.mean2(l), capture ? st(l, 1, 1) : s.rstd2(l), T, d, enc->ln_eps, stream);
     }
     bool drop() const { return buf->drop_active && enc->resid_pdrop > 0.f; }
     int pre_block(int l, const uint16_t* x, const uint16_t* r, bool r_folded, bool keep, bool up_only, const uint16_t** x_out,
@@ -217,9 +259,9 @@
 
 int blocks_forward(const CxEncoderDesc* enc, const CxChunkBuffers* buf, const Slots& s, const uint16_t* h0,
                    const int32_t* cu_seqlens, int Bc, int T, int max_seqlen, int save, const uint16_t** h_final,
-                   void* stream, const CxVitExt* ext = nullptr) {
+                   void* stream, const CxVitExt* ext = nullptr, const LnStats* stats = nullptr) {
     const int d = enc->d, L = enc->n_layer;
-    const BlockRunner run{enc, buf, s, cu_seqlens, Bc, T, max_seqlen, stream, ext};
+    const BlockRunner run{enc, buf, s, cu_seqlens, Bc, T, max_seqlen, stream, ext, stats};
     if (!enc->prenorm) {
         const uint16_t* h_in = h0;
         for (int l = 0; l < L; ++l) {
@@ -289,7 +331,7 @@
 
 int blocks_backward(const CxEncoderDesc* enc, const CxChunkBuffers* buf, const Slots& s, const int32_t* cu_seqlens, int Bc,
                     int T, int max_seqlen, const PooledGrad* pg, const uint16_t** da_out, const uint16_t** db_out, void* stream,
-                    const CxVitExt* ext = nullptr) {
+                    const CxVitExt* ext = nullptr, const LnStats* stats = nullptr) {
     const int d = enc->d, I = enc->d_inner, H = enc->n_head, L = enc->n_layer;
     auto mlp_bwd = [&](const CxLayerWeights& w, int l, const uint16_t* dm, const uint16_t* mlp_in, const uint16_t* add,
                        bool* folded, bool bias_done) -> int {
@@ -358,7 +400,7 @@
         return cx_layernorm_bwd_colsum(a, b2, z, g, mean, rstd, dz_extra, dz, gg, gb, *done ? gbias : nullptr, buf->ws_f32,
                                        buf->ws_floats, T, d, stream);
     };
-    const BlockRunner run{enc, buf, s, cu_seqlens, Bc, T, max_seqlen, stream, ext};
+    const BlockRunner run{enc, buf, s, cu_seqlens, Bc, T, max_seqlen, stream, ext, stats};
     if (!enc->prenorm) {
         const uint16_t* da = buf->g_a;
         const uint16_t* db = nullptr;
@@ -549,9 +591,10 @@
 
 int text_forward_impl(const CxEncoderDesc* enc, const CxChunkBuffers* buf, const int64_t* input_ids,
                       const int64_t* token_type_ids, const int32_t* indices, const int32_t* cu_seqlens, int Bc, int S, int T,
-                      int max_seqlen, int save_for_backward, float* emb_out, void* stream) {
+                      int max_seqlen, int save_for_backward, float* emb_out, void* stream, const LnStats* stats = nullptr) {
     if (Bc <= 0 || T <= 0) return CX_OK;
     CX_TRY(check_desc(enc, buf, T));
+    if (stats && (!stats->p || stats->ld < T || enc->prenorm)) return CX_ERR_ARG;
     (void)hipGetLastError();
     const int d = enc->d, I = enc->d_inner;
     const Slots s = make_slots(enc, buf, save_for_backward);
@@ -565,7 +608,7 @@
     if (buf->drop_active && enc->embd_pdrop > 0.f)
         CX_TRY(cx_dropout_scale(buf->h0, (long)T * d, enc->embd_pdrop, buf->drop_seed, buf->drop_offset, 2 * enc->n_layer, stream));
     const uint16_t* h_final = nullptr;
-    CX_TRY(blocks_forward(enc, buf, s, buf->h0, cu_seqlens, Bc, T, max_seqlen, s.mode, &h_final, stream));
+    CX_TRY(blocks_forward(enc, buf, s, buf->h0, cu_seqlens, Bc, T, max_seqlen, s.mode, &h_final, stream, nullptr, stats));
     return cx_pool_normalize_fwd(h_final, cu_seqlens, emb_out, buf->pool_norm, Bc, d, enc->pool_mode, enc->normalize,
                                  stream);
 }
@@ -573,10 +616,11 @@
 int text_backward_impl(const CxEncoderDesc* enc, const CxChunkBuffers* buf, const int64_t* input_ids,
                        const int64_t* token_type_ids, const int32_t* indices, const int32_t* cu_seqlens, int Bc, int S, int T,
                        int max_seqlen, const float* demb, const float* emb_out, const int32_t* sort_ids,
-                       const int32_t* sort_perm, void* stream) {
+                       const int32_t* sort_perm, void* stream, const LnStats* stats = nullptr) {
     if (Bc <= 0 || T <= 0) return CX_OK;
     CX_TRY(check_desc(enc, buf, T));
     if (!demb || !emb_out) return CX_ERR_ARG;
+    if (stats && (!stats->p || stats->ld < T || enc->prenorm)) return CX_ERR_ARG;
     CX_TRY(check_bwd_buffers(buf));
     (void)hipGetLastError();
     const int d = enc->d, I = enc->d_inner;
@@ -589,7 +633,7 @@
                                      enc->normalize, stream));
     const uint16_t* da = fold_pool ? nullptr : buf->g_a;
     const uint16_t* db = nullptr;
-    CX_TRY(blocks_backward(enc, buf, s, cu_seqlens, Bc, T, max_seqlen, fold_pool ? &pg : nullptr, &da, &db, stream));
+    CX_TRY(blocks_backward(enc, buf, s, cu_seqlens, Bc, T, max_seqlen, fold_pool ? &pg : nullptr, &da, &db, stream, nullptr, stats));
     if (buf->drop_active && enc->embd_pdrop > 0.f) {
         CX_TRY(cx_dropout_scale(const_cast<uint16_t*>(da), (long)T * d, enc->embd_pdrop, buf->drop_seed, buf->drop_offset,
                                 2 * enc->n_layer, stream));
@@ -650,6 +694,23 @@
                               const int32_t* sort_perm, void* stream) {
     return text_backward_impl(enc, buf, input_ids, token_type_ids, indices, cu_seqlens, Bc, S, T, max_seqlen, demb, emb_out,
                               sort_ids, sort_perm, stream);
+}
+
+int cx_encoder_forward_stats(const CxEncoderDesc* enc, const CxChunkBuffers* buf, const int64_t* input_ids,
+                             const int64_t* token_type_ids, const int32_t* indices, const int32_t* cu_seqlens, int Bc, int S,
+                             int T, int max_seqlen, int save_for_backward, float* emb_out, float* ln_stats, long stats_ld,
+                             int stats_valid, void* stream) {
+    const LnStats st{ln_stats, stats_ld, stats_valid != 0};
+    return text_forward_impl(enc, buf, input_ids, token_type_ids, indices, cu_seqlens, Bc, S, T, max_seqlen, save_for_backward,
+                             emb_out, stream, ln_stats ? &st : nullptr);
+}
+int cx_encoder_backward_stats(const CxEncoderDesc* enc, const CxChunkBuffers* buf, const int64_t* input_ids,
+                              const int64_t* token_type_ids, const int32_t* indices, const int32_t* cu_seqlens, int Bc, int S,
+                              int T, int max_seqlen, const float* demb, const float* emb_out, const int32_t* sort_ids,
+                              const int32_t* sort_perm, const float* ln_stats, long stats_ld, void* stream) {
+    const LnStats st{const_cast<float*>(ln_stats), stats_ld, true};
+    return text_backward_impl(enc, buf, input_ids, token_type_ids, indices, cu_seqlens, Bc, S, T, max_seqlen, demb, emb_out,
+                              sort_ids, sort_perm, stream, ln_stats ? &st : nullptr);
 }
 
 int cx_encoder_forward_hidden(const CxEncoderDesc* enc, const CxChunkBuffers* buf, const int64_t* input_ids,
diff --git a/contrastors_amd/csrc/gemm_api.hip b/contrastors_amd/csrc/gemm_api.hip
--- a/contrastors_amd/csrc/gemm_api.hip
+++ b/contrastors_amd/csrc/gemm_api.hip
@@ -189,6 +189,22 @@
     return cx_launch_gemm_v6(p, GEMM_EPI_NONE, (hipStream_t)stream) == hipSuccess ? CX_OK : CX_ERR_LAUNCH;
 }
 
+int cx_gemm_bf16_nt_residual_ln(const uint16_t* X, const uint16_t* W, uint16_t* Z, uint16_t* H, const float* bias,
+                                const uint16_t* Residual, const float* mean, const float* rstd, const float* gamma,
+                                const float* beta, int M, int N, int K, int ldx, int ldw, int ldz, int ldr, int ldh, void* stream) {
+    if (M <= 0 || N <= 0) return CX_OK;
+    if (!Residual || !Z || !H || !mean || !rstd || !gamma || !beta) return CX_ERR_ARG;
+    if (N != 256 && N != 512 && N != 768 && N != 1024) return CX_ERR_SHAPE;
+    if (K <= 0 || (K % 64) != 0 || (ldz % 8) != 0 || (ldr % 8) != 0 || (ldh % 8) != 0) return CX_ERR_SHAPE;
+    if ((ldx % 8) != 0 || (ldw % 8) != 0 || ((uintptr_t)gamma % 16) != 0 || ((uintptr_t)beta % 16) != 0) return CX_ERR_ALIGN;
+    GemmParams p = base_params(X, W, Z, bias, M, N, K, ldx, ldw, ldz);
+    p.Out2 = const_cast<uint16_t*>(Residual); p.ldo2 = ldr;
+    p.Out3 = H; p.ldo3 = ldh;
+    p.ln_mean = mean; p.ln_rstd = rstd; p.ln_gamma = gamma; p.ln_beta = beta;
+    ProfScope prof(2.0 * (double)M * (double)N * (double)K, (hipStream_t)stream);
+    return cx_launch_gemm_v6(p, GEMM_EPI_RESID_LN, (hipStream_t)stream) == hipSuccess ? CX_OK : CX_ERR_LAUNCH;
+}
+
 int cx_gemm_bf16_bias_gelu(const uint16_t* X, const uint16_t* W, const float* bias, uint16_t* Pre, uint16_t* Act, int M, int N,
                            int K, int ldx, int ldw, int ld_pre, int ld_act, void* stream) {
     return cx_gemm_bf16_bias_act(X, W, bias, Pre, Act, M, N, K, ldx, ldw, ld_pre, ld_act, 0, stream);
diff --git a/contrastors_amd/csrc/gemm_bf16.hip b/contrastors_amd/csrc/gemm_bf16.hip
--- a/contrastors_amd/csrc/gemm_bf16.hip
+++ b/contrastors_amd/csrc/gemm_bf16.hip
@@ -821,6 +821,25 @@
     return e == hipSuccess ? CX_OK : CX_ERR_LAUNCH;
 }
 
+int cx_gemm_bf16_nt_residual_ln(const uint16_t* X, const uint16_t* W, uint16_t* Z, uint16_t* H, const float* bias,
+                                const uint16_t* Residual, const float* mean, const float* rstd, const float* gamma,
+                                const float* beta, int M, int N, int K, int ldx, int ldw, int ldz, int ldr, int ldh, void* stream) {
+    if (M <= 0 || N <= 0) return CX_OK;
+    if (!Residual || !Z || !H || !mean || !rstd || !gamma || !beta) return CX_ERR_ARG;
+    if (N != 256 && N != 512 && N != 768 && N != 1024) return CX_ERR_SHAPE;
+    if (K <= 0 || (K % 64) != 0 || (ldz % 8) != 0 || (ldr % 8) != 0 || (ldh % 8) != 0) return CX_ERR_SHAPE;
+    if ((ldx % 8) != 0 || (ldw % 8) != 0 || ((uintptr_t)gamma % 16) != 0 || ((uintptr_t)beta % 16) != 0) return CX_ERR_ALIGN;
+    if (cx_gemm_get_variant() != 6) return CX_ERR_SHAPE;
+    GemmParams p = {};
+    p.X = X; p.W = W; p.Out = Z; p.bias = bias;
+    p.M = M; p.N = N; p.K = K; p.ldx = ldx; p.ldw = ldw; p.ldo = ldz;
+    p.split_k = 1; p.alpha = 1.f; p.dbg = g_dbg;
+    p.Out2 = const_cast<uint16_t*>(Residual); p.ldo2 = ldr;
+    p.Out3 = H; p.ldo3 = ldh;
+    p.ln_mean = mean; p.ln_rstd = rstd; p.ln_gamma = gamma; p.ln_beta = beta;
+    return cx_launch_gemm_v6(p, GEMM_EPI_RESID_LN, (hipStream_t)stream) == hipSuccess ? CX_OK : CX_ERR_LAUNCH;
+}
+
 int cx_gemm_bf16_bias_gelu(const uint16_t* X, const uint16_t* W, const float* bias, uint16_t* Pre, uint16_t* Act, int M,
                            int N, int K, int ldx, int ldw, int ld_pre, int ld_act, void* stream) {
     return cx_gemm_bf16_bias_act(X, W, bias, Pre, Act, M, N, K, ldx, ldw, ld_pre, ld_act, 0, stream);
diff --git a/contrastors_amd/csrc/gemm_bf16_v6.hip b/contrastors_amd/csrc/gemm_bf16_v6.hip
--- a/contrastors_amd/csrc/gemm_bf16_v6.hip
+++ b/contrastors_amd/csrc/gemm_bf16_v6.hip
@@ -308,8 +308,10 @@
             auto pcol = [&](int q) { return (q & 1) * 16 + 4 * g4; };
             auto qoff = [](int q, int rowb) { return (q >> 1) * 16 * rowb + (q & 1) * 32; };
             if constexpr ((DBG & 16) != 0) {
-            } else if constexpr (EPI == GEMM_EPI_NONE || EPI == GEMM_EPI_ACT_BWD || EPI == GEMM_EPI_QACT_BWD) {
+            } else if constexpr (EPI == GEMM_EPI_NONE || EPI == GEMM_EPI_ACT_BWD || EPI == GEMM_EPI_QACT_BWD || EPI == GEMM_EPI_RESID_LN) {
                 constexpr bool ACTB = EPI == GEMM_EPI_ACT_BWD || EPI == GEMM_EPI_QACT_BWD;
+                constexpr bool LNF = EPI == GEMM_EPI_RESID_LN;
+                constexpr int LN_OFF = 32 * ROWB;
                 float cs0 = 0.f, cs1 = 0.f, cs2 = 0.f, cs3 = 0.f, cs4 = 0.f, cs5 = 0.f, cs6 = 0.f, cs7 = 0.f;
                 constexpr int act_kind = EPI == GEMM_EPI_QACT_BWD ? CX_ACT_QUICK_GELU : CX_ACT_GELU;
                 auto mul_grad = [&](uint4& v, const uint4& r) {
@@ -349,6 +351,15 @@
                     const bf16_t* resp = RES ? resid + (size_t)(m0 + rrow) * p.ldo2 + n0 + rch * 8 : nullptr;
                     const char* rd = my + rrow * ROWB + rch * 16;
                     char* wr = my + prow(0) * ROWB + pcol(0) * 2;
+                    bf16_t* hp = LNF ? reinterpret_cast<bf16_t*>(p.Out3) + (size_t)(m0 + rrow) * p.ldo3 + n0 + rch * 8 : nullptr;
+                    float2 sg = {}, sb = {}, sm0 = {}, sm1 = {};
+                    if constexpr (LNF) {
+                        sg = *reinterpret_cast<const float2*>(p.ln_gamma + n0 + 2 * lane);
+                        sb = *reinterpret_cast<const float2*>(p.ln_beta + n0 + 2 * lane);
+                        sm0 = make_float2(p.ln_mean[m0 + lane], p.ln_rstd[m0 + lane]);
+                        sm1 = make_float2(p.ln_mean[m0 + 64 + lane], p.ln_rstd[m0 + 64 + lane]);
+                        __builtin_amdgcn_sched_barrier(0);
+                    }
                     uint2 pk[16];
                     auto pack_pass = [&](int b) {
 #pragma unroll
@@ -419,10 +430,43 @@
                         gst(o + (size_t)20 * p.ldo, v5);
                         gst(o + (size_t)24 * p.ldo, v6);
                         gst(o + (size_t)28 * p.ldo, v7);
+                        if constexpr (LNF) {
+                            __builtin_amdgcn_sched_barrier(0);
+                            const char* st = my + LN_OFF;
+                            const float4 ga = *reinterpret_cast<const float4*>(st + rch * 32), gb = *reinterpret_cast<const float4*>(st + rch * 32 + 16);
+                            const float4 ba = *reinterpret_cast<const float4*>(st + 512 + rch * 32), bb = *reinterpret_cast<const float4*>(st + 512 + rch * 32 + 16);
+                            const char* ms = st + 1024 + (b * 32 + rrow) * 8;
+                            const float2 s0 = *reinterpret_cast<const float2*>(ms), s1 = *reinterpret_cast<const float2*>(ms + 4 * 8),
+                                         s2 = *reinterpret_cast<const float2*>(ms + 8 * 8), s3 = *reinterpret_cast<const float2*>(ms + 12 * 8),
+                                         s4 = *reinterpret_cast<const float2*>(ms + 16 * 8), s5 = *reinterpret_cast<const float2*>(ms + 20 * 8),
+                                         s6 = *reinterpret_cast<const float2*>(ms + 24 * 8), s7 = *reinterpret_cast<const float2*>(ms + 28 * 8);
+                            __builtin_amdgcn_sched_barrier(0);
+                            const float gam[8] = {ga.x, ga.y, ga.z, ga.w, gb.x, gb.y, gb.z, gb.w};
+                            const float bet[8] = {ba.x, ba.y, ba.z, ba.w, bb.x, bb.y, bb.z, bb.w};
+                            bf16_t* oh = hp + (size_t)(b * 32) * p.ldo3;
+                            gst(oh, ln_affine8(v0, s0.x, s0.y, gam, bet));
+                            gst(oh + (size_t)4 * p.ldo3, ln_affine8(v1, s1.x, s1.y, gam, bet));
+                            gst(oh + (size_t)8 * p.ldo3, ln_affine8(v2, s2.x, s2.y, gam, bet));
+                            gst(oh + (size_t)12 * p.ldo3, ln_affine8(v3, s3.x, s3.y, gam, bet));
+                            gst(oh + (size_t)16 * p.ldo3, ln_affine8(v4, s4.x, s4.y, gam, bet));
+                            gst(oh + (size_t)20 * p.ldo3, ln_affine8(v5, s5.x, s5.y, gam, bet));
+                            gst(oh + (size_t)24 * p.ldo3, ln_affine8(v6, s6.x, s6.y, gam, bet));
+                            gst(oh + (size_t)28 * p.ldo3, ln_affine8(v7, s7.x, s7.y, gam, bet));
+                            __builtin_amdgcn_sched_barrier(0);
+                        }
                     };
                     if constexpr (RES) { CX_RES_ROWS(0) }
                     pack_pass(0);
                     stage();
+                    if constexpr (LNF) {
+                        __builtin_amdgcn_sched_barrier(0);
+                        char* st = my + LN_OFF;
+                        *reinterpret_cast<float2*>(st + lane * 8) = sg;
+                        *reinterpret_cast<float2*>(st + 512 + lane * 8) = sb;
+                        *reinterpret_cast<float2*>(st + 1024 + lane * 8) = sm0;
+                        *reinterpret_cast<float2*>(st + 1536 + lane * 8) = sm1;
+                        __builtin_amdgcn_sched_barrier(0);
+                    }
                     one_pass(std::integral_constant<int, 0>{});
                     one_pass(std::integral_constant<int, 1>{});
                     one_pass(std::integral_constant<int, 2>{});
@@ -547,6 +591,14 @@
                             }
                             if (m < p.M && n + 8 <= p.N)
                                 gst(reinterpret_cast<bf16_t*>(p.Out) + (size_t)m * p.ldo + n, vv);
+                            if constexpr (LNF) {
+                                if (m < p.M && n + 8 <= p.N) {
+                                    float gam[8], bet[8];
+                                    load8_f32(p.ln_gamma + n, gam);
+                                    load8_f32(p.ln_beta + n, bet);
+                                    gst(reinterpret_cast<bf16_t*>(p.Out3) + (size_t)m * p.ldo3 + n, ln_affine8(vv, p.ln_mean[m], p.ln_rstd[m], gam, bet));
+                                }
+                            }
                         }
                     }
                 };
@@ -557,6 +609,12 @@
                         store_tile(std::true_type{});
                     }
                     flush_colsum();
+                } else if constexpr (LNF) {
+                    if (fast) {
+                        fast_tile(std::true_type{});
+                    } else {
+                        store_tile(std::false_type{});
+                    }
                 } else if (fast) {
                     if (resid) {
                         fast_tile(std::true_type{});
@@ -1420,6 +1478,7 @@
            : epi == GEMM_EPI_GELU ? launch6<GEMM_EPI_GELU>(p, stream)
            : epi == GEMM_EPI_QGELU ? launch6<GEMM_EPI_QGELU>(p, stream)
            : epi == GEMM_EPI_SWIGLU_BWD ? launch6<GEMM_EPI_SWIGLU_BWD>(p, stream)
+           : epi == GEMM_EPI_RESID_LN ? launch6<GEMM_EPI_RESID_LN>(p, stream)
            : epi == GEMM_EPI_ACT_BWD ? (p.act == CX_ACT_QUICK_GELU ? launch6<GEMM_EPI_QACT_BWD>(p, stream) : launch6<GEMM_EPI_ACT_BWD>(p, stream))
                                   : launch6<GEMM_EPI_NONE>(p, stream);
 }
diff --git a/contrastors_amd/csrc/gemm_bf16_v7.hip b/contrastors_amd/csrc/gemm_bf16_v7.hip
--- a/contrastors_amd/csrc/gemm_bf16_v7.hip
+++ b/contrastors_amd/csrc/gemm_bf16_v7.hip
@@ -69,7 +69,8 @@
     extern __shared__ __attribute__((aligned(16))) char dsm[];
     constexpr bool IS_BWD = EPI == GEMM_EPI_SWIGLU_BWD_AG;
     constexpr bool IS_SWIGLU = EPI == GEMM_EPI_SWIGLU_G;
-    static_assert(EPI == GEMM_EPI_NONE || IS_BWD || IS_SWIGLU, "v7 serves the plain / residual, SwiGLU (gate save) and SwiGLU-backward (act, gate) forms");
+    constexpr bool LNF = EPI == GEMM_EPI_RESID_LN;
+    static_assert(EPI == GEMM_EPI_NONE || LNF || IS_BWD || IS_SWIGLU, "v7 serves the plain / residual (+ LayerNorm apply), SwiGLU (gate save) and SwiGLU-backward (act, gate) forms");
     const int tid = threadIdx.x;
     const int lane = tid & 63;
     const int wave = __builtin_amdgcn_readfirstlane(tid >> 6);
@@ -309,7 +310,7 @@
 #define V7_CELL(c) (dsm + vxor7<((c) << 4)>(cb))
 #define V7_ROW(i) (dsm + vxor7<(((i) & 3) << 6)>(rb) + 1024 * (i))
         if constexpr ((DBG & 16) != 0) {
-        } else if constexpr (EPI == GEMM_EPI_NONE) {
+        } else if constexpr (EPI == GEMM_EPI_NONE || LNF) {
             const bf16_t* resid = reinterpret_cast<const bf16_t*>(p.Out2);
             const __amdgpu_buffer_rsrc_t rs_out = rsrc7(reinterpret_cast<bf16_t*>(p.Out) + (size_t)m0 * p.ldo + n0, rows_here * (uint32_t)p.ldo * 2u);
             const uint32_t vo = ((uint32_t)lrow * (uint32_t)p.ldo + lch * 8) * 2u;
@@ -376,6 +377,28 @@
                     bst7(rs_out, vo, so * (8 * b + 4), v4); bst7(rs_out, vo, so * (8 * b + 5), v5);
                     bst7(rs_out, vo, so * (8 * b + 6), v6); bst7(rs_out, vo, so * (8 * b + 7), v7);
                     __builtin_amdgcn_sched_barrier(0);
+                    if constexpr (LNF) {
+                        const __amdgpu_buffer_rsrc_t rs_h = rsrc7(reinterpret_cast<bf16_t*>(p.Out3) + (size_t)m0 * p.ldo3 + n0, rows_here * (uint32_t)p.ldo3 * 2u);
+                        const __amdgpu_buffer_rsrc_t rs_g = rsrc7(p.ln_gamma + n0, (uint32_t)BN7 * 4u), rs_b = rsrc7(p.ln_beta + n0, (uint32_t)BN7 * 4u);
+                        const __amdgpu_buffer_rsrc_t rs_mu = rsrc7(p.ln_mean + m0, rows_here * 4u), rs_rs = rsrc7(p.ln_rstd + m0, rows_here * 4u);
+                        const uint32_t vh = ((uint32_t)lrow * (uint32_t)p.ldo3 + lch * 8) * 2u;
+                        const uint32_t sh = (uint32_t)p.ldo3 * 8u;
+                        const float4 ga = bldf7(rs_g, (uint32_t)lch * 32u, 0u), gb = bldf7(rs_g, (uint32_t)lch * 32u, 16u);
+                        const float4 ba = bldf7(rs_b, (uint32_t)lch * 32u, 0u), bb = bldf7(rs_b, (uint32_t)lch * 32u, 16u);
+                        const float gam[8] = {ga.x, ga.y, ga.z, ga.w, gb.x, gb.y, gb.z, gb.w};
+                        const float bet[8] = {ba.x, ba.y, ba.z, ba.w, bb.x, bb.y, bb.z, bb.w};
+#define V7_LN_ROW(i_, v_)                                                                                                            \
+    {                                                                                                                               \
+        const float mu_ = __uint_as_float(__builtin_amdgcn_raw_buffer_load_b32(rs_mu, (uint32_t)lrow * 4u, (uint32_t)(32 * b + 4 * (i_)) * 4u, 0)); \
+        const float rs_ = __uint_as_float(__builtin_amdgcn_raw_buffer_load_b32(rs_rs, (uint32_t)lrow * 4u, (uint32_t)(32 * b + 4 * (i_)) * 4u, 0)); \
+        bst7(rs_h, vh, sh * (8 * b + (i_)), ln_affine8(v_, mu_, rs_, gam, bet));                                                     \
+    }
+                        V7_LN_ROW(0, v0) V7_LN_ROW(1, v1) V7_LN_ROW(2, v2) V7_LN_ROW(3, v3)
+                        V7_LN_ROW(4, v4) V7_LN_ROW(5, v5) V7_LN_ROW(6, v6) V7_LN_ROW(7, v7)
+#undef V7_LN_ROW
+                        asm volatile("s_nop 1" ::: "memory");
+                        __builtin_amdgcn_sched_barrier(0);
+                    }
                 };
                 if constexpr (RES) { V7_RES_ROWS(0) }
                 __builtin_amdgcn_sched_barrier(0);
@@ -384,7 +407,10 @@
                 one_pass(std::integral_constant<int, 1>{});
 #undef V7_RES_ROWS
             };
-            if (p.bias) {
+            if constexpr (LNF) {
+                if (p.bias) tile_epi(std::true_type{}, std::true_type{});
+                else tile_epi(std::true_type{}, std::false_type{});
+            } else if (p.bias) {
                 if (resid) tile_epi(std::true_type{}, std::true_type{});
                 else tile_epi(std::false_type{}, std::true_type{});
             } else {
@@ -612,9 +638,9 @@
 }
 
 bool cx_gemm_v7_covers(const GemmParams& p, int epi) {
-    if (epi != GEMM_EPI_NONE && epi != GEMM_EPI_SWIGLU_G && epi != GEMM_EPI_SWIGLU_BWD_AG) return false;
+    if (epi != GEMM_EPI_NONE && epi != GEMM_EPI_RESID_LN && epi != GEMM_EPI_SWIGLU_G && epi != GEMM_EPI_SWIGLU_BWD_AG) return false;
     if ((p.N % BN7) != 0 || (p.K % BK7) != 0 || p.K < 2 * BK7) return false;
-    if (epi == GEMM_EPI_NONE && p.alpha != 1.f) return false;
+    if ((epi == GEMM_EPI_NONE || epi == GEMM_EPI_RESID_LN) && p.alpha != 1.f) return false;
     if ((p.N / BN7) > 256) return false;
     return true;
 }
@@ -658,7 +684,7 @@
     p.dbg = 1;
 #endif
 #ifndef CX_PRODUCT
-    if (g_v7_dbg) {
+    if (g_v7_dbg && epi != GEMM_EPI_RESID_LN) {
         p.tiles_m = (p.M + BM7 - 1) / BM7;
         p.tiles_n = p.N / BN7;
         p.sup_n = force_gn > 0 ? force_gn : v7_groups(p.tiles_m, p.tiles_n, p.K);
@@ -678,5 +704,6 @@
     p.sup_m = v7_stagger_unit(p, epi);
     return epi == GEMM_EPI_SWIGLU_G        ? launch7<GEMM_EPI_SWIGLU_G>(p, stream)
            : epi == GEMM_EPI_SWIGLU_BWD_AG ? launch7<GEMM_EPI_SWIGLU_BWD_AG>(p, stream)
+           : epi == GEMM_EPI_RESID_LN      ? launch7<GEMM_EPI_RESID_LN>(p, stream)
                                            : launch7<GEMM_EPI_NONE>(p, stream);
 }
diff --git a/contrastors_amd/csrc/gemm_params.h b/contrastors_amd/csrc/gemm_params.h
--- a/contrastors_amd/csrc/gemm_params.h
+++ b/contrastors_amd/csrc/gemm_params.h
@@ -8,6 +8,7 @@
        GEMM_EPI_SWIGLU_G = 5,
        GEMM_EPI_SWIGLU_BWD_AG = 6,
        GEMM_EPI_QACT_BWD = 8,
+       GEMM_EPI_RESID_LN = 9,
        GEMM_EPI_ACT_BWD = 7 };
 
 struct GemmParams {
@@ -27,6 +28,12 @@
     float* colsum_part;
     int sup_m, sup_n;
     long long* trace;
+    void* Out3;
+    int ldo3;
+    const float* ln_mean;
+    const float* ln_rstd;
+    const float* ln_gamma;
+    const float* ln_beta;
 };
 
 hipError_t cx_launch_gemm_v5(GemmParams p, int form, int out_mode, int epi, hipStream_t stream);
diff --git a/contrastors_amd/csrc/layernorm.hip b/contrastors_amd/csrc/layernorm.hip
--- a/contrastors_amd/csrc/layernorm.hip
+++ b/contrastors_amd/csrc/layernorm.hip
@@ -61,7 +61,6 @@
     rstd = rsqrtf(wave_mean(v, d) + eps);
 }
 
-CX_DEVICE float ln_affine(float z, float mean, float rstd, float g, float b) { return (z - mean) * rstd * g + b; }
 CX_DEVICE float ln_bwd_accum(float zz, float g, float dy, float mean, float rstd, float& s1, float& s2, float& dg, float& db) {
     const float xh = (zz - mean) * rstd;
     const float wdy = g * dy;
diff --git a/contrastors_amd/loss.py b/contrastors_amd/loss.py
--- a/contrastors_amd/loss.py
+++ b/contrastors_amd/loss.py
@@ -330,8 +330,10 @@
     return bool(getattr(trunk, "uses_rng", False)) if trunk is not None else bool(getattr(model, "training", False))
 
 
-def get_chunked_embeddings(model, chunks, rand_states=None, keep_tail: int = 0, kept: Optional[dict] = None):
+def get_chunked_embeddings(model, chunks, rand_states=None, keep_tail: int = 0, kept: Optional[dict] = None,
+                           ln_stats: Optional[list] = None):
     embs = []
+    capture = getattr(getattr(model, "trunk", None), "capture_ln_stats", None) if ln_stats is not None else None
     needed = rand_states is not None and _uses_rng(model)
     n = len(chunks)
     trainable = kept is not None and keep_tail > 0 and model.training and not getattr(model, "frozen_trunk", False)
@@ -349,6 +351,8 @@
                     out = model(**c)["embedding"]
                 kept[i] = out
                 embs.append(out.detach())
+                if ln_stats is not None:
+                    ln_stats.append(None)
                 continue
             except torch.OutOfMemoryError:
                 if outstanding is not None:
@@ -357,20 +361,34 @@
                 if rand_states is not None:
                     rand_states[-1].restore()
                 _log_once(("gradcache-tail-oom",), "GradCache: a kept chunk ran out of memory; the rest of the step re-forwards")
+        if capture is not None:
+            capture()
         with torch.no_grad():
             embs.append(model(**c)["embedding"])
+        if ln_stats is not None:
+            ln_stats.append(trunk.take_ln_stats() if capture is not None else None)
     return torch.cat(embs, dim=0)
 
 
-def accumulate_gradients(model, chunks, cache, rand_states=None, final: bool = False, skip=()):
+def accumulate_gradients(model, chunks, cache, rand_states=None, final: bool = False, skip=(), ln_stats: Optional[list] = None):
     todo = [i for i in range(len(chunks)) if i not in skip]
+    trunk = getattr(model, "trunk", None)
     for i in todo:
         c, g = chunks[i], cache[i]
+        st = ln_stats[i] if ln_stats is not None and i < len(ln_stats) else None
+        if st is not None and hasattr(trunk, "offer_ln_stats"):
+            ln_stats[i] = None
+            trunk.offer_ln_stats(st)
         state = rand_states[i] if rand_states is not None else RandContext(c, needed=False)
         if final and i == todo[-1] and hasattr(model, "arm_overlapped_reduce"):
             model.arm_overlapped_reduce()
-        with state:
-            out = model(**c)["embedding"]
+        try:
+            with state:
+                out = model(**c)["embedding"]
+        finally:
+            if st is not None and hasattr(trunk, "clear_ln_stats"):
+                trunk.clear_ln_stats()
+        del st
         out.backward(g.to(out.dtype))
 
 
@@ -636,9 +654,11 @@
                       f"{len(q_chunks)} + {len(d_chunks)}) keep their activations (no re-forward for them)")
         q_rnd, d_rnd = [], []
         q_kept, d_kept = {}, {}
+        q_st = [] if was_training1 and not fell_back else None
+        d_st = [] if was_training2 and not fell_back else None
         try:
-            q_embs = get_chunked_embeddings(tower1, q_chunks, q_rnd, keep_tail=nq_keep, kept=q_kept)
-            d_embs = get_chunked_embeddings(tower2, d_chunks, d_rnd, keep_tail=nd_keep, kept=d_kept)
+            q_embs = get_chunked_embeddings(tower1, q_chunks, q_rnd, keep_tail=nq_keep, kept=q_kept, ln_stats=q_st)
+            d_embs = get_chunked_embeddings(tower2, d_chunks, d_rnd, keep_tail=nd_keep, kept=d_kept, ln_stats=d_st)
             q_cache, d_cache, loss = cache_loss(q_embs, d_embs, logit_scale, bidirectional=bidirectional, use_fp8=pol.use_fp8)
         except BaseException:
             _release_resident(tower1, list(q_kept.values()))
@@ -662,9 +682,9 @@
                 tower2.arm_overlapped_reduce()
             o.backward(d_grads[i].to(o.dtype))
         if re_q:
-            accumulate_gradients(tower1, q_chunks, q_grads, q_rnd, final=(not shared) or not re_d, skip=done_q)
+            accumulate_gradients(tower1, q_chunks, q_grads, q_rnd, final=(not shared) or not re_d, skip=done_q, ln_stats=q_st)
         if re_d:
-            accumulate_gradients(tower2, d_chunks, d_grads, d_rnd, final=True, skip=done_d)
+            accumulate_gradients(tower2, d_chunks, d_grads, d_rnd, final=True, skip=done_d, ln_stats=d_st)
     seen = set()
     for tw, active in ((tower1, was_training1), (tower2, was_training2)):
         if active and id(tw) not in seen and hasattr(tw, "sync_gradients"):
diff --git a/contrastors_amd/nomic_bert.py b/contrastors_amd/nomic_bert.py
--- a/contrastors_amd/nomic_bert.py
+++ b/contrastors_amd/nomic_bert.py
@@ -188,6 +188,7 @@
             else:
                 setattr(self.desc, name, t[name].data_ptr() if name in t else None)
         self.emb_out: Optional[torch.Tensor] = None
+        self.ln_stats = None
 
     def nbytes(self) -> int:
         return sum(x.numel() * x.element_size() for x in self.tensors.values())
@@ -200,6 +201,14 @@
 
 
 _FULL_CACHE: Dict[tuple, tuple] = {}
+
+
+class LnStatsCache:
+
+    __slots__ = ("t", "T", "B", "epoch")
+
+    def __init__(self, t: torch.Tensor, T: int, B: int, epoch: int):
+        self.t, self.T, self.B, self.epoch = t, T, B, epoch
 
 
 @dataclass
@@ -318,6 +327,10 @@
         self._arena_nograd: Optional[_ChunkArena] = None
         self._arena_free: List[_ChunkArena] = []
         self._outstanding = 0
+        self.reforward_stats = True
+        self._stats_mode = None
+        self._stats_captured = None
+        self._weights_epoch = 0
         self._overlap_armed = None
         self._ov_works = None
         self.gradient_checkpointing = False
@@ -455,6 +468,7 @@
 
     @torch.no_grad()
     def sync_shadows(self):
+        self._weights_epoch = getattr(self, "_weights_epoch", 0) + 1
         s = _C.cur_stream()
         n = self._lin_end - self._lin_begin
         _C.check(self.lib.cx_cast_f32_to_bf16(self.flat_param.data_ptr() + 4 * self._lin_begin, self.w16.data_ptr(),
@@ -778,6 +792,42 @@
             self.checkpoint_keep = parse_checkpoint_keep(keep_layers, "checkpoint_keep_layers")
         self._arena_free = []
 
+    def _stats_supported(self) -> bool:
+        return bool(getattr(self, "reforward_stats", False)) and not self.uses_rng and type(self).forward_chunk is NomicBertEngine.forward_chunk
+
+    def capture_ln_stats(self):
+        self._stats_captured = None
+        self._stats_mode = ("capture", None) if self._stats_supported() else None
+
+    def take_ln_stats(self):
+        st, self._stats_captured, self._stats_mode = self._stats_captured, None, None
+        return st
+
+    def offer_ln_stats(self, st):
+        self._stats_mode = ("replay", st) if st is not None and self._stats_supported() else None
+
+    def clear_ln_stats(self):
+        self._stats_mode = None
+
+    def _new_stats(self, vb: VarlenBatch):
+        try:
+            t = torch.empty(self.config.n_layer, 2, 2, _round_up(vb.T, 64), dtype=torch.float32, device=self.device_)
+        except torch.OutOfMemoryError:
+            return None
+        return LnStatsCache(t, vb.T, vb.B, self._weights_epoch)
+
+    def _stats_for(self, vb: VarlenBatch, arena: _ChunkArena, save: bool):
+        mode, self._stats_mode = getattr(self, "_stats_mode", None), None
+        if not self._stats_supported():
+            return None, False
+        if mode is not None and mode[0] == "replay" and save:
+            st = mode[1]
+            if st.T == vb.T and st.B == vb.B and st.epoch == self._weights_epoch:
+                return st, True
+        if (mode is not None and mode[0] == "capture" and not save) or (save and arena.checkpoint and arena.keep_layers < self.config.n_layer):
+            return self._new_stats(vb), False
+        return None, False
+
     def forward_chunk(self, vb: VarlenBatch, save_for_backward: bool, normalize: Optional[bool] = None,
                       out: Optional[torch.Tensor] = None) -> Tuple[torch.Tensor, Optional[_ChunkArena]]:
         d = self.config.n_embd
@@ -790,7 +840,19 @@
         arena = self._get_arena(vb.T, vb.B, save_for_backward)
         self._arm_dropout(arena)
         self._desc.normalize = int(self.normalize_default if normalize is None else normalize)
-        if vb.token_type_ids is None:
+        stats, stats_valid = self._stats_for(vb, arena, save_for_backward)
+        arena.ln_stats = stats if save_for_backward else None
+        if stats is not None:
+            if vb.token_type_ids is not None:
+                self._check_token_types()
+            rc = self.lib.cx_encoder_forward_stats(C.byref(self._desc), C.byref(arena.desc), vb.input_ids.data_ptr(),
+                                                   _C.ptr(vb.token_type_ids), vb.indices.data_ptr(), vb.cu_seqlens.data_ptr(),
+                                                   vb.B, vb.S, vb.T, vb.max_seqlen, int(save_for_backward), out.data_ptr(),
+                                                   stats.t.data_ptr(), stats.t.shape[-1], int(stats_valid), _C.cur_stream())
+            _C.check(rc, "cx_encoder_forward_stats")
+            if not save_for_backward:
+                self._stats_captured = stats
+        elif vb.token_type_ids is None:
             rc = self.lib.cx_encoder_forward(C.byref(self._desc), C.byref(arena.desc), vb.input_ids.data_ptr(),
                                              vb.indices.data_ptr(), vb.cu_seqlens.data_ptr(), vb.B, vb.S, vb.T,
                                              vb.max_seqlen, int(save_for_backward), out.data_ptr(), _C.cur_stream())
@@ -826,7 +888,15 @@
         self._desc.normalize = arena.normalize
         sids, perm = vb.embedding_sort()
         fires = self._begin_backward(arena)
-        if vb.token_type_ids is None:
+        stats, arena.ln_stats = getattr(arena, "ln_stats", None), None
+        if stats is not None and arena.checkpoint:
+            rc = self.lib.cx_encoder_backward_stats(C.byref(self._desc), C.byref(arena.desc), vb.input_ids.data_ptr(),
+                                                    _C.ptr(vb.token_type_ids), vb.indices.data_ptr(), vb.cu_seqlens.data_ptr(),
+                                                    vb.B, vb.S, vb.T, vb.max_seqlen, demb.data_ptr(), arena.emb_out.data_ptr(),
+                                                    _C.ptr(sids), _C.ptr(perm), stats.t.data_ptr(), stats.t.shape[-1],
+                                                    _C.cur_stream())
+            _C.check(rc, "cx_encoder_backward_stats")
+        elif vb.token_type_ids is None:
             rc = self.lib.cx_encoder_backward(C.byref(self._desc), C.byref(arena.desc), vb.input_ids.data_ptr(),
                                               vb.indices.data_ptr(), vb.cu_seqlens.data_ptr(), vb.B, vb.S, vb.T,
                                               vb.max_seqlen, demb.data_ptr(), arena.emb_out.data_ptr(), _C.ptr(sids),
diff --git a/include/contrastors_hip.h b/include/contrastors_hip.h
--- a/include/contrastors_hip.h
+++ b/include/contrastors_hip.h
@@ -110,6 +110,10 @@
 int cx_gemm_bf16_nt_residual(const uint16_t* X, const uint16_t* W, uint16_t* Out, const float* bias,
                              const uint16_t* Residual, int M, int N, int K, int ldx, int ldw, int ldo, int ldr,
                              void* stream);
+int cx_gemm_bf16_nt_residual_ln(const uint16_t* X, const uint16_t* W, uint16_t* Z, uint16_t* H, const float* bias,
+                                const uint16_t* Residual, const float* mean, const float* rstd, const float* gamma,
+                                const float* beta, int M, int N, int K, int ldx, int ldw, int ldz, int ldr, int ldh,
+                                void* stream);
 int cx_gemm_bf16_nt_splitk(const uint16_t* X, const uint16_t* W, uint16_t* Out, const float* bias, const uint16_t* Residual,
                            float* ws, long ws_floats, int M, int N, int K, int ldx, int ldw, int ldo, int ldr, void* stream);
 int cx_gemm_bf16_swiglu(const uint16_t* X, const uint16_t* W, uint16_t* YG, uint16_t* Act, int M, int I, int K, int ldx,
@@ -323,6 +327,14 @@
                               const int64_t* token_type_ids, const int32_t* indices, const int32_t* cu_seqlens, int Bc, int S,
                               int T, int max_seqlen, const float* demb, const float* emb_out, const int32_t* sort_ids,
                               const int32_t* sort_perm, void* stream);
+int cx_encoder_forward_stats(const CxEncoderDesc* enc, const CxChunkBuffers* buf, const int64_t* input_ids,
+                             const int64_t* token_type_ids, const int32_t* indices, const int32_t* cu_seqlens, int Bc, int S,
+                             int T, int max_seqlen, int save_for_backward, float* emb_out, float* ln_stats, long stats_ld,
+                             int stats_valid, void* stream);
+int cx_encoder_backward_stats(const CxEncoderDesc* enc, const CxChunkBuffers* buf, const int64_t* input_ids,
+                              const int64_t* token_type_ids, const int32_t* indices, const int32_t* cu_seqlens, int Bc, int S,
+                              int T, int max_seqlen, const float* demb, const float* emb_out, const int32_t* sort_ids,
+                              const int32_t* sort_perm, const float* ln_stats, long stats_ld, void* stream);
 
 int cx_encoder_forward_hidden(const CxEncoderDesc* enc, const CxChunkBuffers* buf, const int64_t* input_ids,
                               const int32_t* indices, const int32_t* cu_seqlens, int Bc, int S, int T, int max_seqlen,
```

After: 4433 (median of 6 runs). Within noise of the previous version (+0.9%).
